# karpathy/minbpe

Hardware: AMD Instinct MI355X
Metric: BPE merges/sec (higher is better)
Workload: dtype int32; 1 GPU; regex1g: RegexTokenizer.train, 1 GB synth seed 2, vocab 32000; mode=default, parallelism=single

## Files before the change

minbpe_amd/csrc/api/api_ctx.hip:

```cpp

struct DpComm {
    bpe_allreduce_fn fn = nullptr;
    void *user = nullptr;
    int rank = 0, nranks = 1;
};

struct bpe_ctx {
    int device = 0;
    int num_cus = 256;
    hipStream_t stream = nullptr;
    bool own_stream = false;
    std::string err;

    uint8_t *d_bytes = nullptr;
    uint64_t nbytes = 0, cap_bytes = 0;
    uint64_t *d_offsets = nullptr;
    uint64_t n_chunks = 0, cap_offsets = 0;
    bool have_bytes = false;
    uint8_t *d_wexp = nullptr;
    const struct DpComm *dp_comm = nullptr;
    long long *d_dp_ckey = nullptr;
    uint32_t *d_dp_cfold = nullptr;
    uint64_t cap_dp_cfold = 0;
    bool dp_force_comm = false;
    int dp_kcap = DP_KCAP_DEFAULT;
    uint64_t *d_round_lb = nullptr;
    uint64_t cap_round_lb = 0;
    bool fuse_load = true;
    uint64_t cap_wexp = 0;
    bool weighted = false;

    uint32_t *d_ids[2] = {nullptr, nullptr};
    uint64_t cap_ids = 0;
    int par = 0;
    uint64_t n = 0;
    bool have_ids = false;

    uint32_t *d_mat = nullptr, *d_first = nullptr, *d_rowmax = nullptr;
    uint32_t vcap = 0;
    uint32_t vcur = 0;
    bool stats_valid = false;

    DevState *d_st = nullptr;
    uint64_t *d_tsum = nullptr, *d_tile_off = nullptr;
    uint8_t *d_tile_sin = nullptr;
    unsigned long long *d_sup = nullptr;
    uint64_t cap_tiles = 0;
    IterRec *h_rec = nullptr;
    int rec_cap = 0;
    unsigned long long *d_scratch = nullptr;
    uint32_t *d_delta = nullptr;
    uint32_t *d_dirty_list = nullptr;
    uint32_t *d_dirty_n = nullptr;
    int depth = 8;
    int repack_acc = 200;
    double repack_waste = 0.0;
    int use_slots = 2;
    int fused_rows = 0;
    uint32_t sel_epoch = 0;
    unsigned long long apply_target = 0;
    int rep_shift = 5;
    bool slotted = false;
    uint64_t slot_T = 0;
    int mq = 0;
    uint32_t *d_meta[2] = {nullptr, nullptr};
    uint4 *d_hdr[2] = {nullptr, nullptr};
    uint32_t *d_slot_lens = nullptr;
    unsigned long long *d_slot_off = nullptr, *d_slot_bsum = nullptr;
    uint32_t *d_ids2 = nullptr;
    bool slot2 = false;
    SlotHdr *d_hdr2[2] = {nullptr, nullptr};
    StageRec *d_stage = nullptr;
    uint32_t *d_smask = nullptr;
    uint32_t *d_cand = nullptr;
    uint32_t *d_idx = nullptr;
    uint32_t *d_idx_tmp = nullptr;
    uint32_t *d_idx_dirty = nullptr;
    uint32_t *d_removed = nullptr;
    uint64_t idx_cap_words = 0;
    uint64_t idx_cap_rows = 0;
    bool idx_rebuild = false;
    bool last_aa_indexed = false;
    bool idx_live = false;
    int use_sparse = 1;
    int rep_max = 8;
    int rep_min = 4;
    int lds_delta = 1;
    int exp_no_delta = 0;
    int tie_window = 0;
    int tie_index = 1;
    int sparse_ratio = 1;
    uint64_t last_count = ~0ull;
    uint64_t n_sparse = 0, n_dense = 0, n_index_builds = 0;
    uint64_t n_lean = 0, n_deferred = 0;
    int lean = 1;
    int64_t lean_count = 1 << 20;
    int lean_backoff = 1;
    int lean_grid = 256;
    int lean_scan = 31;
    int lean_select = 1;
    int aa_sparse = 1;
    int lean_chain = 1;
    int chain_dense = 1;
    unsigned long long *d_chain_req = nullptr;
    int ts = TILE2_MAX;
    int small_slots = 1;
    int count_is_removed = 1;
    int chain_prefetch = 1;
    int chain_kcap = CH_KSWEEP;
    int fuse_step = 0;
    unsigned long long *d_step_pub = nullptr;
    uint32_t *d_step_bar = nullptr;
    uint32_t step_bar_target = 0;
    bool forced = false;
    int32_t *d_forced = nullptr;
    uint64_t cap_forced = 0;
    int enc_replay = 1;
    int pinned_upload = 1;
    uint8_t *h_stage = nullptr;
    hipEvent_t ev_stage[4] = {nullptr, nullptr, nullptr, nullptr};
    bool stage_busy[4] = {false, false, false, false};
    uint64_t n_fused = 0;
    unsigned long long *d_step_stamps = nullptr;
    int pool_hint = 0;
    PoolEnt *d_pool = nullptr;
    uint32_t *d_pool_gather = nullptr;
    int chain_scan = 127;
    int chain = 1;
    StepRec *h_srec = nullptr;
    uint64_t n_steps = 0, n_full = 0, n_chained = 0;
    int lean_sum = 1;
    uint4 *d_lean_sum = nullptr;
    bool sum_valid = false;
    uint32_t *d_dbits = nullptr;
    unsigned long long *d_lean_res = nullptr;
    uint32_t lean_tag = 0;
    bool rows_pending = false;
    uint64_t cap_slots = 0;
    int dp_rank = 0, dp_nranks = 1, dp_merges = 0, dp_enq = 0, dp_done = 0;
    bool dp_active = false;
    void *comm = nullptr;
    int comm_rank = 0, comm_nranks = 1;
    uint32_t *d_dp_folded = nullptr, *d_dp_table = nullptr;
    long long *d_dp_key = nullptr;
    uint64_t dp_cur_len = 0;
    bool dp_sparse = false;
    uint32_t dp_dl = 0;
    std::vector<uint8_t> dp_flip;
    int merge_impl = 0;
    unsigned long long *d_desc = nullptr;
    unsigned long long *d_gdesc = nullptr;
    uint64_t cap_desc = 0;
    uint32_t epoch = 0;
    uint32_t lb_tune = 1;

    uint32_t *d_enc_tmp = nullptr, *d_enc_len = nullptr;
    int32_t *d_enc_out = nullptr;
    unsigned long long *d_enc_off = nullptr, *d_enc_bsum = nullptr, *d_enc_long = nullptr;
    unsigned long long *d_enc_huge = nullptr;
    int enc_long = 1;
    unsigned long long *d_ht_keys = nullptr;
    uint32_t *d_ht_vals = nullptr;
    int32_t *d_merge_ids = nullptr;
    uint64_t cap_enc_n = 0, cap_enc_chunks = 0, cap_ht = 0, cap_merge_ids = 0;
    EncEntry *d_enc_tab = nullptr;
    uint32_t *d_enc_rep = nullptr;
    uint8_t *d_enc_mid = nullptr;
    uint32_t *d_enc_midn = nullptr;
    uint64_t cap_enc_tab = 0;
    int enc_cache = 1;
    int enc_chain = 1;
    int enc_hash_bits = 0;

    uint8_t *d_dec_blob = nullptr, *d_dec_out = nullptr;
    unsigned long long *d_dec_voff = nullptr, *d_dec_off = nullptr, *d_dec_bsum = nullptr;
    int32_t *d_dec_ids = nullptr;
    uint32_t *d_dec_len = nullptr;
    uint64_t cap_dec_blob = 0, cap_dec_voff = 0, cap_dec_n = 0, cap_dec_out = 0;
    uint32_t dec_V = 0;
    bool dec_have_vocab = false, dec_have_result = false;
    uint64_t dec_n = 0, dec_total = 0;

    int mode = 1;
    int profile = 0;
    int prof_iter = -1;
    int prof_stride = 64;
    bool prof_active = false;
    int scan_sup_min = 1024;
    int k1 = 2;
    bool stream_is_bytes = false;

    std::vector<ProfEv> prof_open;
    std::vector<hipEvent_t> ev_pool;
    double prof_ms[BPE_PROF_NKINDS] = {0};
    uint64_t prof_launches[BPE_PROF_NKINDS] = {0};
    uint64_t prof_bytes[BPE_PROF_NKINDS] = {0};
};

#define GK(c, kern) ((c)->ts == TILE2_MIN ? bpe::bpe_g1::kern : bpe::bpe_g4::kern)
inline uint32_t idx_h(const bpe_ctx *c) { return c->ts == TILE2_MIN ? bpe::bpe_g1::IDX_H : bpe::bpe_g4::IDX_H; }

namespace {

int fail(bpe_ctx *c, int code, const char *fmt, ...) {
    char buf[512];
    va_list ap;
    va_start(ap, fmt);
    vsnprintf(buf, sizeof buf, fmt, ap);
    va_end(ap);
    if (c) c->err = buf; else g_create_err = buf;
    return code;
}

#define HIPCHK(c, call)                                                                  \
    do {                                                                                 \
        hipError_t e_ = (call);                                                          \
        if (e_ != hipSuccess)                                                            \
            return fail((c), BPE_E_HIP, "%s failed: %s (%s:%d)", #call, hipGetErrorString(e_), \
                        __FILE__, __LINE__);                                             \
    } while (0)

#define LAUNCHCHK(c, name)                                                                \
    do {                                                                                  \
        hipError_t e_ = hipGetLastError();                                                \
        if (e_ != hipSuccess)                                                             \
            return fail((c), BPE_E_HIP, "launch %s failed: %s", name, hipGetErrorString(e_)); \
    } while (0)

#define TRY(expr)              \
    do {                       \
        int rc_ = (expr);      \
        if (rc_ != BPE_OK) return rc_; \
    } while (0)

struct DevTmp {
    void *p = nullptr;
    DevTmp() = default;
    DevTmp(const DevTmp &) = delete;
    DevTmp &operator=(const DevTmp &) = delete;
    ~DevTmp() {
        if (p) (void)hipFree(p);
    }
    hipError_t alloc(size_t bytes) { return hipMalloc(&p, bytes ? bytes : 1); }
    template <typename T>
    T *as() const { return (T *)p; }
};

struct EventList {
    std::vector<hipEvent_t> v;
    ~EventList() {
        for (hipEvent_t e : v)
            if (e) (void)hipEventDestroy(e);
    }
};

template <typename T>
int dev_realloc(bpe_ctx *c, T *&p, size_t count) {
    if (p) HIPCHK(c, hipFree(p));
    p = nullptr;
    if (count) HIPCHK(c, hipMalloc((void **)&p, count * sizeof(T)));
    return BPE_OK;
}

inline uint64_t ntiles_of(uint64_t n) { return (n + TILE - 1) / TILE; }

int ensure_ids(bpe_ctx *c, uint64_t n) {
    const uint64_t need = (ntiles_of(n) + 2) * TILE;
    if (need > c->cap_ids) {
        TRY(dev_realloc(c, c->d_ids[0], need));
        TRY(dev_realloc(c, c->d_ids[1], need));
        TRY(dev_realloc(c, c->d_ids2, need));
        c->cap_ids = need;
    }
    const uint64_t nt = ntiles_of(n) + 1;
    const uint64_t nt2 = (TILE / TILE2_MIN) * nt + 4;
    if (nt > c->cap_tiles) {
        TRY(dev_realloc(c, c->d_tsum, nt));
        TRY(dev_realloc(c, c->d_tile_off, nt));
        TRY(dev_realloc(c, c->d_tile_sin, nt));
        TRY(dev_realloc(c, c->d_sup, 2 * 3 * (nt / SUP_TILES + 2)));
        TRY(dev_realloc(c, c->d_meta[0], nt));
        TRY(dev_realloc(c, c->d_meta[1], nt));
        TRY(dev_realloc(c, c->d_hdr[0], nt));
        TRY(dev_realloc(c, c->d_hdr[1], nt));
        TRY(dev_realloc(c, c->d_hdr2[0], nt2));
        TRY(dev_realloc(c, c->d_hdr2[1], nt2));
        TRY(dev_realloc(c, c->d_stage, nt2));
        TRY(dev_realloc(c, c->d_smask, nt2 / 32 + 2));
        TRY(dev_realloc(c, c->d_cand, nt2));
        HIPCHK(c, hipMemsetAsync(c->d_smask, 0, (nt2 / 32 + 2) * sizeof(uint32_t), c->stream));
        TRY(dev_realloc(c, c->d_slot_lens, nt2));
        TRY(dev_realloc(c, c->d_slot_off, nt2 + 1));
        TRY(dev_realloc(c, c->d_slot_bsum, nt2 / SCAN_TILE + 2));
        TRY(dev_realloc(c, c->d_desc, nt2));
        TRY(dev_realloc(c, c->d_gdesc, nt / 64 + 2));
        HIPCHK(c, hipMemsetAsync(c->d_desc, 0, nt2 * sizeof(unsigned long long), c->stream));
        HIPCHK(c, hipMemsetAsync(c->d_gdesc, 0, (nt / 64 + 2) * sizeof(unsigned long long), c->stream));
        c->cap_tiles = nt;
    }
    return BPE_OK;
}

int ensure_table(bpe_ctx *c, uint32_t v) {
    if (v > 65535) return fail(c, BPE_E_LIMIT, "vocab %u exceeds this build's 65535 limit", v);
    if (v <= c->vcap) return BPE_OK;
    uint32_t nv = std::max<uint32_t>(v, 256);
    nv = (nv + 63) & ~63u;
    TRY(dev_realloc(c, c->d_mat, (size_t)nv * nv));
    TRY(dev_realloc(c, c->d_rowmax, (size_t)nv * 2));
    TRY(dev_realloc(c, c->d_delta, (size_t)nv * 4 * DELTA_REPL + 256 * DELTA_SKEW));
    TRY(dev_realloc(c, c->d_dirty_list, (size_t)nv));
    if (!c->d_dirty_n) HIPCHK(c, hipMalloc((void **)&c->d_dirty_n, sizeof(uint32_t)));
    if (!c->d_dbits) {
        HIPCHK(c, hipMalloc((void **)&c->d_dbits, DBITS_WORDS * sizeof(uint32_t)));
        HIPCHK(c, hipMemsetAsync(c->d_dbits, 0, DBITS_WORDS * sizeof(uint32_t), c->stream));
    }
    TRY(dev_realloc(c, c->d_lean_res, 2 * ((size_t)nv + 8)));
    if (!c->d_lean_sum) HIPCHK(c, hipMalloc((void **)&c->d_lean_sum, 4 * (size_t)LEAN_SUM_CAP * sizeof(uint4)));
    HIPCHK(c, hipMemsetAsync(c->d_lean_res, 0, 2 * ((size_t)nv + 8) * sizeof(unsigned long long), c->stream));
    if (!c->d_removed) {
        HIPCHK(c, hipMalloc((void **)&c->d_removed, 256 * REMOVED_STRIDE * sizeof(uint32_t)));
        HIPCHK(c, hipMemsetAsync(c->d_removed, 0, 256 * REMOVED_STRIDE * sizeof(uint32_t), c->stream));
    }
    HIPCHK(c, hipMemsetAsync(c->d_delta, 0, ((size_t)nv * 4 * DELTA_REPL + 256 * DELTA_SKEW) * sizeof(uint32_t), c->stream));
    HIPCHK(c, hipMemsetAsync(c->d_dirty_n, 0, sizeof(uint32_t), c->stream));
    HIPCHK(c, hipMemsetAsync(c->d_rowmax, 0, (size_t)nv * 2 * sizeof(uint32_t), c->stream));
    if (c->d_first) {
        HIPCHK(c, hipFree(c->d_first));
        c->d_first = nullptr;
    }
    c->vcap = nv;
    c->stats_valid = false;
    return BPE_OK;
}

int ensure_rec(bpe_ctx *c, int n) {
    if (n <= c->rec_cap) return BPE_OK;
    if (c->h_rec) HIPCHK(c, hipHostFree(c->h_rec));
    c->h_rec = nullptr;
    HIPCHK(c, hipHostMalloc((void **)&c->h_rec, sizeof(IterRec) * (size_t)n, hipHostMallocMapped));
    c->rec_cap = n;
    return BPE_OK;
}

int ensure_srec(bpe_ctx *c) {
    if (!c->h_srec) HIPCHK(c, hipHostMalloc((void **)&c->h_srec, sizeof(StepRec) * STEP_RING, hipHostMallocMapped));
    memset(c->h_srec, 0, sizeof(StepRec) * STEP_RING);
    return BPE_OK;
}

constexpr int PROF_FULL_ITERS = 1024;
int prof_begin(bpe_ctx *c, int kind, uint64_t bytes) {
    c->prof_active = c->profile >= 2 || (c->profile == 1 && kind == BPE_PROF_MERGE);
    if (!c->prof_active) return BPE_OK;
    uint32_t weight = 1;
    if (c->prof_iter >= PROF_FULL_ITERS && c->prof_stride > 1) {
        if (c->prof_iter % c->prof_stride) {
            c->prof_active = false;
            return BPE_OK;
        }
        weight = (uint32_t)c->prof_stride;
    }
    ProfEv ev;
    ev.kind = kind;
    ev.bytes = bytes;
    ev.weight = weight;
    for (hipEvent_t *e : {&ev.e0, &ev.e1}) {
        if (!c->ev_pool.empty()) {
            *e = c->ev_pool.back();
            c->ev_pool.pop_back();
        } else {
            HIPCHK(c, hipEventCreate(e));
        }
    }
    HIPCHK(c, hipEventRecord(ev.e0, c->stream));
    c->prof_open.push_back(ev);
    return BPE_OK;
}
int prof_end(bpe_ctx *c) {
    if (!c->prof_active) return BPE_OK;
    c->prof_active = false;
    HIPCHK(c, hipEventRecord(c->prof_open.back().e1, c->stream));
    return BPE_OK;
}
int prof_drain(bpe_ctx *c) {
    if (c->prof_open.empty()) return BPE_OK;
    HIPCHK(c, hipStreamSynchronize(c->stream));
    for (ProfEv &ev : c->prof_open) {
        float ms = 0.f;
        HIPCHK(c, hipEventElapsedTime(&ms, ev.e0, ev.e1));
        c->prof_ms[ev.kind] += (double)ms * ev.weight;
        c->prof_launches[ev.kind] += ev.weight;
        c->prof_bytes[ev.kind] += ev.bytes * ev.weight;
        c->ev_pool.push_back(ev.e0);
        c->ev_pool.push_back(ev.e1);
    }
    c->prof_open.clear();
    return BPE_OK;
}

int dp_allreduce(bpe_ctx *c, void *buf, uint64_t count, int32_t dtype, int32_t op) {
    const DpComm *dp = c->dp_comm;
    if (!dp || !dp->fn) return fail(c, BPE_E_STATE, "no communicator");
    if (dp->nranks == 1 && !c->dp_force_comm) return BPE_OK;
    const int rc = dp->fn(dp->user, buf, count, dtype, op, (void *)c->stream);
    if (rc != 0) return fail(c, BPE_E_HIP, "all-reduce failed (%d)", rc);
    return BPE_OK;
}

inline unsigned grid_for(uint64_t work_items, unsigned per_block, unsigned cap) {
    uint64_t g = (work_items + per_block - 1) / per_block;
    if (g < 1) g = 1;
    if (g > cap) g = cap;
    return (unsigned)g;
}

inline bool load_count_fusable(const bpe_ctx *c) { return c->fuse_load && c->k1 == 2 && !c->weighted && c->nbytes >= 2; }

int start_from_bytes(bpe_ctx *c, bool count = false) {
    const uint64_t n = c->nbytes;
    TRY(ensure_ids(c, n));
    if (count) {
        const uint64_t segs = (n + LC_SEG - 1) / LC_SEG;
        if (segs + 2 > c->cap_round_lb) {
            TRY(dev_realloc(c, c->d_round_lb, (size_t)segs + 2));
            c->cap_round_lb = segs + 2;
        }
        TRY(prof_begin(c, BPE_PROF_PAIR_COUNT, 4 * n));
        const uint64_t *off = c->n_chunks ? c->d_offsets : nullptr;
        if (off) {
            hipLaunchKernelGGL(k_seg_lb, dim3((unsigned)((segs + 256) / 256)), dim3(256), 0, c->stream, off,
                               (uint64_t)c->n_chunks, segs, c->d_round_lb);
            LAUNCHCHK(c, "k_seg_lb");
        }
        const uint64_t wgs = (segs + LC_WAVES - 1) / LC_WAVES;
        hipLaunchKernelGGL(k_load_count, dim3((unsigned)std::min<uint64_t>(wgs, (uint64_t)c->num_cus)), dim3(PC_THREADS),
                           LC_LDS_BYTES, c->stream, c->d_bytes, off, c->d_round_lb, (uint64_t)c->n_chunks, n, c->d_ids[0],
                           c->d_mat, c->vcap);
        LAUNCHCHK(c, "k_load_count");
        hipLaunchKernelGGL(k_init_state, dim3(1), dim3(1), 0, c->stream, c->d_st, (unsigned long long)n);
        LAUNCHCHK(c, "k_init_state");
        TRY(prof_end(c));
    } else {
        TRY(prof_begin(c, BPE_PROF_WIDEN, 5 * n));
        if (n) {
            hipLaunchKernelGGL(k_widen, dim3(grid_for(n, 256 * 16, c->num_cus * 8)), dim3(256), 0,
                               c->stream, c->d_bytes, c->d_ids[0], n);
            LAUNCHCHK(c, "k_widen");
            if (c->n_chunks) {
                hipLaunchKernelGGL(k_mark_starts, dim3(grid_for(c->n_chunks, 256, c->num_cus * 8)),
                                   dim3(256), 0, c->stream, c->d_ids[0], c->d_offsets, c->n_chunks, n);
                LAUNCHCHK(c, "k_mark_starts");
                if (c->weighted) {
                    hipLaunchKernelGGL(k_mark_weights, dim3(grid_for(c->n_chunks, 256, c->num_cus * 8)), dim3(256),
                                       0, c->stream, c->d_ids[0], c->d_offsets, c->d_wexp, c->n_chunks, n);
                    LAUNCHCHK(c, "k_mark_weights");
                }
            }
        }
        hipLaunchKernelGGL(k_init_state, dim3(1), dim3(1), 0, c->stream, c->d_st, (unsigned long long)n);
        LAUNCHCHK(c, "k_init_state");
        TRY(prof_end(c));
    }
    c->apply_target = 0;
    c->par = 0;
    c->n = n;
    c->vcur = 256;
    c->have_ids = true;
    c->stats_valid = false;
    c->stream_is_bytes = true;
    return BPE_OK;
}

int clear_table(bpe_ctx *c) {
    TRY(prof_begin(c, BPE_PROF_TABLE, 0));
    HIPCHK(c, hipMemsetAsync(c->d_mat, 0, (size_t)c->vcur * c->vcap * sizeof(uint32_t), c->stream));
    TRY(prof_end(c));
    return BPE_OK;
}

int launch_pair_count(bpe_ctx *c, bool with_first) {
    const uint64_t n = c->n;
    TRY(prof_begin(c, BPE_PROF_PAIR_COUNT, 4 * n));
    if (n >= 2) {
        if (with_first) {
            hipLaunchKernelGGL(k_pair_count_simple<true>, dim3(grid_for(n, 1024, c->num_cus * 8)),
                               dim3(256), 0, c->stream, c->d_ids[c->par], c->d_st, c->par, c->d_mat,
                               c->vcap, c->d_first);
        } else if (c->k1 == 0) {
            hipLaunchKernelGGL(k_pair_count_simple<false>, dim3(grid_for(n, 1024, c->num_cus * 8)),
                               dim3(256), 0, c->stream, c->d_ids[c->par], c->d_st, c->par, c->d_mat,
                               c->vcap, (uint32_t *)nullptr);
        } else if (c->k1 == 2 && c->vcur <= 256 && c->stream_is_bytes && !c->weighted) {
            hipLaunchKernelGGL(k_pair_count_bytes, dim3(grid_for(n, 4 * PC_THREADS, c->num_cus)),
                               dim3(PC_THREADS), PC_LDS_BYTES, c->stream, c->d_ids[c->par], c->d_st,
                               c->par, c->d_mat, c->vcap);
        } else if (c->k1 >= 3 && !c->weighted && c->vcap <= 65536) {
            hipLaunchKernelGGL(k_pair_count_h32, dim3(grid_for(n, 4 * PC_THREADS, c->num_cus)),
                               dim3(PC_THREADS), PC_LDS_BYTES, c->stream, c->d_ids[c->par], c->d_st,
                               c->par, c->d_mat, c->vcap);
        } else {
            hipLaunchKernelGGL(k_pair_count_lds, dim3(grid_for(n, 4 * PC_THREADS, c->num_cus)),
                               dim3(PC_THREADS), PC_LDS_BYTES, c->stream, c->d_ids[c->par], c->d_st,
                               c->par, c->d_mat, c->vcap);
        }
        LAUNCHCHK(c, "k_pair_count");
    }
    TRY(prof_end(c));
    return BPE_OK;
}

inline uint32_t vcap_rep(const bpe_ctx *c) { return c->vcap | ((uint32_t)c->rep_shift << 24); }

SlotRef stream_ref(const bpe_ctx *c) {
    SlotRef r;
    if (c->slotted) {
        r.b0 = c->d_ids[0];
        r.b1 = c->d_ids[1];
        r.meta = c->d_meta[c->mq];
        r.T = c->slot_T;
    } else {
        r.b0 = c->d_ids[c->par];
        r.b1 = nullptr;
        r.meta = nullptr;
        r.T = 0;
    }
    return r;
}

SlotRefH stream_ref_h(const bpe_ctx *c) {
    SlotRefH r;
    r.b0 = c->d_ids[0];
    r.b1 = c->d_ids[1];
    r.hdr = c->d_hdr2[c->mq];
    r.T = c->slot_T;
    return r;
}

inline bool aa_through_index(const bpe_ctx *c) { return c->aa_sparse && c->idx_live; }

int launch_select(bpe_ctx *c, bool rowmax_all, bool sparse_next = false) {
    TRY(prof_begin(c, BPE_PROF_ARGMAX, 0));
    if (c->forced) {
        hipLaunchKernelGGL(GK(c, k_forced_pair), dim3(1), dim3(1), 0, c->stream, c->d_st, c->d_forced, (uint32_t)c->prof_iter,
                           c->d_mat, c->vcap);
        LAUNCHCHK(c, "k_forced_pair");
        if (sparse_next && c->slotted && c->slot2) {
            CandArgs C;
            C.idx = c->d_idx;
            C.dirty = c->d_idx_dirty;
            C.cand = c->d_cand;
            C.stride = (uint32_t)c->idx_cap_words;
            C.T = (uint32_t)c->slot_T;
            C.enable = 1;
            C.tie_index = C.tie_window = 0;
            C.aa = aa_through_index(c) ? 1u : 0u;
            hipLaunchKernelGGL(GK(c, k_dp_cand), dim3(1), dim3(1024), 0, c->stream, c->d_st, C);
            LAUNCHCHK(c, "k_dp_cand");
        }
        TRY(prof_end(c));
        return BPE_OK;
    }
    if (rowmax_all) {
        hipLaunchKernelGGL(k_rowmax_all, dim3(c->vcur), dim3(256), 0, c->stream, c->d_mat, c->vcap,
                           c->vcur, c->d_rowmax);
        LAUNCHCHK(c, "k_rowmax_all");
    }
    const uint64_t nslots = c->slotted ? c->slot_T : ntiles_of(c->n);
    const unsigned blocks = (unsigned)std::max<uint64_t>(1, std::min<uint64_t>(nslots, TIE_BLOCKS));
    CandArgs C;
    C.idx = c->d_idx;
    C.dirty = c->d_idx_dirty;
    C.cand = c->d_cand;
    C.stride = (uint32_t)c->idx_cap_words;
    C.T = (uint32_t)c->slot_T;
    C.enable = sparse_next ? 1u : 0u;
    C.tie_index = (c->slotted && c->slot2 && c->idx_live && c->tie_index) ? 1u : 0u;
    C.tie_window = c->tie_window ? 1u : 0u;
    C.aa = (sparse_next && aa_through_index(c)) ? 1u : 0u;
    if (c->slotted && c->slot2)
        hipLaunchKernelGGL(GK(c, k_select<SlotRefH>), dim3(blocks), dim3(1024), 0, c->stream, c->d_rowmax, c->d_mat,
                           c->vcap, c->vcur, c->d_st, stream_ref_h(c), c->par, c->dp_active ? 1 : 0,
                           ++c->sel_epoch, C);
    else
        hipLaunchKernelGGL(k_select<SlotRef>, dim3(blocks), dim3(1024), 0, c->stream, c->d_rowmax, c->d_mat,
                           c->vcap, c->vcur, c->d_st, stream_ref(c), c->par, c->dp_active ? 1 : 0,
                           ++c->sel_epoch, C);
    LAUNCHCHK(c, "k_select");
    TRY(prof_end(c));
    return BPE_OK;
}

int launch_rowsel_lean(bpe_ctx *c) {
    TRY(prof_begin(c, BPE_PROF_ARGMAX, 0));
    CandArgs C;
    C.idx = c->d_idx;
    C.dirty = c->d_idx_dirty;
    C.cand = nullptr;
    C.stride = (uint32_t)c->idx_cap_words;
    C.T = (uint32_t)c->slot_T;
    C.enable = 0;
    C.tie_index = 1;
    C.tie_window = 0;
    C.aa = 0;
    hipLaunchKernelGGL(GK(c, k_rowsel_lean), dim3(1 + (unsigned)c->lean_scan), dim3(1024), 0, c->stream, c->d_rowmax, c->d_mat,
                       c->vcap, c->vcur, c->d_st, stream_ref_h(c), C, c->d_dbits, c->d_lean_res, ++c->lean_tag);
    LAUNCHCHK(c, "k_rowsel_lean");
    TRY(prof_end(c));
    c->rows_pending = false;
    return BPE_OK;
}

int launch_sel_lean(bpe_ctx *c) {
    TRY(prof_begin(c, BPE_PROF_ARGMAX, 0));
    CandArgs C;
    C.idx = c->d_idx;
    C.dirty = c->d_idx_dirty;
    C.cand = nullptr;
    C.stride = (uint32_t)c->idx_cap_words;
    C.T = (uint32_t)c->slot_T;
    C.enable = 0;
    C.tie_index = 1;
    C.tie_window = 0;
    C.aa = 0;
    const uint32_t nwv = ((c->vcur + 255u) / 256u) * 4u;
    hipLaunchKernelGGL(GK(c, k_sel_lean), dim3(1 + (unsigned)c->lean_scan), dim3(1024), 0, c->stream, c->d_rowmax, c->d_mat,
                       c->vcap, c->vcur, c->d_st, stream_ref_h(c), C, c->d_dbits, c->d_lean_res, ++c->lean_tag,
                       c->d_lean_sum, nwv, (uint32_t)c->lean_chain);
    LAUNCHCHK(c, "k_sel_lean");
    TRY(prof_end(c));
    c->rows_pending = false;
    return BPE_OK;
}

int flush_lean_rows(bpe_ctx *c, uint32_t ncols) {
    if (!c->rows_pending) return BPE_OK;
    TRY(prof_begin(c, BPE_PROF_TABLE, 0));
    hipLaunchKernelGGL(GK(c, k_rowmax_lean), dim3((unsigned)c->lean_scan), dim3(1024), 0, c->stream, c->d_mat, c->vcap,
                       c->d_rowmax, c->d_st, ncols, c->d_dbits);
    LAUNCHCHK(c, "k_rowmax_lean");
    TRY(prof_end(c));
    c->rows_pending = false;
    return BPE_OK;
}

template <bool FOLDED>
int launch_table_update(bpe_ctx *c, uint32_t *delta, uint32_t Z, int par, IterRec *rec, int iter,
                        int slot_finish) {
    const uint32_t na = (Z + 1 + 31) / 32;
    if (c->fused_rows) {
        c->apply_target += na;
        hipLaunchKernelGGL(k_apply_delta<FOLDED>, dim3(na + ROW_BLOCKS), dim3(256), 0, c->stream, c->d_mat,
                           c->vcap, delta, FOLDED ? c->vcap : vcap_rep(c), c->d_rowmax, c->d_st, Z,
                           c->d_dirty_list, c->d_dirty_n, par, rec, iter, slot_finish, na,
                           c->apply_target);
    } else {
        hipLaunchKernelGGL(k_apply_delta<FOLDED>, dim3(na), dim3(256), 0, c->stream, c->d_mat, c->vcap,
                           delta, FOLDED ? c->vcap : vcap_rep(c), c->d_rowmax, c->d_st, Z,
                           c->d_dirty_list, c->d_dirty_n, par, rec, iter, slot_finish, na, 0ull);
        LAUNCHCHK(c, "k_apply_delta");
        hipLaunchKernelGGL(k_rowmax_list, dim3(ROW_BLOCKS), dim3(256), 0, c->stream, c->d_mat, c->vcap,
                           Z + 1, c->d_rowmax, c->d_st, c->d_dirty_list, c->d_dirty_n);
    }
    LAUNCHCHK(c, "k_apply_delta");
    return BPE_OK;
}

int launch_merge(bpe_ctx *c, uint32_t newid, int iter, IterRec *rec, bool with_delta) {
    const uint64_t n = c->n;
    const uint64_t nt = ntiles_of(n);
    TRY(prof_begin(c, BPE_PROF_MERGE, 0));
    if (c->merge_impl == 1) {
        if ((++c->epoch & EPOCH_MASK) == 0) {
            HIPCHK(c, hipMemsetAsync(c->d_desc, 0, c->cap_tiles * sizeof(unsigned long long), c->stream));
            HIPCHK(c, hipMemsetAsync(c->d_gdesc, 0, (c->cap_tiles / 64 + 2) * sizeof(unsigned long long), c->stream));
            c->epoch++;
        }
        const unsigned grid = (unsigned)std::max<uint64_t>(nt, 1);
        if (with_delta)
            hipLaunchKernelGGL(k_merge_lookback<true>, dim3(grid), dim3(MT), 0, c->stream,
                               c->d_ids[c->par], c->d_ids[c->par ^ 1], c->d_st, c->par, c->d_desc,
                               c->d_gdesc, c->epoch, newid, c->d_delta, vcap_rep(c), rec, iter, c->d_dirty_n, c->lb_tune);
        else
            hipLaunchKernelGGL(k_merge_lookback<false>, dim3(grid), dim3(MT), 0, c->stream,
                               c->d_ids[c->par], c->d_ids[c->par ^ 1], c->d_st, c->par, c->d_desc,
                               c->d_gdesc, c->epoch, newid, (uint32_t *)nullptr, c->vcap, rec, iter, c->d_dirty_n,
                               c->lb_tune);
        LAUNCHCHK(c, "k_merge_lookback");
    } else {
    if (nt) {
        hipLaunchKernelGGL(k_merge_count, dim3((unsigned)nt), dim3(MT), 0, c->stream,
                           c->d_ids[c->par], c->d_st, c->par, c->d_tsum);
        LAUNCHCHK(c, "k_merge_count");
    }
    if (nt > (uint64_t)c->scan_sup_min) {
        static_assert(sizeof(TS) == 24, "a TS is three 8-byte words");
        const uint64_t nsup = (nt + SUP_TILES - 1) / SUP_TILES;
        TS *ssum = reinterpret_cast<TS *>(c->d_sup), *spre = ssum + (nt / SUP_TILES + 2);
        hipLaunchKernelGGL(k_tile_sup, dim3((unsigned)nsup), dim3(SUP_TILES), 0, c->stream, c->d_tsum, nt, c->d_st, c->par, ssum);
        hipLaunchKernelGGL(k_tile_scan_sup, dim3(1), dim3(1024), 0, c->stream, ssum, nsup, spre, c->d_st, c->par, rec, iter,
                           c->d_ids[c->par], c->d_dirty_n);
        hipLaunchKernelGGL(k_tile_expand, dim3((unsigned)nsup), dim3(SUP_TILES), 0, c->stream, c->d_tsum, nt, c->d_st, c->par,
                           spre, c->d_tile_off, c->d_tile_sin);
    } else {
        hipLaunchKernelGGL(k_tile_scan, dim3(1), dim3(1024), 0, c->stream, c->d_tsum, nt, c->d_tile_off,
                           c->d_tile_sin, c->d_st, c->par, rec, iter, c->d_ids[c->par], c->d_dirty_n);
    }
    LAUNCHCHK(c, "k_tile_scan");
    if (nt) {
        if (with_delta)
            hipLaunchKernelGGL(k_merge_scatter<true>, dim3((unsigned)nt), dim3(MT), 0, c->stream,
                               c->d_ids[c->par], c->d_ids[c->par ^ 1], c->d_st, c->par,
                               c->d_tile_off, c->d_tile_sin, newid, c->d_delta, vcap_rep(c));
        else
            hipLaunchKernelGGL(k_merge_scatter<false>, dim3((unsigned)nt), dim3(MT), 0, c->stream,
                               c->d_ids[c->par], c->d_ids[c->par ^ 1], c->d_st, c->par,
                               c->d_tile_off, c->d_tile_sin, newid, (uint32_t *)nullptr, c->vcap);
        LAUNCHCHK(c, "k_merge_scatter");
    }
    }
    TRY(prof_end(c));
    if (with_delta && c->dp_active) {
        hipLaunchKernelGGL(k_dp_fold, dim3((c->vcap + 255) / 256), dim3(256), 0, c->stream, c->d_delta,
                           vcap_rep(c), newid, c->d_dp_folded);
        LAUNCHCHK(c, "k_dp_fold");
    } else if (with_delta) {
        TRY(prof_begin(c, BPE_PROF_TABLE, 0));
        TRY(launch_table_update<false>(c, c->d_delta, newid, 0, nullptr, 0, 0));
        TRY(prof_end(c));
    }
    c->par ^= 1;
    c->stats_valid = false;
    c->stream_is_bytes = false;
    return BPE_OK;
}


int slots_enter(bpe_ctx *c) {
    c->slot_T = ntiles_of(c->n);
    c->mq = 0;
    hipLaunchKernelGGL(k_slot_init, dim3(grid_for(std::max<uint64_t>(c->slot_T, 1), 256, c->num_cus * 4)),
                       dim3(256), 0, c->stream, c->d_meta[0], c->d_hdr[0], c->slot_T, c->d_st, c->par,
                       (uint32_t)c->par, c->d_ids[c->par]);
    LAUNCHCHK(c, "k_slot_init");
    c->slotted = true;
    return BPE_OK;
}

int slots_leave(bpe_ctx *c) {
    const uint64_t T = c->slot_T;
    if (T) {
        const uint64_t nb = (T + SCAN_TILE - 1) / SCAN_TILE;
        hipLaunchKernelGGL(k_slot_lens, dim3(grid_for(T, 256, c->num_cus * 4)), dim3(256), 0, c->stream,
                           c->d_meta[c->mq], T, c->d_slot_lens);
        hipLaunchKernelGGL(k_scan_blocksum, dim3((unsigned)nb), dim3(256), 0, c->stream, c->d_slot_lens, T,
                           c->d_slot_bsum);
        hipLaunchKernelGGL(k_scan_top, dim3(1), dim3(1024), 0, c->stream, c->d_slot_bsum, nb,
                           c->d_scratch + 3);
        hipLaunchKernelGGL(k_scan_apply, dim3((unsigned)nb), dim3(256), 0, c->stream, c->d_slot_lens, T,
                           c->d_slot_bsum, c->d_slot_off);
        hipLaunchKernelGGL(k_slot_compact, dim3((unsigned)T), dim3(256), 0, c->stream, c->d_ids[0],
                           c->d_ids[1], c->d_meta[c->mq], c->d_slot_off, c->d_ids2);
        LAUNCHCHK(c, "k_slot_compact");
    }
    std::swap(c->d_ids[0], c->d_ids2);
    if (c->par != 0) {
        hipLaunchKernelGGL(k_move_n, dim3(1), dim3(1), 0, c->stream, c->d_st, c->par, 0);
        LAUNCHCHK(c, "k_move_n");
    }
    c->par = 0;
    c->slotted = false;
    return BPE_OK;
}

int launch_merge_slot(bpe_ctx *c, uint32_t newid, int iter, IterRec *rec) {
    TRY(prof_begin(c, BPE_PROF_MERGE, 0));
    if ((++c->epoch & EPOCH_MASK) == 0) {
        HIPCHK(c, hipMemsetAsync(c->d_desc, 0, c->cap_tiles * sizeof(unsigned long long), c->stream));
        HIPCHK(c, hipMemsetAsync(c->d_gdesc, 0, (c->cap_tiles / 64 + 2) * sizeof(unsigned long long), c->stream));
        c->epoch++;
    }
    const unsigned slot_grid = (unsigned)std::max<uint64_t>(c->slot_T, 1);
    hipLaunchKernelGGL(k_merge_slot<true>, dim3(slot_grid), dim3(MT), 0,
                       c->stream, c->d_ids[0], c->d_ids[1], c->d_ids[0], c->d_ids[1], c->d_meta[c->mq],
                       c->d_meta[c->mq ^ 1], c->slot_T, c->d_st, c->par, newid, c->d_delta, vcap_rep(c),
                       c->d_dirty_n, c->d_desc, c->epoch, c->d_hdr[c->mq], c->d_hdr[c->mq ^ 1]);
    LAUNCHCHK(c, "k_merge_slot");
    TRY(prof_end(c));
    if (c->dp_active) {
        hipLaunchKernelGGL(k_dp_fold, dim3((c->vcap + 255) / 256), dim3(256), 0, c->stream, c->d_delta,
                           vcap_rep(c), newid, c->d_dp_folded);
        LAUNCHCHK(c, "k_dp_fold");
    } else {
        TRY(prof_begin(c, BPE_PROF_TABLE, 0));
        TRY(launch_table_update<false>(c, c->d_delta, newid, c->par, rec, iter, 1));
        TRY(prof_end(c));
    }
    c->par ^= 1;
    c->mq ^= 1;
    c->stats_valid = false;
    c->stream_is_bytes = false;
    return BPE_OK;
}

constexpr unsigned SPARSE_GRID = 1024;

int index_build(bpe_ctx *c) {
    const uint64_t nwords = (c->slot_T + 31) / 32;
    if (nwords + 4 > c->idx_cap_words || idx_h(c) > c->idx_cap_rows) {
        if (c->d_idx) HIPCHK(c, hipFree(c->d_idx));
        if (c->d_idx_dirty) HIPCHK(c, hipFree(c->d_idx_dirty));
        c->d_idx = c->d_idx_dirty = nullptr;
        const uint64_t cap = (nwords + 4 + 63) / 64 * 64;
        if (c->d_idx_tmp) HIPCHK(c, hipFree(c->d_idx_tmp));
        c->d_idx_tmp = nullptr;
        c->idx_cap_words = c->idx_cap_rows = 0;
        HIPCHK(c, hipMalloc((void **)&c->d_idx, cap * idx_h(c) * sizeof(uint32_t)));
        HIPCHK(c, hipMalloc((void **)&c->d_idx_tmp, cap * idx_h(c) * sizeof(uint32_t)));
        HIPCHK(c, hipMalloc((void **)&c->d_idx_dirty, cap * sizeof(uint32_t)));
        c->idx_cap_words = cap;
        c->idx_cap_rows = idx_h(c);
    }
    if (nwords) {
        hipLaunchKernelGGL(GK(c, k_index_build), dim3((unsigned)nwords), dim3(1024), (size_t)idx_h(c) * 4, c->stream,
                           c->d_ids[0], c->d_ids[1], c->d_hdr2[c->mq], (uint32_t)c->slot_T, c->d_idx_tmp,
                           c->d_idx_dirty, c->d_st);
        LAUNCHCHK(c, "k_index_build");
        hipLaunchKernelGGL(GK(c, k_index_transpose), dim3((unsigned)((nwords + 31) / 32), idx_h(c) / 32), dim3(256), 0,
                           c->stream, c->d_idx_tmp, (uint32_t)nwords, c->d_idx, (uint32_t)c->idx_cap_words);
        LAUNCHCHK(c, "k_index_transpose");
    }
    c->idx_live = true;
    c->idx_rebuild = false;
    c->n_index_builds++;
    return BPE_OK;
}

int slots2_enter(bpe_ctx *c) {
    c->slot_T = (c->n + (uint64_t)c->ts - 1) / (uint64_t)c->ts;
    c->mq = 0;
    hipLaunchKernelGGL(GK(c, k_slot2_init), dim3(grid_for(std::max<uint64_t>(c->slot_T, 1), 256, c->num_cus * 4)),
                       dim3(256), 0, c->stream, c->d_hdr2[0], c->slot_T, c->d_st, c->par, (uint32_t)c->par,
                       c->d_ids[c->par]);
    LAUNCHCHK(c, "k_slot2_init");
    c->slotted = true;
    c->slot2 = true;
    HIPCHK(c, hipMemsetAsync(c->d_smask, 0, (c->slot_T / 32 + 1) * sizeof(uint32_t), c->stream));
    if (c->idx_live) TRY(index_build(c));
    return BPE_OK;
}

int slots2_leave(bpe_ctx *c) {
    const uint64_t T = c->slot_T;
    if (T) {
        const uint64_t nb = (T + SCAN_TILE - 1) / SCAN_TILE;
        hipLaunchKernelGGL(GK(c, k_slot2_lens), dim3(grid_for(T, 256, c->num_cus * 4)), dim3(256), 0, c->stream,
                           c->d_hdr2[c->mq], T, c->d_slot_lens);
        hipLaunchKernelGGL(k_scan_blocksum, dim3((unsigned)nb), dim3(256), 0, c->stream, c->d_slot_lens, T,
                           c->d_slot_bsum);
        hipLaunchKernelGGL(k_scan_top, dim3(1), dim3(1024), 0, c->stream, c->d_slot_bsum, nb,
                           c->d_scratch + 3);
        hipLaunchKernelGGL(k_scan_apply, dim3((unsigned)nb), dim3(256), 0, c->stream, c->d_slot_lens, T,
                           c->d_slot_bsum, c->d_slot_off);
        hipLaunchKernelGGL(GK(c, k_slot2_compact), dim3((unsigned)((T + 3) / 4)), dim3(256), 0, c->stream, c->d_ids[0],
                           c->d_ids[1], c->d_hdr2[c->mq], T, c->d_slot_off, c->d_ids2);
        LAUNCHCHK(c, "k_slot2_compact");
    }
    std::swap(c->d_ids[0], c->d_ids2);
    if (c->par != 0) {
        hipLaunchKernelGGL(k_move_n, dim3(1), dim3(1), 0, c->stream, c->d_st, c->par, 0);
        LAUNCHCHK(c, "k_move_n");
    }
    c->par = 0;
    c->slotted = false;
    c->slot2 = false;
    return BPE_OK;
}

inline uint32_t delta_layout(const bpe_ctx *c, uint32_t Z) {
    const uint32_t dstride = std::min<uint32_t>(c->vcap, ((Z + 1 + 63) / 64) * 64);
    const uint64_t buf_words = (uint64_t)c->vcap * 4 * DELTA_REPL;
    int shift = 0;
    while (shift < 7 && ((uint64_t)dstride * 4 << (shift + 1)) <= buf_words) shift++;
    const uint64_t cnt = c->last_count;
    const int want = cnt >= (1u << 20) ? 8 : (cnt >= (1u << 16) ? 5 : (cnt >= (1u << 12) ? 3 : 0));
    return dstride | ((uint32_t)std::min(std::min(shift, std::max(want, c->rep_min)), c->rep_max) << 24);
}

int plan_pass2(bpe_ctx *c, bool *sparse_out) {
    const uint32_t T = (uint32_t)c->slot_T;
    const bool small = T <= 16 * SPARSE_GRID;
    const bool can_index = c->use_sparse && T > 0 && (c->use_sparse == 2 || !small || c->lean);
    const bool rare = c->last_count != ~0ull && (small ? c->last_count <= (uint64_t)c->lean_count
                                                       : c->last_count * (uint64_t)c->sparse_ratio < T);
    const bool sparse = can_index && (c->use_sparse == 2 || rare);
    if (sparse && c->small_slots && c->ts != TILE2_MIN && (!small || c->small_slots == 2)) {
        TRY(slots2_leave(c));
        c->ts = TILE2_MIN;
        TRY(slots2_enter(c));
    }
    if (sparse && (!c->idx_live || c->idx_rebuild)) TRY(index_build(c));
    *sparse_out = sparse;
    return BPE_OK;
}

int launch_passes2(bpe_ctx *c, uint32_t newid, bool sparse, uint32_t dl) {
    TRY(prof_begin(c, BPE_PROF_MERGE, 0));
    if ((++c->epoch & EPOCH_MASK) == 0) {
        HIPCHK(c, hipMemsetAsync(c->d_desc, 0, ((TILE / TILE2_MIN) * c->cap_tiles + 4) * sizeof(unsigned long long), c->stream));
        c->epoch++;
    }
    const uint32_t T = (uint32_t)c->slot_T;
    AbArgs A;
    A.b0 = c->d_ids[0];
    A.b1 = c->d_ids[1];
    A.hdr_in = c->d_hdr2[c->mq];
    A.hdr_out = c->d_hdr2[c->mq ^ 1];
    A.stage = c->d_stage;
    A.smask = c->d_smask;
    A.T = T;
    A.st = c->d_st;
    A.newid = newid;
    A.delta = c->exp_no_delta ? nullptr : c->d_delta;
    A.vcap = dl;
    A.idx = c->idx_live ? c->d_idx : nullptr;
    A.istride = (uint32_t)c->idx_cap_words;
    A.cand = c->d_cand;
    A.removed = c->d_removed;
    A.dirty_n = c->d_dirty_n;
    const bool ldsd = c->lds_delta && newid + 1 <= (uint32_t)LDSD_CAP;
    if (sparse) {
        if (ldsd)
            hipLaunchKernelGGL(GK(c, k_merge_ab_sparse<true>), dim3(SPARSE_GRID), dim3(MT), 0, c->stream, A);
        else
            hipLaunchKernelGGL(GK(c, k_merge_ab_sparse<false>), dim3(SPARSE_GRID), dim3(MT), 0, c->stream, A);
        c->n_sparse++;
    } else {
        const unsigned g = std::max((T + MT / 64 - 1) / (MT / 64), 1u);
        const unsigned ge = std::min(g, 5u * (unsigned)c->num_cus);
        if (ldsd && A.idx)
            hipLaunchKernelGGL(GK(c, k_merge_ab_dense_early<true>), dim3(ge), dim3(MT), 0, c->stream, A);
        else if (ldsd)
            hipLaunchKernelGGL(GK(c, k_merge_ab_dense_early<false>), dim3(ge), dim3(MT), 0, c->stream, A);
        else if (A.idx)
            hipLaunchKernelGGL(GK(c, k_merge_ab_dense<true>), dim3(g), dim3(MT), 0, c->stream, A);
        else
            hipLaunchKernelGGL(GK(c, k_merge_ab_dense<false>), dim3(g), dim3(MT), 0, c->stream, A);
        c->n_dense++;
    }
    LAUNCHCHK(c, "k_merge_ab");
    AaArgs B;
    B.b0 = c->d_ids[0];
    B.b1 = c->d_ids[1];
    B.w0 = c->d_ids[0];
    B.w1 = c->d_ids[1];
    B.hdr_in = A.hdr_in;
    B.hdr_out = A.hdr_out;
    B.stage = sparse ? c->d_stage : nullptr;
    B.smask = c->d_smask;
    B.T = T;
    B.st = c->d_st;
    B.newid = newid;
    B.delta = c->d_delta;
    B.vcap = dl;
    B.sdesc = c->d_desc;
    B.epoch = c->epoch;
    const bool aas = sparse && aa_through_index(c);
    B.dirty = (c->idx_live && !aas) ? c->d_idx_dirty : nullptr;
    B.removed = c->d_removed;
    B.cand = aas ? c->d_cand : nullptr;
    B.idx = aas ? c->d_idx : nullptr;
    B.istride = (uint32_t)c->idx_cap_words;
    c->last_aa_indexed = aas;
    hipLaunchKernelGGL(GK(c, k_merge_aa), dim3(std::max(1u, std::min(T, 8u * (unsigned)c->num_cus))), dim3(64), 0,
                       c->stream, B);
    LAUNCHCHK(c, "k_merge_aa");
    TRY(prof_end(c));
    return BPE_OK;
}

int launch_table2(bpe_ctx *c, uint32_t newid, int iter, IterRec *rec, bool sparse, uint32_t dl, bool folded) {
    const uint32_t T = (uint32_t)c->slot_T;
    TRY(prof_begin(c, BPE_PROF_TABLE, 0));
    const uint32_t na = (newid + 1 + 31) / 32;
    if (folded)
        hipLaunchKernelGGL(k_apply2<true>, dim3(na + 8), dim3(256), 0, c->stream, c->d_mat, c->vcap, c->d_dp_folded,
                           c->vcap, c->d_rowmax, c->d_st, newid, c->d_dirty_list, c->d_dirty_n, c->par, rec, iter,
                           na, c->d_hdr2[c->mq], c->d_stage, c->d_removed, c->d_smask, (T + 31) / 32);
    else
        hipLaunchKernelGGL(k_apply2<false>, dim3(na + 8), dim3(256), 0, c->stream, c->d_mat, c->vcap, c->d_delta, dl,
                           c->d_rowmax, c->d_st, newid, c->d_dirty_list, c->d_dirty_n, c->par, rec, iter, na,
                           c->d_hdr2[c->mq], c->d_stage, c->d_removed, c->d_smask, (T + 31) / 32);
    LAUNCHCHK(c, "k_apply2");
    hipLaunchKernelGGL(k_rowmax_list, dim3(ROW_BLOCKS), dim3(1024), 0, c->stream, c->d_mat, c->vcap, newid + 1,
                       c->d_rowmax, c->d_st, c->d_dirty_list, c->d_dirty_n);
    LAUNCHCHK(c, "k_rowmax_list");
    TRY(prof_end(c));
    c->par ^= 1;
    if (!sparse) c->mq ^= 1;
    c->stats_valid = false;
    c->stream_is_bytes = false;
    return BPE_OK;
}

int launch_merge2(bpe_ctx *c, uint32_t newid, int iter, IterRec *rec, bool sparse) {
    const uint32_t dl = delta_layout(c, newid);
    TRY(launch_passes2(c, newid, sparse, dl));
    return launch_table2(c, newid, iter, rec, sparse, dl, false);
}

int launch_lean(bpe_ctx *c, uint32_t newid, int iter, IterRec *rec, bool use_index) {
    const uint32_t T = (uint32_t)c->slot_T;
    const uint32_t dl = delta_layout(c, newid);
    AbArgs A;
    A.b0 = c->d_ids[0];
    A.b1 = c->d_ids[1];
    A.hdr_in = c->d_hdr2[c->mq];
    A.hdr_out = nullptr;
    A.stage = c->d_stage;
    A.smask = c->d_smask;
    A.T = T;
    A.st = c->d_st;
    A.newid = newid;
    A.delta = c->d_delta;
    A.vcap = dl;
    A.idx = c->idx_live ? c->d_idx : nullptr;
    A.istride = (uint32_t)c->idx_cap_words;
    A.cand = nullptr;
    A.removed = c->d_removed;
    A.dirty_n = c->d_dirty_n;
    const uint32_t nwords = (T + 31) / 32;
    const unsigned g = std::max(1u, std::min(use_index ? nwords : (T + 15) / 16, (unsigned)c->lean_grid));
    TRY(prof_begin(c, BPE_PROF_MERGE, 0));
    if (c->idx_live)
        hipLaunchKernelGGL(GK(c, k_merge_ab_lean<true>), dim3(g), dim3(LEAN_MT), 0, c->stream, A, c->d_idx_dirty,
                           use_index ? 1u : 0u, c->d_dbits);
    else
        hipLaunchKernelGGL(GK(c, k_merge_ab_lean<false>), dim3(g), dim3(LEAN_MT), 0, c->stream, A, (const uint32_t *)nullptr, 0u,
                           c->d_dbits);
    LAUNCHCHK(c, "k_merge_ab_lean");
    TRY(prof_end(c));
    TRY(prof_begin(c, BPE_PROF_TABLE, 0));
    const uint32_t na = (newid + 1 + 255) / 256;
    const uint32_t ncommit = std::max(8u, std::min(128u, (nwords + 255) / 256));
    hipLaunchKernelGGL(GK(c, k_apply_lean), dim3(na + ncommit), dim3(256), 0, c->stream, c->d_mat, c->vcap, c->d_delta, dl,
                       c->d_rowmax, c->d_st, newid, c->d_dbits, c->par, rec, iter, na, c->d_hdr2[c->mq], c->d_stage,
                       c->d_removed, c->d_smask, nwords, c->d_lean_sum);
    LAUNCHCHK(c, "k_apply_lean");
    TRY(prof_end(c));
    c->par ^= 1;
    c->stats_valid = false;
    c->stream_is_bytes = false;
    c->rows_pending = true;
    c->n_lean++;
    if (use_index) c->n_sparse++; else c->n_dense++;
    return BPE_OK;
}

int launch_chain_step(bpe_ctx *c, uint32_t step, uint32_t zhi, bool use_index, bool records, bool dense = false) {
    const uint32_t T = (uint32_t)c->slot_T;
    const uint32_t dl = delta_layout(c, zhi);
    const bool fused = c->fuse_step && !c->forced && !dense && !c->dp_comm && use_index && c->idx_live;
    if (!fused) TRY(prof_begin(c, BPE_PROF_ARGMAX, 0));
    CandArgs C;
    C.idx = c->d_idx;
    C.dirty = c->d_idx_dirty;
    C.cand = nullptr;
    C.stride = (uint32_t)c->idx_cap_words;
    C.T = T;
    C.enable = 0;
    C.tie_index = 1;
    C.tie_window = 0;
    C.aa = 0;
    if (!c->idx_live) C.T = 0;
    if (dense && c->dp_comm) C.T = 0;
    (void)records;
    if (!c->d_chain_req) {
        HIPCHK(c, hipMalloc((void **)&c->d_chain_req, PL_REQ_WORDS * sizeof(unsigned long long)));
        HIPCHK(c, hipMemsetAsync(c->d_chain_req, 0, PL_REQ_WORDS * sizeof(unsigned long long), c->stream));
    }
    if (!c->d_pool) {
        HIPCHK(c, hipMalloc((void **)&c->d_pool, (3 * PL_CAP + 128) * sizeof(PoolEnt)));
        HIPCHK(c, hipMalloc((void **)&c->d_pool_gather, (2 + 2 * PL_GATHER) * sizeof(uint32_t)));
        HIPCHK(c, hipMemsetAsync(c->d_pool, 0, (3 * PL_CAP + 128) * sizeof(PoolEnt), c->stream));
        HIPCHK(c, hipMemsetAsync(c->d_pool_gather, 0, (2 + 2 * PL_GATHER) * sizeof(uint32_t), c->stream));
    }
    const DpComm *dp = c->dp_comm;
    uint32_t kcap = (uint32_t)(dense ? CH_KDENSE : std::min(CH_KSWEEP, c->chain_kcap));
    if (dp) kcap = std::min(kcap, (uint32_t)c->dp_kcap);
    const uint32_t hint_below = (uint32_t)(c->pool_hint > 0 ? c->pool_hint : (int)kcap);
    const unsigned nscan = (unsigned)std::max(1, std::min(c->chain_scan, c->num_cus - 1));
    if (fused) {
        if (!c->d_step_pub) {
            HIPCHK(c, hipMalloc((void **)&c->d_step_pub, 64 * sizeof(unsigned long long)));
            HIPCHK(c, hipMemsetAsync(c->d_step_pub, 0, 64 * sizeof(unsigned long long), c->stream));
        }
        if (!c->d_step_bar) {
            HIPCHK(c, hipMalloc((void **)&c->d_step_bar, 256));
            HIPCHK(c, hipMemsetAsync(c->d_step_bar, 0, 256, c->stream));
            c->step_bar_target = 0;
        }
        const uint32_t nwords = (T + 31) / 32;
        StepArgs S;
        S.rowmax = c->d_rowmax;
        S.mat = c->d_mat;
        S.stride = c->vcap;
        S.st = c->d_st;
        S.ref = stream_ref_h(c);
        S.C = C;
        S.dbits = c->d_dbits;
        S.res = c->d_lean_res;
        S.tag = ++c->lean_tag;
        S.req = c->d_chain_req;
        S.kcap = kcap;
        S.pool = c->d_pool;
        S.gather = c->d_pool_gather;
        S.hint_below = hint_below;
        AbArgs &A = S.A;
        A.b0 = c->d_ids[0];
        A.b1 = c->d_ids[1];
        A.hdr_in = c->d_hdr2[c->mq];
        A.hdr_out = nullptr;
        A.stage = c->d_stage;
        A.smask = c->d_smask;
        A.T = T;
        A.st = c->d_st;
        A.newid = 0;
        A.delta = c->d_delta;
        A.vcap = dl;
        A.idx = c->d_idx;
        A.istride = (uint32_t)c->idx_cap_words;
        A.cand = nullptr;
        uint32_t *const removed = (c->weighted || !c->count_is_removed) ? c->d_removed : nullptr;
        A.removed = removed;
        A.dirty_n = c->d_dirty_n;
        S.idx_dirty = c->d_idx_dirty;
        S.use_index = 1u | (c->chain_prefetch ? 2u : 0u);
        const unsigned gapply = (zhi + 1 + 1023) / 1024;
        const unsigned cap = std::min((unsigned)c->num_cus, std::max(std::max((unsigned)c->lean_grid, gapply), 2u));
        const unsigned gmerge = std::max(1u, std::min(std::min(nwords, (unsigned)c->lean_grid), cap));
        const unsigned ns = std::min(nscan, cap - 1);
        const unsigned G = std::min(cap, std::max(std::max(gmerge, gapply), 1 + ns));
        if (G < gapply) return fail(c, BPE_E_INTERNAL, "fused chain step: %u workgroups cannot hold %u tokens", G, zhi + 1);
        S.nscan = ns;
        S.gm = gmerge;
        S.delta = c->d_delta;
        S.dl = dl;
        S.par = c->par;
        S.rec = c->h_rec;
        S.srec = c->h_srec;
        S.step = step;
        S.hdr_cur = c->d_hdr2[c->mq];
        S.stage = c->d_stage;
        S.removed = removed;
        S.smask = c->d_smask;
        S.nwords = nwords;
        S.sums = c->d_lean_sum;
        S.pub = c->d_step_pub;
        S.bar = c->d_step_bar;
        c->step_bar_target += G;
        S.bar_target = c->step_bar_target;
        S.stamps = c->d_step_stamps;
        TRY(prof_begin(c, BPE_PROF_MERGE, 0));
        hipLaunchKernelGGL(GK(c, k_step), dim3(G), dim3(LEAN_MT), 0, c->stream, S);
        LAUNCHCHK(c, "k_step");
        TRY(prof_end(c));
        c->par ^= 1;
        c->stats_valid = false;
        c->stream_is_bytes = false;
        c->rows_pending = true;
        c->n_steps++;
        c->n_fused++;
        c->n_sparse++;
        return BPE_OK;
    }
    if (c->forced)
        hipLaunchKernelGGL(GK(c, k_forced_sel), dim3(1), dim3(64), 0, c->stream, c->d_st, c->d_forced, c->d_mat, c->vcap, kcap);
    else
        hipLaunchKernelGGL(GK(c, k_pool_sel), dim3(1 + nscan), dim3(1024), 0, c->stream, c->d_rowmax, c->d_mat,
                           c->vcap, c->d_st, stream_ref_h(c), C, c->d_dbits, c->d_lean_res, ++c->lean_tag, c->d_chain_req,
                           kcap, c->d_pool, c->d_pool_gather, hint_below, dp ? c->d_dp_ckey : (long long *)nullptr,
                           (unsigned long long)(dp ? dp->rank : 0), c->d_pool + PL_CAP);
    LAUNCHCHK(c, "k_pool_sel");
    if (dp) {
        TRY(dp_allreduce(c, c->d_dp_ckey, DP_KEY_WORDS, BPE_DT_INT64, BPE_OP_MIN));
        hipLaunchKernelGGL(GK(c, k_pool_sel_dp), dim3(1), dim3(PL_CAP), 0, c->stream, c->d_st, c->d_dp_ckey, kcap, c->d_pool,
                           c->d_pool + PL_CAP, hint_below);
        LAUNCHCHK(c, "k_pool_sel_dp");
    }
    TRY(prof_end(c));
    AbArgs A;
    A.b0 = c->d_ids[0];
    A.b1 = c->d_ids[1];
    A.hdr_in = c->d_hdr2[c->mq];
    A.hdr_out = dense ? c->d_hdr2[c->mq ^ 1] : nullptr;
    A.stage = c->d_stage;
    A.smask = c->d_smask;
    A.T = T;
    A.st = c->d_st;
    A.newid = 0;
    A.delta = c->d_delta;
    A.vcap = dl;
    A.idx = c->idx_live ? c->d_idx : nullptr;
    A.istride = (uint32_t)c->idx_cap_words;
    A.cand = nullptr;
    uint32_t *const removed = (c->weighted || dp || !c->count_is_removed) ? c->d_removed : nullptr;
    A.removed = removed;
    A.dirty_n = c->d_dirty_n;
    const uint32_t nwords = (T + 31) / 32;
    TRY(prof_begin(c, BPE_PROF_MERGE, 0));
    if (dense) {
        const unsigned g = std::max(1u, std::min((T + 15) / 16, (unsigned)c->num_cus));
        hipLaunchKernelGGL(GK(c, k_merge_chain_dense), dim3(g), dim3(LEAN_MT), 0, c->stream, A, c->d_dbits);
        const unsigned g1 = std::max(1u, std::min((T + MT / 64 - 1) / (MT / 64), 5u * (unsigned)c->num_cus));
        hipLaunchKernelGGL(GK(c, k_merge_chain_dense1), dim3(g1), dim3(MT), 0, c->stream, A);
    } else {
        const unsigned g = std::max(1u, std::min(use_index ? nwords : (T + 15) / 16, (unsigned)c->lean_grid));
        hipLaunchKernelGGL(GK(c, k_merge_chain), dim3(g), dim3(LEAN_MT), 0, c->stream, A, c->d_idx_dirty,
                           (use_index ? 1u : 0u) | (c->chain_prefetch ? 2u : 0u), c->d_dbits);
    }
    LAUNCHCHK(c, "k_merge_chain");
    TRY(prof_end(c));
    TRY(prof_begin(c, BPE_PROF_TABLE, 0));
    const uint32_t na = (zhi + 1 + 255) / 256;
    const uint32_t ncommit = std::max(8u, std::min(128u, (nwords + 255) / 256));
    const uint32_t fS = std::min<uint32_t>(c->vcap, ((zhi + 1 + 63) / 64) * 64);
    uint32_t *ftail = dp ? c->d_dp_cfold + (size_t)2 * kcap * fS : nullptr;
    if (dp) {
        hipLaunchKernelGGL(GK(c, k_dp_fold_chain), dim3(na), dim3(256), 0, c->stream, c->d_delta, dl, c->d_st, c->d_dp_cfold, fS, ftail);
        LAUNCHCHK(c, "k_dp_fold_chain");
        TRY(dp_allreduce(c, c->d_dp_cfold, (uint64_t)2 * kcap * fS + 64, BPE_DT_INT32, BPE_OP_SUM));
    }
    hipLaunchKernelGGL(GK(c, k_apply_chain), dim3(na + ncommit), dim3(256), 0, c->stream, c->d_mat, c->vcap, c->d_delta, dl, c->d_rowmax,
                       c->d_st, c->d_dbits, c->par, c->h_rec, c->h_srec, step, na, c->d_hdr2[c->mq], c->d_stage,
                       removed, c->d_smask, nwords, c->d_lean_sum, dp ? c->d_dp_cfold : (const uint32_t *)nullptr, fS,
                       (const uint32_t *)ftail);
    LAUNCHCHK(c, "k_apply_chain");
    TRY(prof_end(c));
    c->par ^= 1;
    if (dense) c->mq ^= 1;
    c->stats_valid = false;
    c->stream_is_bytes = false;
    c->rows_pending = true;
    c->n_steps++;
    if (use_index) c->n_sparse++; else c->n_dense++;
    return BPE_OK;
}

constexpr size_t STAGE_PIECE = 32u << 20;
constexpr int STAGE_R = 4, STAGE_T_MAX = 16;
int upload_h2d(bpe_ctx *c, void *dst, const void *src, size_t bytes) {
    if (!bytes) return BPE_OK;
    if (!c->pinned_upload || bytes < 2 * STAGE_PIECE) {
        HIPCHK(c, hipMemcpyAsync(dst, src, bytes, hipMemcpyHostToDevice, c->stream));
        return BPE_OK;
    }
    if (!c->h_stage) {
        if (hipHostMalloc((void **)&c->h_stage, STAGE_PIECE * STAGE_R, hipHostMallocDefault) != hipSuccess) {
            c->h_stage = nullptr;
            (void)hipGetLastError();
            HIPCHK(c, hipMemcpyAsync(dst, src, bytes, hipMemcpyHostToDevice, c->stream));
            return BPE_OK;
        }
        for (int r = 0; r < STAGE_R; r++) HIPCHK(c, hipEventCreateWithFlags(&c->ev_stage[r], hipEventDisableTiming));
    }
    const unsigned hw = std::max(1u, std::thread::hardware_concurrency());
    const int T = (int)std::max(1u, std::min((unsigned)STAGE_T_MAX, hw / 2));
    const size_t pieces = (bytes + STAGE_PIECE - 1) / STAGE_PIECE;
    std::atomic<long long> go{-1};
    std::atomic<unsigned long long> done{0};
    const uint8_t *s8 = static_cast<const uint8_t *>(src);
    uint8_t *stage = c->h_stage;
    auto worker = [&](int w) {
        for (size_t i = 0; i < pieces; i++) {
            while (go.load(std::memory_order_acquire) < (long long)i) std::this_thread::yield();
            const size_t len = std::min(STAGE_PIECE, bytes - i * STAGE_PIECE);
            const size_t per = (len + (size_t)T - 1) / (size_t)T, lo = std::min(len, per * (size_t)w), hi = std::min(len, lo + per);
            if (hi > lo) memcpy(stage + (i % STAGE_R) * STAGE_PIECE + lo, s8 + i * STAGE_PIECE + lo, hi - lo);
            done.fetch_add(1, std::memory_order_release);
        }
    };
    std::vector<std::thread> pool;
    pool.reserve((size_t)T);
    for (int w = 1; w < T; w++) pool.emplace_back(worker, w);
    int rc = BPE_OK;
    hipError_t err = hipSuccess;
    for (size_t i = 0; i < pieces; i++) {
        if (c->stage_busy[i % STAGE_R] && err == hipSuccess) {
            err = hipEventSynchronize(c->ev_stage[i % STAGE_R]);
            c->stage_busy[i % STAGE_R] = false;
        }
        go.store((long long)i, std::memory_order_release);
        {
            const size_t len = std::min(STAGE_PIECE, bytes - i * STAGE_PIECE);
            const size_t per = (len + (size_t)T - 1) / (size_t)T, hi = std::min(len, per);
            if (hi) memcpy(stage + (i % STAGE_R) * STAGE_PIECE, s8 + i * STAGE_PIECE, hi);
            done.fetch_add(1, std::memory_order_release);
        }
        while (done.load(std::memory_order_acquire) < (unsigned long long)T * (i + 1)) std::this_thread::yield();
        if (err == hipSuccess) {
            const size_t len = std::min(STAGE_PIECE, bytes - i * STAGE_PIECE);
            err = hipMemcpyAsync(static_cast<uint8_t *>(dst) + i * STAGE_PIECE, stage + (i % STAGE_R) * STAGE_PIECE, len,
                                 hipMemcpyHostToDevice, c->stream);
            if (err == hipSuccess) err = hipEventRecord(c->ev_stage[i % STAGE_R], c->stream);
            if (err == hipSuccess) c->stage_busy[i % STAGE_R] = true;
        }
    }
    for (std::thread &t : pool) t.join();
    if (err != hipSuccess) rc = fail(c, BPE_E_HIP, "pinned upload: %s", hipGetErrorString(err));
    return rc;
}

int download_d2h(bpe_ctx *c, void *dst, const void *src_dev, size_t bytes) {
    if (!bytes) return BPE_OK;
    if (!c->pinned_upload || bytes < 2 * STAGE_PIECE || !c->h_stage) {
        HIPCHK(c, hipMemcpyAsync(dst, src_dev, bytes, hipMemcpyDeviceToHost, c->stream));
        HIPCHK(c, hipStreamSynchronize(c->stream));
        return BPE_OK;
    }
    const unsigned hw = std::max(1u, std::thread::hardware_concurrency());
    const int T = (int)std::max(1u, std::min((unsigned)STAGE_T_MAX, hw / 2));
    const size_t pieces = (bytes + STAGE_PIECE - 1) / STAGE_PIECE;
    std::atomic<long long> go{-1};
    std::atomic<unsigned long long> done{0};
    uint8_t *d8 = static_cast<uint8_t *>(dst);
    const uint8_t *stage = c->h_stage;
    auto copy_out = [&](size_t i, int w) {
        const size_t len = std::min(STAGE_PIECE, bytes - i * STAGE_PIECE);
        const size_t per = (len + (size_t)T - 1) / (size_t)T, lo = std::min(len, per * (size_t)w), hi = std::min(len, lo + per);
        if (hi > lo) memcpy(d8 + i * STAGE_PIECE + lo, stage + (i % STAGE_R) * STAGE_PIECE + lo, hi - lo);
        done.fetch_add(1, std::memory_order_release);
    };
    auto worker = [&](int w) {
        for (size_t i = 0; i < pieces; i++) {
            while (go.load(std::memory_order_acquire) < (long long)i) std::this_thread::yield();
            copy_out(i, w);
        }
    };
    std::vector<std::thread> pool;
    pool.reserve((size_t)T);
    for (int w = 1; w < T; w++) pool.emplace_back(worker, w);
    hipError_t err = hipSuccess;
    size_t issued = 0;
    for (size_t i = 0; i < pieces; i++) {
        for (; issued < pieces && issued < i + (size_t)STAGE_R && err == hipSuccess; issued++) {
            const size_t len = std::min(STAGE_PIECE, bytes - issued * STAGE_PIECE);
            if (c->stage_busy[issued % STAGE_R]) {
                err = hipEventSynchronize(c->ev_stage[issued % STAGE_R]);
                c->stage_busy[issued % STAGE_R] = false;
                if (err != hipSuccess) break;
            }
            err = hipMemcpyAsync(c->h_stage + (issued % STAGE_R) * STAGE_PIECE, static_cast<const uint8_t *>(src_dev) + issued * STAGE_PIECE,
                                 len, hipMemcpyDeviceToHost, c->stream);
            if (err == hipSuccess) err = hipEventRecord(c->ev_stage[issued % STAGE_R], c->stream);
        }
        if (err == hipSuccess) err = hipEventSynchronize(c->ev_stage[i % STAGE_R]);
        go.store((long long)i, std::memory_order_release);
        copy_out(i, 0);
        while (done.load(std::memory_order_acquire) < (unsigned long long)T * (i + 1)) std::this_thread::yield();
    }
    for (std::thread &t : pool) t.join();
    if (err != hipSuccess) return fail(c, BPE_E_HIP, "pinned download: %s", hipGetErrorString(err));
    return BPE_OK;
}

int read_state(bpe_ctx *c, DevState *out) {
    HIPCHK(c, hipMemcpyAsync(out, c->d_st, sizeof(DevState), hipMemcpyDeviceToHost, c->stream));
    HIPCHK(c, hipStreamSynchronize(c->stream));
    return BPE_OK;
}

}
```

minbpe_amd/csrc/bpe_device.h:

```cpp
#pragma once
#include <stdint.h>

namespace bpe {

constexpr uint32_t FLAG = 0x80000000u;
constexpr uint32_t IDMASK = 0x03FFFFFFu;
constexpr int WSHIFT = 26;
constexpr uint32_t WMASK = 0x7C000000u;
constexpr uint32_t NWMASK = ~WMASK;
constexpr uint32_t INVALID_WORD = 0xFFFFFFFFu;
constexpr uint32_t EMPTY_KEY = 0xFFFFFFFFu;
constexpr unsigned long long NOPOS = ~0ull;

constexpr int MT = 256;
#define BPE_GEOMETRY(NS, MJV, IDXH_LOG2)                                                                         \
    namespace NS {                                                                                               \
    constexpr int MJ = MJV;                            \
    constexpr int WAVE_SPAN = MJ * 256;                                                                          \
    constexpr int TILE = (MT / 64) * WAVE_SPAN;  \
                      \
    constexpr int TILE2 = WAVE_SPAN;                                                                             \
                                  \
    constexpr uint32_t IDX_H = 1u << IDXH_LOG2;                                                                  \
    constexpr int IDX_SHIFT = 32 - IDXH_LOG2;                                                                    \
    }
BPE_GEOMETRY(bpe_g4, 4, 15)
#ifndef BPE_G1_IDXH_LOG2
#define BPE_G1_IDXH_LOG2 13
#endif
BPE_GEOMETRY(bpe_g1, 1, BPE_G1_IDXH_LOG2)
constexpr int TILE2_MAX = 1024, TILE2_MIN = 256;

constexpr int PC_BITS = 14;
constexpr int PC_THREADS = 1024;
constexpr int PC_LDS_BYTES = 131072;
constexpr int PCB_ROUND = 61440;

constexpr int TIE_CAP = 96;
constexpr int ARGMAX_ROWS = 2048;
constexpr uint32_t TIE_WINDOW0 = 0;
constexpr int TIE_BLOCKS = 256;
constexpr int ROW_BLOCKS = 64;
constexpr int DELTA_REPL = 256;
constexpr int DELTA_SKEW = 64;
constexpr int REMOVED_STRIDE = 64;
constexpr int LDSD_CAP = 1920;
__host__ __device__ inline size_t delta_rep_off(uint32_t r, uint32_t stride) {
    return (size_t)r * (4 * (size_t)stride + DELTA_SKEW);
}

constexpr int CH_KMAX = 16;
constexpr int CH_KSWEEP = 15;
constexpr int CH_RSTRIDE = 16;
constexpr uint32_t CH_REP_COUNT = 16384;
constexpr int CH_REP = 4;
constexpr int CH_RMV = 16;
constexpr int DP_KCAP_MAX = CH_KSWEEP;
constexpr int DP_KCAP_DEFAULT = 8;
static_assert(CH_KMAX * CH_RSTRIDE <= DELTA_REPL, "a batch's delta vectors must fit the replica blocks");
static_assert(CH_KMAX * CH_RMV <= 256, "removal counters of a batch");
static_assert(CH_KSWEEP < 16 && CH_KSWEEP <= CH_KMAX, "pair number + 1 must fit a nibble");
constexpr uint32_t CH_FULL = 0, CH_LIST = 1;
constexpr int DP_KEY_WORDS = TIE_CAP + 2;

constexpr int ENC_THREADS = 256;
constexpr int ENC_LMAX = 32;
constexpr int SCAN_TILE = 4096;

constexpr uint32_t ST_OK = 0, ST_EMPTY = 1, ST_INTERNAL = 2, ST_LOOKBACK = 3;
constexpr uint32_t ST_DEFER = 4;
constexpr uint32_t EPOCH_MASK = 0xFFFFFu;
constexpr uint32_t LOOKBACK_SPINS = 1u << 20;

struct SlotRef {
    const uint32_t *b0, *b1;
    const uint32_t *meta;
    unsigned long long T;
};

struct SlotHdr {
    uint32_t w0, w1, w2;
    uint32_t meta;
    uint32_t l0, l1;
    uint32_t pad0, pad1;
};
struct SlotRefH {
    const uint32_t *b0, *b1;
    const SlotHdr *hdr;
    unsigned long long T;
};
struct StageRec {
    uint32_t t, pad[3];
    uint32_t h[8];
};
constexpr uint32_t ROWARG_MULTI = 0xFFFFFFFFu;

struct DevState {
    unsigned long long n[2];
    unsigned long long firstpos;
    int32_t a, b;
    uint32_t count;
    uint32_t ntied;
    uint32_t found;
    uint32_t status;
    int32_t tied[2 * TIE_CAP];
    int32_t fin_a, fin_b;
    unsigned long long removed;
    unsigned long long apply_done;
    uint32_t sel_tie;
    uint32_t sel_done;
    uint32_t adj;
    uint32_t ncand;
    uint32_t gap;
    uint32_t tlive;
    uint32_t defer;
    uint32_t scan_a, scan_b, scan_z;
    uint32_t chain_n, chain_pos, chain_cut;
    uint32_t chain_taken;
    uint32_t sel_ran;
    int32_t chain[2 * TIE_CAP];
    uint32_t iter;
    uint32_t num_merges;
    uint32_t sel_mode;
    uint32_t tl_n, tl_M, tl_skip;
    uint32_t bk, bz0;
    int32_t ba[CH_KMAX], bb[CH_KMAX];
    uint32_t badj[CH_KMAX];
    uint32_t bcnt[CH_KMAX];
    uint32_t brep;
    uint32_t bhm, bhm_key;
    uint32_t dp_wait;
    uint32_t pool_n, pool_theta;
    uint32_t pool_hint;
    uint32_t pool_hint_next;
    unsigned long long pool_epoch;
    alignas(128) uint32_t sel_flag;
    uint32_t pad_flag_[31];
};

struct CandArgs {
    const uint32_t *idx, *dirty;
    uint32_t *cand;
    uint32_t stride;
    uint32_t T;
    uint32_t enable;
    uint32_t tie_index;
    uint32_t tie_window;
    uint32_t aa;
};
struct AbArgs {
    uint32_t *b0, *b1;
    const SlotHdr *hdr_in;
    SlotHdr *hdr_out;
    StageRec *stage;
    uint32_t *smask;
    uint32_t T;
    DevState *st;
    uint32_t newid;
    uint32_t *delta;
    uint32_t vcap;
    uint32_t *idx;
    uint32_t istride;
    const uint32_t *cand;
    uint32_t *removed;
    uint32_t *dirty_n;
};
struct AaArgs {
    const uint32_t *b0, *b1;
    uint32_t *w0, *w1;
    const SlotHdr *hdr_in;
    SlotHdr *hdr_out;
    StageRec *stage;
    uint32_t *smask;
    uint32_t T;
    DevState *st;
    uint32_t newid;
    uint32_t *delta;
    uint32_t vcap;
    unsigned long long *sdesc;
    uint32_t epoch;
    uint32_t *dirty;
    uint32_t *removed;
    const uint32_t *cand;
    uint32_t *idx;
    uint32_t istride;
};
struct PoolEnt {
    uint32_t xy, c;
    unsigned long long key;
};

constexpr uint32_t STEP_RING = 4096;
struct StepRec {
    uint32_t first_iter, k;
    uint32_t status, pad;
    unsigned long long new_len;
    unsigned long long seq;
};

struct IterRec {
    int32_t a, b;
    uint32_t count;
    uint32_t status;
    unsigned long long new_len;
    unsigned long long seq;
};

struct StepArgs {
    uint32_t *rowmax, *mat;
    uint32_t stride;
    DevState *st;
    SlotRefH ref;
    CandArgs C;
    uint32_t *dbits;
    unsigned long long *res;
    uint32_t tag;
    unsigned long long *req;
    uint32_t kcap;
    PoolEnt *pool;
    uint32_t *gather;
    uint32_t hint_below;
    uint32_t nscan;
    AbArgs A;
    const uint32_t *idx_dirty;
    uint32_t use_index;
    uint32_t gm;
    uint32_t *delta;
    uint32_t dl;
    int par;
    IterRec *rec;
    StepRec *srec;
    uint32_t step;
    SlotHdr *hdr_cur;
    const StageRec *stage;
    uint32_t *removed;
    uint32_t *smask;
    uint32_t nwords;
    uint4 *sums;
    unsigned long long *pub;
    uint32_t *bar;
    uint32_t bar_target;
    unsigned long long *stamps;
};
constexpr uint32_t STEP_STAMP_RING = 8192;

}
```

minbpe_amd/csrc/kernels/k_chain.hip:

```cpp
#include <hip/hip_runtime.h>
#include <stdint.h>

#include "../bpe_device.h"

namespace bpe {
namespace BPE_G {

constexpr uint32_t CH_EX_CAP = 2048;

__device__ __forceinline__ int chain_match(const uint32_t *pa, const uint32_t *pb, uint32_t K, uint32_t w0, uint32_t w1) {
    const uint32_t x = w0 & IDMASK, y = w1 & NWMASK;
    int hit = -1;
    for (uint32_t p = 0; p < K; p++)
        if (x == pa[p] && y == pb[p]) hit = (int)p;
    return (w0 == INVALID_WORD) ? -1 : hit;
}

constexpr uint32_t CH_DCAP = 1024;
constexpr uint32_t CH_SD = 2 * CH_DCAP + 2;
__device__ __forceinline__ void chain_slot_load(const AbArgs &A, const uint32_t t, uint4 (&rv)[MJ], uint4 &hv) {
    const int lane = lane_id();
    const uint32_t *src = A.b0 + (size_t)t * TILE2;
#pragma unroll
    for (int j = 0; j < MJ; j++) rv[j] = *reinterpret_cast<const uint4 *>(src + j * 256 + lane * 4);
    hv = (lane & 1) ? make_uint4(INVALID_WORD, INVALID_WORD, 0u, 0u) : make_uint4(INVALID_WORD, INVALID_WORD, INVALID_WORD, 0u);
    const long long hi = 2ll * (long long)t - 2 + lane;
    if (lane < 6 && hi >= 0 && hi < 2ll * (long long)A.T) hv = reinterpret_cast<const uint4 *>(A.hdr_in)[hi];
}
template <bool DENSE, bool THROUGH = false>
__device__ __forceinline__ void merge_chain_wave(uint32_t *__restrict__ out, uint32_t *__restrict__ sd, const uint32_t t, const AbArgs &A,
                                                 const uint32_t *pa, const uint32_t *pb, const uint32_t *pb1,
                                                 const uint32_t K, const uint32_t z0, const uint32_t brep,
                                                 uint4 (&rv)[MJ], const uint4 hv,
                                                 const uint32_t *ph = nullptr, const uint32_t hm = 0,
                                                 const uint32_t tl_in = 0xFFFFFFFFu) {
    const int lane = lane_id();
    const uint32_t Tl = tl_in != 0xFFFFFFFFu ? tl_in : min(A.T, A.st->tlive);
    const uint32_t *src;
    const uint32_t meta = bcast(hv.w, 2);
    const uint32_t len = meta & 0x7FFFFFFFu, buf = meta >> 31;
    auto keep_header = [&]() {
        if (DENSE && (lane == 2 || lane == 3)) reinterpret_cast<uint4 *>(A.hdr_out)[2 * (size_t)t + (lane - 2)] = hv;
    };
    if (len == 0) {
        keep_header();
        return;
    }
    if (buf) {
        src = A.b1 + (size_t)t * TILE2;
#pragma unroll
        for (int j = 0; j < MJ; j++) rv[j] = *reinterpret_cast<const uint4 *>(src + j * 256 + lane * 4);
    }
    const uint32_t first = bcast(hv.x, 2);
    uint32_t halo0 = bcast(hv.x, 4), halo1 = bcast(hv.y, 4), halo2 = bcast(hv.z, 4);
    uint32_t prev2 = bcast(hv.x, 1), prev1 = bcast(hv.y, 1);
    uint32_t tprev = t - 1;
    uint32_t tnext = t + 1;
    {
        const uint32_t nlen = bcast(hv.w, 4) & 0x7FFFFFFFu, plen = bcast(hv.w, 0) & 0x7FFFFFFFu;
        if ((t + 1 < Tl && nlen < 3) || (t > 0 && plen < 2)) {
            uint32_t ctx[7] = {0, 0, 0, 0, 0, 0, 0};
            if (lane == 0) slot_context_walk(A.hdr_in, t, Tl, ctx);
            halo0 = bcast(ctx[0], 0);
            halo1 = bcast(ctx[1], 0);
            halo2 = bcast(ctx[2], 0);
            prev2 = bcast(ctx[3], 0);
            prev1 = bcast(ctx[4], 0);
            tprev = bcast(ctx[5], 0);
            tnext = bcast(ctx[6], 0);
        }
    }
    auto at = [&](int q, uint32_t own) -> uint32_t {
        const int d = q - (int)len;
        return d < 0 ? own : (d == 0 ? halo0 : (d == 1 ? halo1 : (d == 2 ? halo2 : INVALID_WORD)));
    };
    uint32_t x[MJ][4];
#pragma unroll
    for (int j = 0; j < MJ; j++) {
        const int q0 = j * 256 + lane * 4;
        if ((j + 1) * 256 <= (int)len) {
            x[j][0] = rv[j].x;
            x[j][1] = rv[j].y;
            x[j][2] = rv[j].z;
            x[j][3] = rv[j].w;
        } else {
            x[j][0] = at(q0 + 0, rv[j].x);
            x[j][1] = at(q0 + 1, rv[j].y);
            x[j][2] = at(q0 + 2, rv[j].z);
            x[j][3] = at(q0 + 3, rv[j].w);
        }
    }
    uint32_t tail[3];
#pragma unroll
    for (int i = 0; i < 3; i++) tail[i] = at(TILE2 + i, 0u);
    uint32_t rb[MJ], jc[MJ], valid[MJ];
#pragma unroll
    for (int j = 0; j < MJ; j++) {
        rb[j] = 0;
        jc[j] = 0;
    }
    uint32_t s = 0;
    uint32_t ia[MJ];
#pragma unroll
    for (int j = 0; j < MJ; j++) ia[j] = 0;
    uint32_t ip = 0;
    if (hm) {
        auto code = [&](uint32_t w) -> uint32_t {
            const uint32_t id = w & IDMASK;
            const uint32_t e = ph[(__umul24(id, hm) >> 8) & 255u];
            return (e >> 8) == id ? (e & 15u) : 0u;
        };
#pragma unroll
        for (int j = 0; j < MJ; j++) {
#pragma unroll
            for (int k = 0; k < 4; k++) ia[j] |= code(x[j][k]) << (4 * k);
        }
        ip = code(prev1);
    } else {
        for (uint32_t p = 0; p < K; p++) {
            const uint32_t a = pa[p];
#pragma unroll
            for (int j = 0; j < MJ; j++) {
#pragma unroll
                for (int k = 0; k < 4; k++) ia[j] |= ((x[j][k] & IDMASK) == a) ? (p + 1u) << (4 * k) : 0u;
            }
            ip = ((prev1 & IDMASK) == a) ? p + 1u : ip;
        }
    }
#pragma unroll
    for (int j = 0; j < MJ; j++) {
        const uint32_t up = (j < MJ - 1) ? lane_first(x[(j + 1) % MJ][0]) : tail[0];
        const uint32_t nxw = lane_next(x[j][0], up);
#pragma unroll
        for (int k = 0; k < 4; k++) {
            const uint32_t nxt = (k < 3) ? x[j][k + 1] : nxw;
            const uint32_t i = (ia[j] >> (4 * k)) & 15u;
            const uint32_t m = (uint32_t)((nxt & NWMASK) == pb1[i]);
            rb[j] |= m << k;
            jc[j] |= (m ? i : 0u) << (4 * k);
        }
    }
    s = (uint32_t)((prev1 != INVALID_WORD) & ((first & NWMASK) == pb1[ip]));
#pragma unroll
    for (int j = 0; j < MJ; j++) {
        const int nb = (int)len - (j * 256 + lane * 4);
        valid[j] = nb >= 4 ? 0xFu : (nb <= 0 ? 0u : ((1u << nb) - 1u));
    }
    uint32_t anyr = 0;
#pragma unroll
    for (int j = 0; j < MJ; j++) anyr |= rb[j] & valid[j];
    const bool sites = __any(anyr != 0) != 0;
    if (!sites && !s) {
        keep_header();
        return;
    }
    uint32_t mb[MJ], kb[MJ], ex[MJ], cnt[MJ];
#pragma unroll
    for (int j = 0; j < MJ; j++) {
        mb[j] = rb[j] & valid[j];
        const uint32_t upr = (j > 0) ? ((lane_last(rb[(j + MJ - 1) % MJ]) >> 3) & 1u) : s;
        const uint32_t mp = (uint32_t)dpp_mov<0x138>((int)upr, (int)((rb[j] >> 3) & 1u));
        kb[j] = ~((mb[j] << 1) | mp) & valid[j] & 0xFu;
        cnt[j] = (uint32_t)__popc(kb[j]);
    }
    uint32_t total = 0;
    if constexpr (MJ == 4) {
        const uint32_t i01 = wave_iscan_add(cnt[0] | (cnt[1] << 16));
        const uint32_t i23 = wave_iscan_add(cnt[2] | (cnt[3] << 16));
        const uint32_t t01 = lane_last(i01), t23 = lane_last(i23);
        const uint32_t tot0 = t01 & 0xFFFFu, tot1 = t01 >> 16, tot2 = t23 & 0xFFFFu, tot3 = t23 >> 16;
        ex[0] = (i01 & 0xFFFFu) - cnt[0];
        ex[1] = tot0 + (i01 >> 16) - cnt[1];
        ex[2] = tot0 + tot1 + (i23 & 0xFFFFu) - cnt[2];
        ex[3] = tot0 + tot1 + tot2 + (i23 >> 16) - cnt[3];
        total = tot0 + tot1 + tot2 + tot3;
    } else {
#pragma unroll
        for (int j = 0; j < MJ; j++) {
            const uint32_t inc = wave_iscan_add(cnt[j]);
            ex[j] = total + inc - cnt[j];
            total += lane_last(inc);
        }
    }
    uint32_t fstore = 0;
    if (!s) {
        uint32_t fc = 0x7FFFFFFFu;
#pragma unroll
        for (int j = 0; j < MJ; j++) {
            if (mb[j]) {
                const uint32_t k0 = (uint32_t)__ffs((int)mb[j]) - 1u;
                fc = min(fc, ex[j] + (uint32_t)__popc(kb[j] & ((1u << k0) - 1u)));
            }
        }
        fstore = (uint32_t)wave_min_i32((int)fc) & ~3u;
    }
#pragma unroll
    for (int j = 0; j < MJ; j++) {
        uint32_t o = ex[j];
#pragma unroll
        for (int k = 0; k < 4; k++) {
            if ((kb[j] >> k) & 1u) {
                const uint32_t w = x[j][k];
                const uint32_t z = z0 + ((jc[j] >> (4 * k)) & 15u) - 1u;
                out[o++] = ((mb[j] >> k) & 1u) ? (z | (w & (FLAG | WMASK))) : w;
            }
        }
    }
    __builtin_amdgcn_fence(__ATOMIC_RELEASE, "wavefront");
    __builtin_amdgcn_wave_barrier();
    __builtin_amdgcn_fence(__ATOMIC_ACQUIRE, "wavefront");
    {
        uint32_t *dst = (buf ? A.b1 : A.b0) + (size_t)t * TILE2;
        for (uint32_t i = fstore + (uint32_t)lane * 4; i < total; i += 256)
            *reinterpret_cast<uint4 *>(dst + i) = *reinterpret_cast<const uint4 *>(&out[i]);
    }
    if (lane == 0) {
        uint32_t h[8];
        h[0] = total > 0 ? out[0] : INVALID_WORD;
        h[1] = total > 1 ? out[1] : INVALID_WORD;
        h[2] = total > 2 ? out[2] : INVALID_WORD;
        h[3] = total | (buf << 31);
        h[4] = total > 1 ? out[total - 2] : INVALID_WORD;
        h[5] = total > 0 ? out[total - 1] : INVALID_WORD;
        h[6] = h[7] = 0;
        if (DENSE) {
            reinterpret_cast<uint4 *>(A.hdr_out)[2 * (size_t)t] = make_uint4(h[0], h[1], h[2], h[3]);
            reinterpret_cast<uint4 *>(A.hdr_out)[2 * (size_t)t + 1] = make_uint4(h[4], h[5], 0u, 0u);
        } else {
            stage_put<THROUGH>(A.stage + t, t, h);
            atomicOr(&A.smask[t >> 5], 1u << (t & 31));
        }
        if (total < 3 && t + 1 < Tl) A.st->gap = 1;
    }
    if (!sites) return;
    const uint32_t vc = A.vcap & 0xFFFFFFu;
    uint32_t cm2 = 0, ct0 = 0, ct1 = 0;
    if (bcast(mb[0], 0) & 1u) cm2 = (uint32_t)(chain_match(pa, pb, K, prev2, prev1) + 1);
    const uint32_t cm1 = s ? ip : 0u;
    if (bcast(mb[MJ - 1], 63) & 0xCu) {
        ct0 = (uint32_t)(chain_match(pa, pb, K, tail[0], tail[1]) + 1);
        ct1 = (uint32_t)(chain_match(pa, pb, K, tail[1], tail[2]) + 1);
    }
#pragma unroll
    for (int j = 0; j < MJ; j++) {
        if (!__any(mb[j] != 0)) continue;
        uint32_t upm1, dn0;
        if (j > 0) upm1 = lane_last(x[(j + MJ - 1) % MJ][3]);
        else upm1 = prev1;
        if (j < MJ - 1) dn0 = lane_first(x[(j + 1) % MJ][0]);
        else dn0 = tail[0];
        uint32_t W[7];
        W[0] = (uint32_t)dpp_mov<0x138>((int)upm1, (int)x[j][3]);
        W[1] = x[j][0];
        W[2] = x[j][1];
        W[3] = x[j][2];
        W[4] = x[j][3];
        W[5] = lane_next(x[j][0], dn0);
        W[6] = lane_next(x[j][1], (j < MJ - 1) ? lane_first(x[(j + 1) % MJ][1]) : tail[1]);
        const uint32_t lo_fill = (j > 0) ? ((lane_last(jc[(j + MJ - 1) % MJ]) >> 8) & 0xFFu) : (cm2 | (cm1 << 4));
        const uint32_t hi_fill = (j < MJ - 1) ? (lane_first(jc[(j + 1) % MJ]) & 0xFFu) : (ct0 | (ct1 << 4));
        const uint32_t lo = (uint32_t)dpp_mov<0x138>((int)lo_fill, (int)((jc[j] >> 8) & 0xFFu));
        const uint32_t hi = lane_next(jc[j] & 0xFFu, hi_fill);
        const uint32_t win = lo | (jc[j] << 8) | (hi << 24);
        if (mb[j] == 0) continue;
        uint32_t todo = mb[j];
#pragma unroll
        for (int si = 0; si < 2; si++) {
            if (todo == 0) continue;
            const uint32_t k = (uint32_t)__ffs((int)todo) - 1u;
            todo &= todo - 1u;
            const int q = j * 256 + lane * 4 + (int)k;
            const uint32_t wk = win >> (4u * k);
            const uint32_t p = ((wk >> 8) & 15u) - 1u;
            const int li = (int)(wk & 15u) - 1, ri = (int)((wk >> 16) & 15u) - 1;
            const uint32_t Z = z0 + p;
            uint32_t *dl, *dr;
            if (DENSE) {
                dl = sd + p * CH_SD;
                dr = dl + CH_DCAP;
                atomicAdd(&dl[2 * CH_DCAP + 1], 1u);
            } else {
                if (A.removed) atomicAdd(&A.removed[(p * (uint32_t)CH_RMV + (t & (uint32_t)(CH_RMV - 1))) * REMOVED_STRIDE], 1u);
                dl = A.delta + delta_rep_off(p * (uint32_t)CH_RSTRIDE + (t & (brep - 1u)), vc);
                dr = dl + vc;
            }
            const bool k1 = (k & 1u) != 0, k2 = (k & 2u) != 0;
            const uint32_t wa = k2 ? (k1 ? W[4] : W[3]) : (k1 ? W[2] : W[1]);
            const uint32_t wt = word_weight(wa);
            const uint32_t Lw = k2 ? (k1 ? W[3] : W[2]) : (k1 ? W[1] : W[0]);
            if (!(wa & FLAG) && Lw != INVALID_WORD) {
                if (li != (int)p) {
                    const uint32_t Lseq = (li >= 0 && (uint32_t)li < p) ? z0 + (uint32_t)li : (Lw & IDMASK);
                    atomicAdd(&dl[Lseq], wt);
                    if (!DENSE || A.idx) {
                        const uint32_t Lfin = li >= 0 ? z0 + (uint32_t)li : (Lw & IDMASK);
                        index_add(A.idx, A.istride, t, Lfin, Z);
                        if (q == 0) index_add(A.idx, A.istride, tprev, Lfin, Z);
                    }
                }
            }
            const uint32_t R = k2 ? (k1 ? W[6] : W[5]) : (k1 ? W[4] : W[3]);
            if (!(R & FLAG)) {
                if (ri == (int)p) {
                    if (DENSE) atomicAdd(&dl[2 * CH_DCAP], wt);
                    else atomicAdd(&A.st->badj[p], wt);
                } else {
                    atomicAdd(&dr[(ri >= 0 && (uint32_t)ri < p) ? z0 + (uint32_t)ri : (R & IDMASK)], wt);
                }
                if (!DENSE || A.idx) {
                    const uint32_t y = ri >= 0 ? z0 + (uint32_t)ri : (R & IDMASK);
                    index_add(A.idx, A.istride, t, Z, y);
                    if (q + 2 >= (int)len) index_add(A.idx, A.istride, tnext, Z, y);
                }
            }
        }
    }
}

__device__ __forceinline__ uint32_t chain_hash_find(const uint32_t *pa, uint32_t K) {
    if (K < 5) return 0u;
    const uint32_t m = 129u + 2u * (uint32_t)lane_id();
    bool ok = true;
    for (uint32_t i = 1; i < K; i++) {
        const uint32_t hi = (__umul24(pa[i], m) >> 8) & 255u;
        for (uint32_t j = 0; j < i; j++) ok &= hi != ((__umul24(pa[j], m) >> 8) & 255u);
    }
    const unsigned long long bal = __ballot(ok);
    return bal ? 129u + 2u * (uint32_t)(__ffsll((long long)bal) - 1) : 0u;
}
__device__ __forceinline__ uint32_t chain_hash_build(uint32_t *s_ph, uint32_t *s_hm, const uint32_t *s_pa, uint32_t K,
                                                     bool pre_ok = false, uint32_t pre_hm = 0) {
    if (threadIdx.x < 256) s_ph[threadIdx.x] = 0xFFFFFFFFu;
    uint32_t hm = pre_hm;
    if (!pre_ok) {
        if (threadIdx.x == 0) *s_hm = 0;
        __syncthreads();
        if (wave_id() == 0) {
            const uint32_t f = chain_hash_find(s_pa, K);
            if (lane_id() == 0) *s_hm = f;
        }
        __syncthreads();
        hm = *s_hm;
    } else {
        __syncthreads();
    }
    if (hm && threadIdx.x < K) s_ph[(__umul24(s_pa[threadIdx.x], hm) >> 8) & 255u] = (s_pa[threadIdx.x] << 8) | (threadIdx.x + 1u);
    __syncthreads();
    return hm;
}

struct MergeLds {
    alignas(16) uint32_t s_out[LEAN_MT / 64][TILE2];
    uint32_t s_list[LEAN_SUB * 32];
    uint32_t s_tot[2];
    uint32_t s_pa[CH_KMAX], s_pb[CH_KMAX], s_pb1[CH_KMAX + 1];
    uint32_t s_ph[256], s_hm;
};
template <bool THROUGH = false>
__device__ __forceinline__ void merge_chain_body(const AbArgs &A, const uint32_t *__restrict__ idx_dirty, uint32_t use_index,
                                                 MergeLds &L, const uint32_t K, const uint32_t z0, const uint32_t brep,
                                                 const uint32_t blk, const uint32_t nblk, unsigned long long *dbg = nullptr,
                                                 const bool have_st = false, const uint32_t tlive_in = 0, const uint32_t gap_in = 0,
                                                 const bool pre_ok = false, const uint32_t pre_hm = 0) {
    auto dstamp = [&](int i) {
        if (dbg && threadIdx.x == 0) dbg[i] = wall_clock64();
    };
    DevState *st = A.st;
    auto &s_out = L.s_out;
    auto &s_list = L.s_list;
    auto &s_tot = L.s_tot;
    auto &s_pa = L.s_pa;
    auto &s_pb = L.s_pb;
    auto &s_pb1 = L.s_pb1;
    const uint32_t hm = chain_hash_build(L.s_ph, &L.s_hm, s_pa, K, pre_ok, pre_hm);
    const uint32_t *s_ph = L.s_ph;
    const uint32_t Tl = min(A.T, have_st ? tlive_in : st->tlive);
    const uint32_t gap = have_st ? gap_in : st->gap;
    constexpr uint32_t NWV = LEAN_MT / 64;
    AbArgs A1 = A;
    A1.newid = z0;
    const uint32_t a0 = s_pa[0], b0 = s_pb[0];
    auto do_slot = [&](uint32_t t) {
        if (K == 1) {
            merge_ab_wave<true, true, false, THROUGH>(s_out[wave_id()], nullptr, t, A1, a0, b0, Tl);
        } else {
            uint4 rv[MJ], hv;
            chain_slot_load(A, t, rv, hv);
            merge_chain_wave<false, THROUGH>(s_out[wave_id()], nullptr, t, A, s_pa, s_pb, s_pb1, K, z0, brep, rv, hv, s_ph, hm, Tl);
        }
    };
    if (!(use_index & 1u) || gap != 0) {
        const uint32_t nw = nblk * NWV;
        for (uint32_t t = blk * NWV + wave_id(); t < Tl; t += nw) do_slot(t);
        return;
    }
    dstamp(8);
    const uint32_t nwords = (Tl + 31) / 32;
    const uint32_t per = (nwords + nblk - 1) / nblk;
    const uint32_t wlo = blk * per, whi = min(nwords, wlo + per);
    for (uint32_t sub = wlo; sub < whi; sub += LEAN_SUB) {
        uint32_t mk = 0;
        const uint32_t w = sub + threadIdx.x;
        if (threadIdx.x < LEAN_SUB && w < whi) {
            mk = idx_dirty[w];
            for (uint32_t p = 0; p < K; p++) {
                uint32_t h1, h2, h3;
                pair_hash(s_pa[p], s_pb[p], h1, h2, h3);
                mk |= A.idx[(size_t)h1 * A.istride + w] & A.idx[(size_t)h2 * A.istride + w] &
                      A.idx[(size_t)h3 * A.istride + w];
            }
            const uint32_t left = Tl - w * 32;
            if (left < 32) mk &= (1u << left) - 1u;
        }
        const uint32_t c = (uint32_t)__popc(mk);
        const uint32_t inc = wave_iscan_add(c);
        if (threadIdx.x < 128 && lane_id() == 63) s_tot[wave_id()] = inc;
        __syncthreads();
        const uint32_t n = s_tot[0] + s_tot[1];
        if (threadIdx.x < LEAN_SUB) {
            uint32_t o = inc - c + (wave_id() == 1 ? s_tot[0] : 0u);
            while (mk) {
                s_list[o++] = w * 32 + (uint32_t)__ffs((int)mk) - 1u;
                mk &= mk - 1u;
            }
        }
        __syncthreads();
        if (sub == wlo) dstamp(9);
        if (K == 1 || MJ > 1 || !(use_index & 2u)) {
            for (uint32_t i = wave_id(); i < n; i += NWV) do_slot(s_list[i]);
        } else {
            uint32_t i = wave_id();
            uint4 rv[MJ], hv, nrv[MJ], nhv;
            if (i < n) chain_slot_load(A, s_list[i], rv, hv);
            for (; i < n; i += NWV) {
                const bool more = i + NWV < n;
                if (more) chain_slot_load(A, s_list[i + NWV], nrv, nhv);
                merge_chain_wave<false, THROUGH>(s_out[wave_id()], nullptr, s_list[i], A, s_pa, s_pb, s_pb1, K, z0, brep, rv, hv, s_ph, hm, Tl);
                if (more) {
#pragma unroll
                    for (int j = 0; j < MJ; j++) rv[j] = nrv[j];
                    hv = nhv;
                }
            }
        }
        __syncthreads();
    }
}
enum { SW_BK = 48, SW_BZ0, SW_BREP, SW_STATUS, SW_DEFER, SW_SEL_RAN, SW_TLIVE, SW_GAP, SW_BHM, SW_BHM_KEY, SW_ADJ, SW_N };
static_assert(SW_N <= 64, "one wave fetches the state words");
__device__ __forceinline__ void step_words_fetch(const DevState *st, uint32_t *s_w) {
    const uint32_t i = threadIdx.x;
    if (i < (uint32_t)SW_N) {
        const uint32_t *base = reinterpret_cast<const uint32_t *>(st);
        uint32_t off;
        if (i < 16) off = (uint32_t)offsetof(DevState, ba) / 4 + i;
        else if (i < 32) off = (uint32_t)offsetof(DevState, bb) / 4 + (i - 16);
        else if (i < 48) off = (uint32_t)offsetof(DevState, badj) / 4 + (i - 32);
        else {
            constexpr uint32_t o[SW_N - 48] = {
                (uint32_t)offsetof(DevState, bk) / 4,      (uint32_t)offsetof(DevState, bz0) / 4,     (uint32_t)offsetof(DevState, brep) / 4,
                (uint32_t)offsetof(DevState, status) / 4,  (uint32_t)offsetof(DevState, defer) / 4,   (uint32_t)offsetof(DevState, sel_ran) / 4,
                (uint32_t)offsetof(DevState, tlive) / 4,   (uint32_t)offsetof(DevState, gap) / 4,     (uint32_t)offsetof(DevState, bhm) / 4,
                (uint32_t)offsetof(DevState, bhm_key) / 4, (uint32_t)offsetof(DevState, adj) / 4};
            off = o[0];
#pragma unroll
            for (int k = 1; k < SW_N - 48; k++) off = (i == 48u + (uint32_t)k) ? o[k] : off;
        }
        s_w[i] = base[off];
    }
    __syncthreads();
}
__global__ void __launch_bounds__(LEAN_MT)
k_merge_chain(AbArgs A, const uint32_t *__restrict__ idx_dirty, uint32_t use_index, uint32_t *__restrict__ dbits) {
    __shared__ MergeLds L;
    __shared__ uint32_t s_w[64];
    DevState *st = A.st;
    step_words_fetch(st, s_w);
    const uint32_t ran = s_w[SW_SEL_RAN];
    if (blockIdx.x == 0 && ran) {
        for (uint32_t i = threadIdx.x; i < DBITS_WORDS; i += LEAN_MT) dbits[i] = 0;
        __syncthreads();
        if (threadIdx.x == 0) st->sel_ran = 0;
    }
    const uint32_t K = s_w[SW_BK];
    if (s_w[SW_STATUS] || s_w[SW_DEFER] || K == 0) return;
    const uint32_t z0 = s_w[SW_BZ0], brep = s_w[SW_BREP];
    if (threadIdx.x < CH_KMAX) {
        L.s_pa[threadIdx.x] = threadIdx.x < K ? s_w[threadIdx.x] : 0xFFFFFFFFu;
        L.s_pb[threadIdx.x] = threadIdx.x < K ? s_w[16 + threadIdx.x] : 0xFFFFFFFFu;
        L.s_pb1[threadIdx.x + 1] = threadIdx.x < K ? s_w[16 + threadIdx.x] : 0xFFFFFFFFu;
        if (threadIdx.x == 0) L.s_pb1[0] = 0xFFFFFFFFu;
    }
    __syncthreads();
    merge_chain_body(A, idx_dirty, use_index, L, K, z0, brep, blockIdx.x, gridDim.x, nullptr, true, s_w[SW_TLIVE], s_w[SW_GAP],
                     s_w[SW_BHM_KEY] == ((z0 << 8) | K), s_w[SW_BHM]);
}

constexpr int CH_KDENSE = 6;
static_assert((LEAN_MT / 64) * TILE2 * 4 + CH_KDENSE * (int)CH_SD * 4 + 256 <= 160 * 1024, "dense chain pass: LDS");
__global__ void __launch_bounds__(LEAN_MT)
k_merge_chain_dense(AbArgs A, uint32_t *__restrict__ dbits) {
    __shared__ __attribute__((aligned(16))) uint32_t s_out[LEAN_MT / 64][TILE2];
    __shared__ uint32_t s_sd[CH_KDENSE * CH_SD];
    __shared__ uint32_t s_pa[CH_KMAX], s_pb[CH_KMAX], s_pb1[CH_KMAX + 1];
    DevState *st = A.st;
    const uint32_t ran = st->sel_ran;
    if (blockIdx.x == 0 && ran) {
        for (uint32_t i = threadIdx.x; i < DBITS_WORDS; i += LEAN_MT) dbits[i] = 0;
        __syncthreads();
        if (threadIdx.x == 0) st->sel_ran = 0;
    }
    const uint32_t K = st->bk;
    if (!(st->status || st->defer) && K == 1) return;
    if (st->status || st->defer || K == 0 || K > (uint32_t)CH_KDENSE) {
        const uint4 *hi = reinterpret_cast<const uint4 *>(A.hdr_in);
        uint4 *ho = reinterpret_cast<uint4 *>(A.hdr_out);
        for (size_t i = (size_t)blockIdx.x * LEAN_MT + threadIdx.x; i < 2 * (size_t)A.T; i += (size_t)gridDim.x * LEAN_MT) ho[i] = hi[i];
        if (K > (uint32_t)CH_KDENSE && blockIdx.x == 0 && threadIdx.x == 0) st->status = ST_INTERNAL;
        return;
    }
    const uint32_t z0 = st->bz0, brep = st->brep;
    if (threadIdx.x < CH_KMAX) {
        s_pa[threadIdx.x] = threadIdx.x < K ? (uint32_t)st->ba[threadIdx.x] : 0xFFFFFFFFu;
        s_pb[threadIdx.x] = threadIdx.x < K ? (uint32_t)st->bb[threadIdx.x] : 0xFFFFFFFFu;
        s_pb1[threadIdx.x + 1] = threadIdx.x < K ? (uint32_t)st->bb[threadIdx.x] : 0xFFFFFFFFu;
        if (threadIdx.x == 0) s_pb1[0] = 0xFFFFFFFFu;
    }
    for (uint32_t i = threadIdx.x; i < K * CH_SD; i += LEAN_MT) s_sd[i] = 0;
    __syncthreads();
    constexpr uint32_t NWV = LEAN_MT / 64;
    const uint32_t nw = gridDim.x * NWV;
    const uint32_t Tl = min(A.T, st->tlive);
    for (uint32_t t = blockIdx.x * NWV + wave_id(); t < A.T; t += nw)
    {
        uint4 rv[MJ], hv;
        chain_slot_load(A, t, rv, hv);
        merge_chain_wave<true>(s_out[wave_id()], s_sd, t, A, s_pa, s_pb, s_pb1, K, z0, (uint32_t)CH_RSTRIDE, rv, hv, nullptr, 0, Tl);
    }
    __syncthreads();
    const uint32_t vc = A.vcap & 0xFFFFFFu;
    const uint32_t lim = min(vc, (uint32_t)CH_DCAP);
    for (uint32_t p = 0; p < K; p++) {
        const uint32_t *sd = s_sd + p * CH_SD;
        uint32_t *g = A.delta + delta_rep_off(p * (uint32_t)CH_RSTRIDE + (blockIdx.x & (brep - 1u)), vc);
        for (uint32_t i = threadIdx.x; i < lim; i += LEAN_MT) {
            const uint32_t l = sd[i], r = sd[CH_DCAP + i];
            if (l) atomicAdd(&g[i], l);
            if (r) atomicAdd(&g[vc + i], r);
        }
        if (threadIdx.x == 0) {
            const uint32_t adj = sd[2 * CH_DCAP], rem = sd[2 * CH_DCAP + 1];
            if (adj) atomicAdd(&st->badj[p], adj);
            if (rem && A.removed) atomicAdd(&A.removed[(p * (uint32_t)CH_RMV + (blockIdx.x & (uint32_t)(CH_RMV - 1))) * REMOVED_STRIDE], rem);
        }
    }
}
__global__ void __launch_bounds__(MT, 5)
k_merge_chain_dense1(AbArgs A) {
    __shared__ __attribute__((aligned(16))) uint32_t s_out[MT / 64][TILE2];
    __shared__ uint32_t s_delta[2 * LDSD_CAP + 2];
    const DevState *st = A.st;
    if (st->status || st->defer || st->bk != 1) return;
    const uint32_t a = (uint32_t)st->ba[0], b = (uint32_t)st->bb[0];
    A.newid = st->bz0;
    ldsd_clear(s_delta);
    const uint32_t nw = gridDim.x * (MT / 64);
    const uint32_t Tl = min(A.T, st->tlive);
    for (uint32_t t = blockIdx.x * (MT / 64) + wave_id(); t < A.T; t += nw)
        merge_ab_wave<false, false, true>(s_out[wave_id()], s_delta, t, A, a, b, Tl);
    ldsd_flush(s_delta, A);
}

template <bool OWNED>
__device__ __forceinline__ void apply_chain_tokens(const uint32_t t, uint32_t *__restrict__ mat, uint32_t stride,
                                                   uint32_t *__restrict__ delta, uint32_t vcap, const uint32_t *__restrict__ rowmax,
                                                   uint32_t *__restrict__ dbits, uint4 *__restrict__ sums,
                                                   const uint32_t *__restrict__ folded, uint32_t fS, const uint32_t *__restrict__ ftail,
                                                   const uint32_t K, const uint32_t z0, const uint32_t ran,
                                                   const uint32_t *pairs, const uint32_t *adjs, const uint32_t brep_in) {
    auto dld = [&](const uint32_t *p) -> uint32_t { return OWNED ? ld_agent(p) : *p; };
    auto pair_a = [&](uint32_t p) -> uint32_t { return pairs[p] >> 16; };
    auto pair_b = [&](uint32_t p) -> uint32_t { return pairs[p] & 0xFFFFu; };
    {
        const uint32_t Zlast = z0 + K - 1u;
        if ((t & ~255u) > Zlast) return;
        const bool live = t <= Zlast;
        const uint32_t nrep = 1u << (vcap >> 24);
        const uint32_t vc = vcap & 0xFFFFFFu;
        uint2 rm = make_uint2(0u, 0u);
        uint32_t prevflag = 0, oldword = 0;
        if (OWNED) {
            oldword = ran ? 0u : dbits[t >> 5];
            prevflag = (oldword >> (t & 31)) & 1u;
            if (live) {
                const unsigned long long v = ld_agent64(reinterpret_cast<const unsigned long long *>(rowmax) + t);
                rm = make_uint2((uint32_t)v, (uint32_t)(v >> 32));
            }
        } else if (live) {
            prevflag = (dbits[t >> 5] >> (t & 31)) & 1u;
            rm = reinterpret_cast<const uint2 *>(rowmax)[t];
        }
        bool flagged = false;
        if (K == 1) {
            const uint32_t a = pair_a(0), b = pair_b(0), Z = z0;
            const uint32_t adj = folded ? ftail[0] : adjs[0];
            constexpr int RB = OWNED ? 8 : 16;
            uint32_t x[RB][2];
            auto load_batch = [&](uint32_t r0) {
#pragma unroll
                for (int k = 0; k < RB; k++) {
                    const uint32_t r = r0 + k;
                    x[k][0] = (live && r < nrep) ? dld(&delta[delta_rep_off(r, vc) + t]) : 0u;
                    x[k][1] = (live && r < nrep) ? dld(&delta[delta_rep_off(r, vc) + vc + t]) : 0u;
                }
            };
            if (!folded) load_batch(0);
            const uint32_t old_ta = live ? mat[(size_t)t * stride + a] : 0u;
            uint32_t sl = 0, sr = 0;
            if (folded) {
                sl = live ? folded[t] : 0u;
                sr = live ? folded[(size_t)fS + t] : 0u;
            }
            for (uint32_t r0 = 0; !folded;) {
#pragma unroll
                for (int k = 0; k < RB; k++) {
                    if (x[k][0]) delta[delta_rep_off(r0 + k, vc) + t] = 0;
                    if (x[k][1]) delta[delta_rep_off(r0 + k, vc) + vc + t] = 0;
                    sl += x[k][0];
                    sr += x[k][1];
                }
                r0 += RB;
                if (r0 >= nrep) break;
                load_batch(r0);
            }
            const uint32_t dr = sr + (t == a ? adj : 0u), ir = sr + (t == Z ? adj : 0u);
            if (sl) {
                atomicSub(&mat[(size_t)t * stride + a], sl);
                atomicAdd(&mat[(size_t)t * stride + Z], sl);
                flagged |= old_ta == rm.x;
            }
            if (dr) atomicSub(&mat[(size_t)b * stride + t], dr);
            if (ir) atomicAdd(&mat[(size_t)Z * stride + t], ir);
            if (live && t == b) mat[(size_t)a * stride + b] = 0;
            flagged |= live && ((t == a) | (t == b) | (t == Z));
        } else {
            const uint32_t brep = folded ? 0u : brep_in;
            constexpr int G = OWNED ? 4 : 8;
            for (uint32_t g = 0; g < K; g += G) {
                uint32_t x[G][CH_REP][2];
                if (brep == (uint32_t)CH_REP) {
#pragma unroll
                    for (int q = 0; q < G; q++) {
#pragma unroll
                        for (int r = 0; r < CH_REP; r++) {
                            const size_t o = delta_rep_off((g + (uint32_t)q) * (uint32_t)CH_RSTRIDE + (uint32_t)r, vc);
                            x[q][r][0] = (live && g + (uint32_t)q < K) ? dld(&delta[o + t]) : 0u;
                            x[q][r][1] = (live && g + (uint32_t)q < K) ? dld(&delta[o + vc + t]) : 0u;
                        }
                    }
                }
#pragma unroll
                for (int q = 0; q < G; q++) {
                    const uint32_t p = g + (uint32_t)q;
                    if (p >= K) break;
                    const uint32_t a = pair_a(p), b = pair_b(p), Z = z0 + p;
                    const uint32_t adj = folded ? ftail[p] : adjs[p];
                    uint32_t sl = 0, sr = 0;
                    if (folded) {
                        sl = live ? folded[(size_t)(2 * p) * fS + t] : 0u;
                        sr = live ? folded[(size_t)(2 * p + 1) * fS + t] : 0u;
                    } else if (brep == (uint32_t)CH_REP) {
#pragma unroll
                        for (int r = 0; r < CH_REP; r++) {
                            const size_t o = delta_rep_off(p * (uint32_t)CH_RSTRIDE + (uint32_t)r, vc);
                            if (x[q][r][0]) delta[o + t] = 0;
                            if (x[q][r][1]) delta[o + vc + t] = 0;
                            sl += x[q][r][0];
                            sr += x[q][r][1];
                        }
                    } else {
                        constexpr int YB = OWNED ? CH_RSTRIDE / 2 : CH_RSTRIDE;
#pragma unroll
                        for (int r0 = 0; r0 < CH_RSTRIDE; r0 += YB) {
                            uint32_t y[YB][2];
#pragma unroll
                            for (int r = 0; r < YB; r++) {
                                const size_t o = delta_rep_off(p * (uint32_t)CH_RSTRIDE + (uint32_t)(r0 + r), vc);
                                y[r][0] = live ? dld(&delta[o + t]) : 0u;
                                y[r][1] = live ? dld(&delta[o + vc + t]) : 0u;
                            }
#pragma unroll
                            for (int r = 0; r < YB; r++) {
                                const size_t o = delta_rep_off(p * (uint32_t)CH_RSTRIDE + (uint32_t)(r0 + r), vc);
                                if (y[r][0]) delta[o + t] = 0;
                                if (y[r][1]) delta[o + vc + t] = 0;
                                sl += y[r][0];
                                sr += y[r][1];
                            }
                        }
                    }
                    const uint32_t dr = sr + (t == a ? adj : 0u), ir = sr + (t == Z ? adj : 0u);
                    if (sl) {
                        const uint32_t old = atomicSub(&mat[(size_t)t * stride + a], sl);
                        atomicAdd(&mat[(size_t)t * stride + Z], sl);
                        flagged |= old == rm.x;
                    }
                    if (dr) atomicSub(&mat[(size_t)b * stride + t], dr);
                    if (ir) atomicAdd(&mat[(size_t)Z * stride + t], ir);
                    if (live && t == b) mat[(size_t)a * stride + b] = 0;
                    flagged |= live && ((t == a) | (t == b) | (t == Z));
                }
            }
        }
        if (OWNED) {
            const unsigned long long fb = __ballot(flagged);
            const uint32_t mine = (lane_id() < 32) ? (uint32_t)fb : (uint32_t)(fb >> 32);
            const uint32_t neww = oldword | mine;
            if ((lane_id() & 31) == 0 && (ran || neww != oldword)) dbits[t >> 5] = neww;
        } else if (flagged && !prevflag) {
            atomicOr(&dbits[t >> 5], 1u << (t & 31));
        }
        const uint32_t vs = (!live || flagged || prevflag) ? 0u : rm.x;
        const uint32_t gw = t >> 6, base = gw * 64u;
        const int lane = lane_id();
        const uint32_t m = wave_umax_dpp(vs);
        const unsigned long long bal = __ballot(m != 0 && vs == m);
        const int fl = bal ? __ffsll((long long)bal) - 1 : 0;
        const uint32_t arg = (uint32_t)__shfl((int)rm.y, fl);
        if (lane == 0) sums[gw] = make_uint4(m, base + (uint32_t)fl, arg, (uint32_t)__popcll(bal));
    }
}
__device__ __forceinline__ void apply_chain_records(DevState *st, int par, IterRec *rec, StepRec *srec, uint32_t step,
                                                    uint32_t *__restrict__ removed, const uint32_t K, const bool noop,
                                                    const uint32_t status, const uint32_t defer, const uint32_t remote) {
    {
        uint32_t v = 0;
        if (removed) {
#pragma unroll
            for (int i = 0; i < 4; i++) {
                const uint32_t x = ld_agent(&removed[(threadIdx.x * 4 + i) * REMOVED_STRIDE]);
                if (x) removed[(threadIdx.x * 4 + i) * REMOVED_STRIDE] = 0;
                v += x;
            }
        }
        static_assert(CH_RMV == 16, "lanes 4p .. 4p + 3 hold the removals of pair p");
        v += (uint32_t)__shfl_xor((int)v, 1);
        v += (uint32_t)__shfl_xor((int)v, 2);
        uint32_t rem[CH_KMAX];
#pragma unroll
        for (int p = 0; p < CH_KMAX; p++) rem[p] = (uint32_t)__shfl((int)v, 4 * p);
        if (K == 1) {
            uint32_t tot = 0;
#pragma unroll
            for (int p = 0; p < CH_KMAX; p++) tot += rem[p];
            rem[0] = tot;
        }
        if (!removed) {
#pragma unroll
            for (int p = 0; p < CH_KMAX; p++) rem[p] = st->bcnt[p];
        }
        if (threadIdx.x == 0) {
            const unsigned long long n = st->n[par];
            unsigned long long nn = n;
            const uint32_t iter = st->iter;
            const uint32_t mode_used = st->sel_mode;
            uint32_t k_done = 0;
            if (!noop) {
                for (uint32_t p = 0; p < K; p++) {
                    nn -= rem[p];
                    iter_rec_put(rec + iter + p, st->ba[p], st->bb[p], st->bcnt[p], ST_OK, nn);
                }
                k_done = K;
                st->iter = iter + K;
                st->sel_mode = (st->tl_n > st->tl_skip) ? CH_LIST : CH_FULL;
            } else if (status == 0 && !defer) {
                st->sel_mode = CH_FULL;
            }
            if (status == 0) st->n[par ^ 1] = nn;
            if (remote && st->status == 0) st->status = ST_INTERNAL;
            st->removed = 0;
            st->pool_hint = st->pool_hint_next;
            StepRec *sr = srec + (step % STEP_RING);
            step_rec_put(sr, iter, k_done, (status == 0 && defer) ? (uint32_t)ST_DEFER : status, mode_used | (defer << 8), nn);
            __builtin_amdgcn_s_waitcnt(0);
            for (uint32_t p = 0; p < k_done; p++) iter_rec_seal(rec + iter + p, (unsigned long long)(iter + p) + 1);
            step_rec_seal(sr, (unsigned long long)step + 1);
        }
    }
}
template <bool THROUGH = false>
__device__ __forceinline__ void apply_chain_commit(uint32_t first, uint32_t stp, uint32_t nwords, uint32_t *__restrict__ smask,
                                                   const StageRec *__restrict__ stage, SlotHdr *__restrict__ hdr_cur) {
    for (uint32_t w = first; w < nwords; w += stp) {
        uint32_t m = THROUGH ? ld_agent(&smask[w]) : smask[w];
        if (!m) continue;
        smask[w] = 0;
        while (m) {
            uint32_t tt[4], h[4][8];
#pragma unroll
            for (int i = 0; i < 4; i++) {
                tt[i] = m ? w * 32 + (uint32_t)__ffs((int)m) - 1u : 0xFFFFFFFFu;
                m &= m - 1u;
                if (tt[i] != 0xFFFFFFFFu) stage_get<THROUGH>(stage + tt[i], h[i]);
            }
#pragma unroll
            for (int i = 0; i < 4; i++) {
                if (tt[i] == 0xFFFFFFFFu) continue;
                uint4 *dst = reinterpret_cast<uint4 *>(hdr_cur + tt[i]);
                dst[0] = make_uint4(h[i][0], h[i][1], h[i][2], h[i][3]);
                dst[1] = make_uint4(h[i][4], h[i][5], h[i][6], h[i][7]);
            }
        }
    }
}
__global__ void __launch_bounds__(256)
k_apply_chain(uint32_t *__restrict__ mat, uint32_t stride, uint32_t *__restrict__ delta, uint32_t vcap,
              const uint32_t *__restrict__ rowmax, DevState *st, uint32_t *__restrict__ dbits, int par, IterRec *rec,
              StepRec *srec, uint32_t step, uint32_t na, SlotHdr *__restrict__ hdr_cur, const StageRec *__restrict__ stage,
              uint32_t *__restrict__ removed, uint32_t *__restrict__ smask, uint32_t nwords, uint4 *__restrict__ sums,
              const uint32_t *__restrict__ folded, uint32_t fS, const uint32_t *__restrict__ ftail) {
    __shared__ uint32_t s_w[64], s_pairs[CH_KMAX];
    step_words_fetch(st, s_w);
    const uint32_t remote = (folded && ftail[16] != 0) ? 1u : 0u;
    const uint32_t status = s_w[SW_STATUS] ? s_w[SW_STATUS] : (remote ? ST_INTERNAL : 0u), defer = s_w[SW_DEFER];
    const uint32_t K = s_w[SW_BK], z0 = s_w[SW_BZ0];
    const bool noop = status || defer || K == 0;
    if (blockIdx.x < na) {
        if (noop) return;
        if (threadIdx.x < CH_KMAX) s_pairs[threadIdx.x] = (s_w[threadIdx.x] << 16) | (s_w[16 + threadIdx.x] & 0xFFFFu);
        if (threadIdx.x == 0 && K == 1) s_w[32] = s_w[SW_ADJ];
        __syncthreads();
        apply_chain_tokens<false>(blockIdx.x * 256u + threadIdx.x, mat, stride, delta, vcap, rowmax, dbits, sums, folded, fS,
                                  ftail, K, z0, 0u, s_pairs, s_w + 32, s_w[SW_BREP]);
        return;
    }
    if (blockIdx.x == na && threadIdx.x < 64) apply_chain_records(st, par, rec, srec, step, removed, K, noop, status, defer, remote);
    if (noop) return;
    apply_chain_commit((blockIdx.x - na) * blockDim.x + threadIdx.x, (gridDim.x - na) * blockDim.x, nwords, smask, stage, hdr_cur);
}

__global__ void __launch_bounds__(256)
k_dp_fold_chain(uint32_t *__restrict__ delta, uint32_t dl, const DevState *__restrict__ st, uint32_t *__restrict__ folded,
                uint32_t S, uint32_t *__restrict__ tail) {
    const uint32_t status = st->status, K = st->bk, z0 = st->bz0;
    const bool noop = status || st->defer || K == 0;
    const uint32_t t = blockIdx.x * 256u + threadIdx.x;
    if (t < 32) tail[t] = t == 16 ? (status ? 1u : 0u) : ((!noop && t < K && t < 16) ? (K == 1 ? st->adj : st->badj[t]) : 0u);
#ifdef BPE_DP_DEBUG
    if (t >= 32 && t < 64) {
        uint32_t v = 0;
        if (t == 32) v = st->iter;
        else if (t == 33) v = st->sel_mode;
        else if (t == 34) v = K;
        else if (t == 35) v = st->tl_n;
        else if (t == 36) v = st->tl_M;
        else if (t == 37) v = st->tl_skip;
        else if (t == 38) v = st->defer;
        else if (t == 39) v = st->gap;
        else if (t < 48) v = (uint32_t)st->ba[t - 40] << 16 | (uint32_t)st->bb[t - 40];
        else v = (uint32_t)st->chain[2 * (t - 48)] << 16 | (uint32_t)st->chain[2 * (t - 48) + 1];
        tail[t] = v;
    }
#endif
    if (noop || t > z0 + K - 1u || t >= S) return;
    const uint32_t nrep = 1u << (dl >> 24), vc = dl & 0xFFFFFFu;
    if (K == 1) {
        uint32_t sl = 0, sr = 0;
        for (uint32_t r = 0; r < nrep; r++) {
            const size_t o = delta_rep_off(r, vc);
            const uint32_t x = delta[o + t], y = delta[o + vc + t];
            if (x) delta[o + t] = 0;
            if (y) delta[o + vc + t] = 0;
            sl += x;
            sr += y;
        }
        folded[t] = sl;
        folded[(size_t)S + t] = sr;
        return;
    }
    const uint32_t brep = st->brep;
    for (uint32_t p = 0; p < K; p++) {
        uint32_t x[CH_RSTRIDE][2];
#pragma unroll
        for (int r = 0; r < CH_RSTRIDE; r++) {
            const size_t o = delta_rep_off(p * (uint32_t)CH_RSTRIDE + (uint32_t)r, vc);
            x[r][0] = (uint32_t)r < brep ? delta[o + t] : 0u;
            x[r][1] = (uint32_t)r < brep ? delta[o + vc + t] : 0u;
        }
        uint32_t sl = 0, sr = 0;
#pragma unroll
        for (int r = 0; r < CH_RSTRIDE; r++) {
            const size_t o = delta_rep_off(p * (uint32_t)CH_RSTRIDE + (uint32_t)r, vc);
            if (x[r][0]) delta[o + t] = 0;
            if (x[r][1]) delta[o + vc + t] = 0;
            sl += x[r][0];
            sr += x[r][1];
        }
        folded[(size_t)(2 * p) * S + t] = sl;
        folded[(size_t)(2 * p + 1) * S + t] = sr;
    }
}
__global__ void k_dp_after_sum(DevState *st, const uint32_t *__restrict__ tail) {
    if (tail[8] != 0 && st->status == 0) st->status = ST_INTERNAL;
}

__global__ void __launch_bounds__(64)
k_forced_sel(DevState *st, const int32_t *__restrict__ pairs, const uint32_t *__restrict__ mat, uint32_t stride, uint32_t kcap) {
    const uint32_t lane = threadIdx.x;
    const uint32_t status = st->status, defer = st->defer, iter = st->iter, nm = st->num_merges;
    if (status || defer) return;
    if (iter >= nm) {
        if (lane == 0) st->bk = 0;
        return;
    }
    const uint32_t r = iter + lane;
    const bool in = lane < kcap && r < nm;
    const uint32_t a = in ? (uint32_t)pairs[2 * r] : 0xFFFFFFFEu, b = in ? (uint32_t)pairs[2 * r + 1] : 0xFFFFFFFDu;
    uint32_t bad = in ? ((a == b) | (a >= 256u + iter) | (b >= 256u + iter)) : 1u;
#pragma unroll
    for (int j = 0; j < CH_KSWEEP - 1; j++) {
        const uint32_t aj = (uint32_t)__shfl((int)a, j), bj = (uint32_t)__shfl((int)b, j);
        if ((uint32_t)j < lane) bad |= (aj == a) | (aj == b) | (bj == a) | (bj == b);
    }
    const unsigned long long bb = __ballot(bad != 0);
    const uint32_t K = bb ? min(kcap, (uint32_t)__ffsll((long long)bb) - 1u) : kcap;
    const uint32_t c = lane < K ? mat[(size_t)a * stride + b] : 0u;
    const uint32_t cmax = wave_umax_dpp(c);
    __shared__ uint32_t s_pa[CH_KMAX];
    if (lane < CH_KMAX) s_pa[lane] = a;
    __syncthreads();
    const uint32_t hm = chain_hash_find(s_pa, K);
    if (lane == 0) {
        st_agent(&st->adj, 0u);
        st->count = c;
        st->ntied = 1;
        st->firstpos = NOPOS;
        st->sel_tie = 0;
        st->a = (int32_t)a;
        st->b = (int32_t)b;
        st->fin_a = (int32_t)a;
        st->fin_b = (int32_t)b;
        st->bk = K;
        st->bz0 = 256u + iter;
        st->tl_n = st->tl_skip = 0;
        st->dp_wait = 0;
        st->sel_mode = CH_LIST;
        st->found = K ? 1u : 0u;
        if (K == 0) st->defer = 1;
        st->brep = cmax > CH_REP_COUNT ? (uint32_t)CH_RSTRIDE : (uint32_t)CH_REP;
        st->bhm = hm;
        st->bhm_key = ((256u + iter) << 8) | K;
        st->pool_n = 0;
    }
    if (lane < K) {
        st->ba[lane] = (int32_t)a;
        st->bb[lane] = (int32_t)b;
        st_agent(&st->badj[lane], 0u);
        st->bcnt[lane] = c;
    }
}
__global__ void k_forced_pair(DevState *st, const int32_t *__restrict__ pairs, uint32_t iter, const uint32_t *__restrict__ mat,
                              uint32_t stride) {
    if (threadIdx.x != 0 || blockIdx.x != 0) return;
    st->adj = 0;
    st->chain_n = 0;
    if (st->status) return;
    const int32_t a = pairs[2 * iter], b = pairs[2 * iter + 1];
    st->a = a;
    st->b = b;
    st->fin_a = a;
    st->fin_b = b;
    st->count = mat[(size_t)(uint32_t)a * stride + (uint32_t)b];
    st->ntied = 1;
    st->firstpos = NOPOS;
    st->sel_tie = 0;
    st->found = 1;
    st->ncand = 0;
}

__global__ void k_set_iter(DevState *st, uint32_t iter, uint32_t num_merges) {
    st->iter = iter;
    st->num_merges = num_merges;
    st->sel_mode = CH_FULL;
    st->tl_n = st->tl_skip = 0;
    st->bk = 0;
    st->scan_a = st->scan_b = st->scan_z = NOROW;
    st->chain_n = 0;
    st->dp_wait = 0;
    st->pool_n = 0;
    st->pool_hint = st->pool_hint_next = 1;
    st->pool_epoch = 0;
}
__global__ void k_clear_defer_chain(DevState *st) {
    st->defer = 0;
    st->chain_n = 0;
    st->sel_mode = CH_FULL;
    st->tl_n = st->tl_skip = 0;
    st->bk = 0;
    st->dp_wait = 0;
    st->pool_n = 0;
    st->pool_hint = st->pool_hint_next = 1;
}

}
}
```

minbpe_amd/csrc/kernels/k_pool.hip:

```cpp
#include <hip/hip_runtime.h>
#include <stdint.h>

#include "../bpe_device.h"

namespace bpe {
namespace BPE_G {

constexpr uint32_t PL_CAP = 256;
constexpr uint32_t PL_ROWS = 128;
constexpr uint32_t PL_GATHER = 1024;
static_assert(PL_GATHER >= 4 * PL_CAP, "maintain: four variants per entry");
constexpr uint32_t PL_REQ_WORDS = 2 + PL_ROWS + 256;

struct PoolScratch {
    uint32_t dl[PL_CAP];
    uint32_t rank[PL_GATHER];
    uint32_t w[8];
    uint32_t wtot[PL_CAP / 64];
    uint32_t fv, nl, k;
};
__device__ __forceinline__ void pool_sort(const uint32_t *ixy, const uint32_t *ic, const unsigned long long *ikey,
                                          uint32_t *oxy, uint32_t *oc, unsigned long long *okey, uint32_t n, PoolScratch &X) {
    const uint32_t tid = threadIdx.x;
    uint32_t sh = 0;
    while (sh < 4 && (n << (sh + 1)) <= blockDim.x) sh++;
    const uint32_t tpe = 1u << sh, e = tid >> sh, q = tid & (tpe - 1u);
    if (tid < n) X.rank[tid] = 0;
    __syncthreads();
    if (e < n) {
        const uint32_t c = ic[e], x = ixy[e];
        uint32_t r = 0;
#pragma unroll 4
        for (uint32_t j = q; j < n; j += tpe) {
            const uint32_t cj = ic[j];
            r += (cj > c) | ((cj == c) & (ixy[j] < x));
        }
        if (r) atomicAdd(&X.rank[e], r);
    }
    __syncthreads();
    if (tid < n) {
        const uint32_t r = X.rank[tid];
        oxy[r] = ixy[tid];
        oc[r] = ic[tid];
        okey[r] = ikey[tid];
    }
    __syncthreads();
}
constexpr int PL_KSH = 40, PL_KSH_DP = 43, PL_POS_DP = 33;
__device__ __forceinline__ void pool_level_bounds(const uint32_t *c, uint32_t n, uint32_t *ls, uint32_t *le, PoolScratch &X) {
    const uint32_t tid = threadIdx.x, w = (uint32_t)wave_id(), lane = (uint32_t)lane_id();
    const bool in = tid < n;
    const bool start = in && (tid == 0 || c[tid - 1] != c[tid]);
    const unsigned long long bal = __ballot(start);
    if (tid < PL_CAP && lane == 0) {
        X.w[w] = bal ? w * 64u + 63u - (uint32_t)__clzll((long long)bal) : 0xFFFFFFFFu;
        X.w[4 + w] = bal ? w * 64u + (uint32_t)__ffsll((long long)bal) - 1u : 0xFFFFFFFFu;
    }
    __syncthreads();
    if (in) {
        const unsigned long long upto = lane == 63 ? ~0ull : ((2ull << lane) - 1ull);
        const unsigned long long below = bal & upto, above = bal & ~upto;
        uint32_t lo = 0, hi = n;
        if (below) {
            lo = w * 64u + 63u - (uint32_t)__clzll((long long)below);
        } else {
            for (int v = (int)w - 1; v >= 0; v--)
                if (X.w[v] != 0xFFFFFFFFu) {
                    lo = X.w[v];
                    break;
                }
        }
        if (above) {
            hi = w * 64u + (uint32_t)__ffsll((long long)above) - 1u;
        } else {
            for (uint32_t v = w + 1; v < PL_CAP / 64; v++)
                if (X.w[4 + v] != 0xFFFFFFFFu) {
                    hi = X.w[4 + v];
                    break;
                }
        }
        ls[tid] = lo;
        le[tid] = hi;
    }
    __syncthreads();
}
__device__ __forceinline__ void pool_levels_dirty(const unsigned long long *key, uint32_t n, const uint32_t *ls, const uint32_t *le,
                                                  uint32_t *dirty, int ksh, PoolScratch &X) {
    const uint32_t tid = threadIdx.x;
    if (tid < n) X.dl[tid] = 0;
    __syncthreads();
    if (tid < n) {
        const uint32_t lo = ls[tid], hi = le[tid];
        const unsigned long long e0 = key[lo] >> ksh;
        if (hi - lo > 1 && (e0 == 0 || (key[tid] >> ksh) != e0)) X.dl[lo] = 1;
    }
    __syncthreads();
    if (tid < n) dirty[tid] = X.dl[ls[tid]];
    __syncthreads();
}
__device__ __forceinline__ void pool_finish(DevState *st, PoolEnt *__restrict__ pool, const uint32_t *b_xy, const uint32_t *b_c,
                                            const unsigned long long *b_key, uint32_t *a_xy, uint32_t *a_c,
                                            unsigned long long *a_key, const uint32_t *s_ls, const uint32_t *s_le,
                                            uint32_t *s_dirty, uint32_t *s_clash, uint32_t *s_k, uint32_t *s_unt, uint32_t n,
                                            uint32_t kmax, uint32_t iter, uint32_t theta, unsigned long long epoch, bool rebuilt,
                                            uint32_t hint_below, int ksh, PoolScratch &X) {
    const uint32_t tid = threadIdx.x;
    const uint32_t nwalk = min(n, kmax);
    const uint32_t sh = blockDim.x >= 4 * PL_CAP ? 2u : 0u;
    const uint32_t tpe = 1u << sh, e = tid >> sh, q = tid & (tpe - 1u);
    if (tid < n) {
        X.rank[tid] = 0;
        X.dl[tid] = 0;
    }
    if (tid == 0) *s_unt = 0;
    __syncthreads();
    if (e < n) {
        const uint32_t lo = s_ls[e], hi = s_le[e];
        const unsigned long long k = b_key[e];
        uint32_t r = 0;
#pragma unroll 4
        for (uint32_t j = lo + q; j < hi; j += tpe) {
            const unsigned long long kj = b_key[j];
            r += (kj < k) | ((kj == k) & (j < e));
        }
        if (r) atomicAdd(&X.rank[e], r);
        if (q == 0) {
            const unsigned long long e0 = b_key[lo] >> ksh;
            if (hi - lo > 1 && (e0 == 0 || (k >> ksh) != e0)) X.dl[lo] = 1;
        }
    }
    __syncthreads();
    if (tid < n) {
        const uint32_t lo = s_ls[tid];
        const uint32_t r = lo + X.rank[tid];
        a_xy[r] = b_xy[tid];
        a_c[r] = b_c[tid];
        a_key[r] = b_key[tid];
        s_dirty[r] = X.dl[lo];
    }
    __syncthreads();
    if (tid < 64) {
        uint32_t bad = 0;
        if (tid < nwalk) {
            const uint32_t x = a_xy[tid] >> 16, y = a_xy[tid] & 0xFFFFu;
            bad = (x == y) | s_dirty[tid];
#pragma unroll
            for (uint32_t j = 0; j < (uint32_t)CH_KSWEEP - 1u; j++) {
                if (j < tid) {
                    const uint32_t xj = a_xy[j] >> 16, yj = a_xy[j] & 0xFFFFu;
                    bad |= (xj == x) | (xj == y) | (yj == x);
                }
            }
        }
        const unsigned long long bb = __ballot(bad != 0);
        if (tid == 0) *s_k = bb ? min(nwalk, (uint32_t)__ffsll((long long)bb) - 1u) : nwalk;
    }
    __syncthreads();
    const uint32_t K = *s_k;
    if (tid == 0) {
        st_agent(&st->adj, 0u);
        st->count = a_c[0];
        st->ntied = s_le[0];
        st->firstpos = NOPOS;
        st->sel_tie = 0;
        st->a = (int32_t)(a_xy[0] >> 16);
        st->b = (int32_t)(a_xy[0] & 0xFFFFu);
        st->fin_a = (int32_t)(a_xy[0] >> 16);
        st->fin_b = (int32_t)(a_xy[0] & 0xFFFFu);
        st->bk = K;
        st->bz0 = 256u + iter;
        st->tl_n = st->tl_skip = 0;
        st->dp_wait = 0;
        st->sel_mode = rebuilt ? CH_FULL : CH_LIST;
        if (K == 0) {
            st->found = 0;
            st->defer = ((a_xy[0] >> 16) == (a_xy[0] & 0xFFFFu) && !s_dirty[0]) ? 1u : 2u;
            st->pool_n = 0;
            st->pool_hint_next = 1;
        } else {
            st->found = 1;
        }
    }
    if (K == 0) return;
    if (tid < K) X.rank[tid] = a_xy[tid] >> 16;
    __syncthreads();
    if (tid < 64) {
        uint32_t c = 0;
        if (tid < K) {
            c = a_c[tid];
            st->ba[tid] = (int32_t)(a_xy[tid] >> 16);
            st->bb[tid] = (int32_t)(a_xy[tid] & 0xFFFFu);
            st_agent(&st->badj[tid], 0u);
            st->bcnt[tid] = c;
        }
        const uint32_t cmax = wave_umax_dpp(c);
        const uint32_t hm = chain_hash_find(reinterpret_cast<const uint32_t *>(X.rank), K);
        if (tid == 0) {
            st->brep = cmax > CH_REP_COUNT ? (uint32_t)CH_RSTRIDE : (uint32_t)CH_REP;
            st->bhm = hm;
            st->bhm_key = ((256u + iter) << 8) | K;
        }
    }
    bool unt = false;
    if (tid >= K && tid < n) {
        PoolEnt e2;
        e2.xy = a_xy[tid];
        e2.c = a_c[tid];
        e2.key = a_key[tid];
        pool[tid - K] = e2;
        const uint32_t x = e2.xy >> 16, y = e2.xy & 0xFFFFu;
        bool touched = false;
#pragma unroll
        for (uint32_t p = 0; p < (uint32_t)CH_KSWEEP; p++)
            if (p < K) touched |= ((a_xy[p] & 0xFFFFu) == x) | ((a_xy[p] >> 16) == y);
        unt = !touched;
    }
    if (tid < PL_CAP) {
        const unsigned long long ub = __ballot(unt);
        if (lane_id() == 0 && ub) atomicAdd(s_unt, (uint32_t)__popcll(ub));
    }
    __syncthreads();
    if (tid == 0) {
        st->pool_n = n - K;
        st->pool_theta = theta;
        st->pool_epoch = epoch;
        st->pool_hint_next = *s_unt < hint_below ? 1u : 0u;
    }
}

struct PoolLds {
    unsigned long long s_red[32];
    uint32_t s_words[DBITS_WORDS], s_pref[DBITS_WORDS + 1];
    uint32_t s_exrow[CH_EX_CAP], s_exm[CH_EX_CAP], s_exarg[CH_EX_CAP];
    uint32_t a_xy[PL_GATHER], a_c[PL_GATHER], b_xy[PL_GATHER], b_c[PL_GATHER];
    unsigned long long a_key[PL_GATHER], b_key[PL_GATHER];
    uint32_t s_ls[PL_CAP], s_le[PL_CAP], s_dirty[PL_CAP], s_clash[PL_CAP];
    int32_t s_tied[2 * TIE_CAP];
    unsigned long long s_pos[TIE_CAP];
    uint32_t s_lidx[TIE_CAP];
    uint32_t s_rows[PL_ROWS], s_cnt[8], s_r16[16], s_wtot[PL_CAP / 64];
    uint32_t s_fail, s_n, s_theta, s_nrows, s_nl, s_reach, s_k, s_unt, s_x;
    PoolScratch X;
    uint32_t s_sw[64];
};
__device__ __forceinline__ void
pool_sel_body(uint32_t *__restrict__ rowmax, uint32_t *__restrict__ mat, uint32_t stride, DevState *st, const SlotRefH &ref,
              const CandArgs &C, uint32_t *__restrict__ dbits, unsigned long long *__restrict__ res, uint32_t tag,
              unsigned long long *__restrict__ req, uint32_t kcap, PoolEnt *__restrict__ pool, uint32_t *__restrict__ gather,
              uint32_t hint_below, long long *__restrict__ dpkey, unsigned long long dprank, PoolEnt *__restrict__ mid,
              PoolLds &L, const uint32_t blk, const uint32_t nblk, unsigned long long *dbg = nullptr) {
    auto dstamp = [&](int i) {
        if (dbg && threadIdx.x == 0 && blk == 0) dbg[i] = wall_clock64();
    };
    auto &s_red = L.s_red;
    auto &s_words = L.s_words;
    auto &s_pref = L.s_pref;
    auto &s_exrow = L.s_exrow;
    auto &s_exm = L.s_exm;
    auto &s_exarg = L.s_exarg;
    auto &a_xy = L.a_xy;
    auto &a_c = L.a_c;
    auto &b_xy = L.b_xy;
    auto &b_c = L.b_c;
    auto &a_key = L.a_key;
    auto &b_key = L.b_key;
    auto &s_ls = L.s_ls;
    auto &s_le = L.s_le;
    auto &s_dirty = L.s_dirty;
    auto &s_clash = L.s_clash;
    auto &s_tied = L.s_tied;
    auto &s_pos = L.s_pos;
    auto &s_lidx = L.s_lidx;
    auto &s_rows = L.s_rows;
    auto &s_cnt = L.s_cnt;
    auto &s_r16 = L.s_r16;
    auto &s_wtot = L.s_wtot;
    uint32_t &s_fail = L.s_fail, &s_n = L.s_n, &s_theta = L.s_theta, &s_nrows = L.s_nrows, &s_nl = L.s_nl, &s_k = L.s_k, &s_reach = L.s_reach,
             &s_unt = L.s_unt, &s_x = L.s_x;
    const uint32_t tid = threadIdx.x;
    enum { PW_STATUS = 32, PW_DEFER, PW_GAP, PW_ITER, PW_NM, PW_HINT, PW_THETA, PW_POOLN, PW_BK, PW_BZ0, PW_EPOCH_LO, PW_EPOCH_HI, PW_N };
    PoolEnt my_ent;
    my_ent.xy = my_ent.c = 0;
    my_ent.key = 0;
    if (blk == 0 && tid < PL_CAP) my_ent = pool[tid];
    if (tid < (uint32_t)PW_N) {
        const uint32_t *base = reinterpret_cast<const uint32_t *>(st);
        uint32_t off;
        if (tid < 16) off = (uint32_t)offsetof(DevState, ba) / 4 + tid;
        else if (tid < 32) off = (uint32_t)offsetof(DevState, bb) / 4 + (tid - 16);
        else {
            constexpr uint32_t o[PW_N - 32] = {
                (uint32_t)offsetof(DevState, status) / 4,     (uint32_t)offsetof(DevState, defer) / 4,      (uint32_t)offsetof(DevState, gap) / 4,
                (uint32_t)offsetof(DevState, iter) / 4,       (uint32_t)offsetof(DevState, num_merges) / 4, (uint32_t)offsetof(DevState, pool_hint) / 4,
                (uint32_t)offsetof(DevState, pool_theta) / 4, (uint32_t)offsetof(DevState, pool_n) / 4,     (uint32_t)offsetof(DevState, bk) / 4,
                (uint32_t)offsetof(DevState, bz0) / 4,        (uint32_t)offsetof(DevState, pool_epoch) / 4, (uint32_t)offsetof(DevState, pool_epoch) / 4 + 1};
            off = o[0];
#pragma unroll
            for (int k = 1; k < PW_N - 32; k++) off = (tid == 32u + (uint32_t)k) ? o[k] : off;
        }
        L.s_sw[tid] = base[off];
    }
    __syncthreads();
    const uint32_t *s_sw = L.s_sw;
    const uint32_t status = s_sw[PW_STATUS], defer = s_sw[PW_DEFER], gap = s_sw[PW_GAP];
    const uint32_t iter = s_sw[PW_ITER], nm = s_sw[PW_NM], hint = s_sw[PW_HINT];
    if (dpkey && blk == 0 && tid < (uint32_t)DP_KEY_WORDS)
        dpkey[tid] = tid == 0 ? -(long long)status : (tid == 1 ? 0ll : 0x7FFFFFFFFFFFFFFFll);
    if (status || defer) return;
    if (iter >= nm) {
        if (blk == 0 && tid == 0) st->bk = 0;
        return;
    }
    const uint32_t vcur = 256u + iter;
    const DirtyView D{s_words, s_pref};
    if (blk != 0) {
        if (!hint) return;
        const uint32_t nd = dirty_view_build(dbits, D);
        if (nd) lean_scan_rows(mat, stride, rowmax, vcur, NOROW, NOROW, NOROW, D, 3 + nd, blk - 1, nblk - 1, res, tag,
                               true, s_red, 3);
        if (tid == 0) {
            uint32_t n = 0, th = 0;
            if (!granule_get(req, tag, n)) n = 0;
            if (n && !granule_get(req + 1 + PL_ROWS, tag, th)) n = 0;
            s_n = n;
            s_theta = th;
        }
        __syncthreads();
        const uint32_t n = s_n, theta = s_theta;
        if (blk - 1 >= n) return;
        for (uint32_t j = blk - 1; j < n; j += nblk - 1) {
            if (tid == 0) {
                uint32_t x = 0;
                s_x = granule_get(req + 1 + j, tag, x) ? x : 0xFFFFFFFFu;
            }
            __syncthreads();
            const uint32_t x = s_x;
            if (x != 0xFFFFFFFFu) {
                const uint32_t *row = mat + (size_t)x * stride;
                const uint32_t n4 = (vcur + 3) & ~3u;
                constexpr int U = 8;
                for (uint32_t base = 0; base < n4; base += U * 4096) {
                    uint4 q[U];
#pragma unroll
                    for (int u = 0; u < U; u++) {
                        const uint32_t y = base + ((uint32_t)u * 1024u + tid) * 4u;
                        q[u] = (y < n4) ? *reinterpret_cast<const uint4 *>(row + y) : make_uint4(0u, 0u, 0u, 0u);
                    }
#pragma unroll
                    for (int u = 0; u < U; u++) {
                        const uint32_t y = base + ((uint32_t)u * 1024u + tid) * 4u;
                        const uint32_t v[4] = {q[u].x, q[u].y, q[u].z, q[u].w};
#pragma unroll
                        for (int k = 0; k < 4; k++) {
                            if (v[k] >= theta && y + k < vcur) {
                                const uint32_t s = atomicAdd(&gather[0], 1u);
                                if (s < PL_GATHER) {
                                    __hip_atomic_store(&gather[2 + 2 * s], (x << 16) | (y + k), __ATOMIC_RELAXED, __HIP_MEMORY_SCOPE_AGENT);
                                    __hip_atomic_store(&gather[3 + 2 * s], v[k], __ATOMIC_RELAXED, __HIP_MEMORY_SCOPE_AGENT);
                                }
                            }
                        }
                    }
                }
            }
            __syncthreads();
        }
        __builtin_amdgcn_s_waitcnt(0);
        __syncthreads();
        if (tid == 0) granule_put(req + 2 + PL_ROWS + blk, tag, 1u);
        return;
    }
    auto dismiss = [&]() {
        if (hint && tid == 0) granule_put(req, tag, 0u);
    };
    uint32_t rm[SEL_RPT];
    if (hint) select_load(rowmax, vcur, rm);
    uint32_t theta = s_sw[PW_THETA];
    unsigned long long epoch = (unsigned long long)s_sw[PW_EPOCH_LO] | ((unsigned long long)s_sw[PW_EPOCH_HI] << 32);
    const uint32_t n0 = min(s_sw[PW_POOLN], PL_CAP);
    if (tid == 0) {
        s_fail = 0;
        s_nrows = 0;
        s_nl = 0;
        s_unt = 0;
    }
    if (tid < 8) s_cnt[tid] = 0;
    dstamp(8);
    uint32_t vx[4] = {0, 0, 0, 0}, vy[4] = {0, 0, 0, 0}, cv[4] = {0, 0, 0, 0}, keepm = 0, ec = 0;
    unsigned long long ekey = 0;
    uint32_t mxm = 0, nmulti = 0;
    bool multi = false;
    auto multi_variants = [&](auto &&emit) {
        const uint32_t zp = s_sw[PW_BZ0];
        const uint32_t x = vx[0], y = vy[0];
        const bool hy = vy[2] != y;
        for (uint32_t m = mxm | 0x80000000u; m; m &= m - 1u) {
            const uint32_t p = (uint32_t)__ffs((int)m) - 1u;
            const uint32_t lx = p == 31u ? x : zp + p;
            for (uint32_t r = 0; r < (hy ? 2u : 1u); r++) {
                const uint32_t ry = r ? vy[2] : y;
                const uint32_t c = mat[(size_t)lx * stride + ry];
                if (c >= theta) emit(lx, ry, c);
            }
        }
    };
    if (tid < n0) {
        const uint32_t Kp = min(s_sw[PW_BK], (uint32_t)CH_KMAX), zp = s_sw[PW_BZ0];
        const PoolEnt e = my_ent;
        const uint32_t x = e.xy >> 16, y = e.xy & 0xFFFFu;
        ec = e.c;
        ekey = e.key;
        int32_t zx = -1, zy = -1;
        for (uint32_t p = 0; p < Kp; p++) {
            if (s_sw[16 + p] == x) {
                zx = (int32_t)(zp + p);
                mxm |= 1u << p;
            }
            if (s_sw[p] == y) zy = (int32_t)(zp + p);
        }
        multi = (mxm & (mxm - 1u)) != 0;
        vx[0] = vx[2] = x;
        vx[1] = vx[3] = zx >= 0 ? (uint32_t)zx : x;
        vy[0] = vy[1] = y;
        vy[2] = vy[3] = zy >= 0 ? (uint32_t)zy : y;
        if (zx < 0 && zy < 0) {
            cv[0] = e.c;
            keepm = 1u;
        } else if (multi) {
            multi_variants([&](uint32_t, uint32_t, uint32_t) { nmulti++; });
        } else {
            const bool on[4] = {true, zx >= 0, zy >= 0, zx >= 0 && zy >= 0};
#pragma unroll
            for (int v = 0; v < 4; v++) cv[v] = on[v] ? mat[(size_t)vx[v] * stride + vy[v]] : 0u;
#pragma unroll
            for (int v = 0; v < 4; v++) keepm |= (on[v] && cv[v] >= theta) ? 1u << v : 0u;
        }
    }
    __syncthreads();
    {
        const uint32_t no = multi ? nmulti : (uint32_t)__popc(keepm);
        const uint32_t inc = wave_iscan_add(no);
        if (tid < PL_CAP && lane_id() == 63) s_wtot[wave_id()] = inc;
        __syncthreads();
        if (tid < PL_CAP) {
            uint32_t o = inc - no;
            for (int w = 0; w < wave_id(); w++) o += s_wtot[w];
            if (multi) {
                multi_variants([&](uint32_t lx, uint32_t ry, uint32_t c) {
                    if (o < PL_GATHER) {
                        a_xy[o] = (lx << 16) | ry;
                        a_c[o] = c;
                        a_key[o] = c == ec ? ekey : 0ull;
                    }
                    o++;
                });
            }
#pragma unroll
            for (int v = 0; v < 4; v++) {
                if ((keepm >> v) & 1u) {
                    if (o < PL_GATHER) {
                        a_xy[o] = (vx[v] << 16) | vy[v];
                        a_c[o] = cv[v];
                        a_key[o] = cv[v] == ec ? ekey : 0ull;
                    }
                    o++;
                }
            }
        }
        __syncthreads();
    }
    dstamp(9);
    uint32_t n1 = 0;
    if (n0) for (uint32_t w = 0; w < PL_CAP / 64; w++) n1 += s_wtot[w];
    if (n1 > PL_GATHER) n1 = 0;
    bool rebuilt = false;
    if (hint && n1 < min(kcap, nm - iter)) n1 = 0;
    if (n1 == 0) {
        if (!hint) {
            if (tid == 0) {
                st->bk = 0;
                st->found = 0;
                st->pool_n = 0;
                st->pool_hint_next = 1;
                st->sel_mode = CH_LIST;
                st->tl_n = st->tl_skip = 0;
            }
            return;
        }
        rebuilt = true;
        const uint32_t nd = dirty_view_build(dbits, D);
        if (tid == 0) st->sel_ran = 1;
        if (nd > CH_EX_CAP) {
            if (tid == 0) {
                st->found = 0;
                st->bk = 0;
                st->defer = 2;
            }
            dismiss();
            return;
        }
        for (uint32_t i = tid; i < nd; i += 1024) {
            const uint32_t x = dirty_view_row(D, i);
            uint32_t m = 0, arg = 0;
            const bool ok = granule_get(res + 2 * (size_t)i, tag, m) && granule_get(res + 2 * (size_t)i + 1, tag, arg);
            if (!ok) s_fail = 1;
            s_exrow[i] = x;
            s_exm[i] = m;
            s_exarg[i] = arg;
        }
        __syncthreads();
        if (s_fail) {
            if (tid == 0) atomicExch(&st->status, ST_LOOKBACK);
            dismiss();
            return;
        }
        const uint2 *__restrict__ rowma = reinterpret_cast<const uint2 *>(rowmax);
        auto stale = [&](uint32_t x) -> bool { return (s_words[x >> 5] >> (x & 31)) & 1u; };
        uint32_t m = 0;
#pragma unroll
        for (int i = 0; i < SEL_RPT; i++) {
            const uint32_t x = tid + 1024u * (uint32_t)i;
            if (x >= vcur || stale(x)) rm[i] = 0u;
            m = max(m, rm[i]);
        }
        for (uint32_t x = tid + 1024u * SEL_RPT; x < vcur; x += 1024)
            if (!stale(x)) m = max(m, rowma[x].x);
        for (uint32_t i = tid; i < nd; i += 1024) m = max(m, s_exm[i]);
        m = wave_umax_dpp(m);
        if (lane_id() == 0) s_r16[wave_id()] = m;
        __syncthreads();
        uint32_t M = 0;
#pragma unroll
        for (int w = 0; w < 16; w++) M = max(M, s_r16[w]);
        if (M == 0) {
            if (tid == 0) {
                st->status = ST_EMPTY;
                st->count = 0;
                st->found = 0;
                st->bk = 0;
                st->sel_tie = 0;
            }
            dismiss();
            return;
        }
        uint32_t th[8], cn[8];
#pragma unroll
        for (int k = 0; k < 8; k++) {
            th[k] = k < 7 ? M - (M >> (2 + k)) : M;
            cn[k] = 0;
        }
        auto tally = [&](uint32_t v) {
#pragma unroll
            for (int k = 0; k < 8; k++) cn[k] += v >= th[k];
        };
#pragma unroll
        for (int i = 0; i < SEL_RPT; i++) tally(rm[i]);
        for (uint32_t x = tid + 1024u * SEL_RPT; x < vcur; x += 1024)
            if (!stale(x)) tally(rowma[x].x);
        for (uint32_t i = tid; i < nd; i += 1024) tally(s_exm[i]);
#pragma unroll
        for (int k = 0; k < 8; k++) {
            const uint32_t s = wave_sum_u32(cn[k]);
            if (lane_id() == 0 && s) atomicAdd(&s_cnt[k], s);
        }
        __syncthreads();
        int ks = -1;
#pragma unroll
        for (int k = 7; k >= 0; k--)
            if (s_cnt[k] <= PL_ROWS) ks = k;
        if (ks < 0) {
            if (tid == 0) {
                st->count = M;
                st->found = 0;
                st->bk = 0;
                st->defer = 2;
            }
            dismiss();
            return;
        }
        theta = th[0];
#pragma unroll
        for (int k = 1; k < 8; k++) theta = (k == ks) ? th[k] : theta;
        if (ks == 0) theta = th[0];
        auto row_in = [&](uint32_t x, uint32_t v) {
            if (v >= theta) {
                const uint32_t s = atomicAdd(&s_nrows, 1u);
                if (s < PL_ROWS) s_rows[s] = x;
            }
        };
#pragma unroll
        for (int i = 0; i < SEL_RPT; i++) row_in(tid + 1024u * (uint32_t)i, rm[i]);
        for (uint32_t x = tid + 1024u * SEL_RPT; x < vcur; x += 1024)
            if (!stale(x)) row_in(x, rowma[x].x);
        for (uint32_t i = tid; i < nd; i += 1024) row_in(s_exrow[i], s_exm[i]);
        if (tid == 0) __hip_atomic_store(&gather[0], 0u, __ATOMIC_RELAXED, __HIP_MEMORY_SCOPE_AGENT);
        __builtin_amdgcn_s_waitcnt(0);
        __syncthreads();
        const uint32_t nrows = min(s_nrows, PL_ROWS);
        if (tid < nrows) granule_put(req + 1 + tid, tag, s_rows[tid]);
        if (tid == 0) {
            granule_put(req + 1 + PL_ROWS, tag, theta);
            granule_put(req, tag, nrows);
        }
        const uint32_t nh = min(nblk - 1, nrows);
        if (tid < nh) {
            uint32_t d = 0;
            if (!granule_get(req + 2 + PL_ROWS + (tid + 1), tag, d)) s_fail = 1;
        }
        __syncthreads();
        if (s_fail) {
            if (tid == 0) atomicExch(&st->status, ST_LOOKBACK);
            return;
        }
        const uint32_t ng = __hip_atomic_load(&gather[0], __ATOMIC_RELAXED, __HIP_MEMORY_SCOPE_AGENT);
        if (ng > PL_GATHER || ng == 0) {
            if (tid == 0) {
                st->count = M;
                st->found = 0;
                st->bk = 0;
                if (ng) st->defer = 2; else atomicExch(&st->status, ST_INTERNAL);
            }
            return;
        }
        if (tid < ng) {
            a_xy[tid] = __hip_atomic_load(&gather[2 + 2 * tid], __ATOMIC_RELAXED, __HIP_MEMORY_SCOPE_AGENT);
            a_c[tid] = __hip_atomic_load(&gather[3 + 2 * tid], __ATOMIC_RELAXED, __HIP_MEMORY_SCOPE_AGENT);
            a_key[tid] = 0ull;
        }
        n1 = ng;
        __syncthreads();
    } else {
        dismiss();
        if (hint && tid == 0) st->sel_ran = 1;
    }
    dstamp(10);
    pool_sort(a_xy, a_c, a_key, b_xy, b_c, b_key, n1, L.X);
    dstamp(11);
    uint32_t n = n1;
    if (n1 > PL_CAP) {
        if (tid == 0) {
            uint32_t cut = PL_CAP;
            while (cut > 0 && b_c[cut - 1] == b_c[cut]) cut--;
            s_n = cut;
        }
        __syncthreads();
        n = s_n;
        if (n == 0) {
            if (tid == 0) {
                st->count = b_c[0];
                st->found = 0;
                st->bk = 0;
                st->defer = 2;
                st->pool_n = 0;
                st->pool_hint_next = 1;
            }
            return;
        }
        theta = b_c[n] + 1;
        __syncthreads();
    }
    const uint32_t kmax = min(kcap, nm - iter);
    const uint32_t nwalk = min(n, kmax);
    const int ksh = dpkey ? PL_KSH_DP : PL_KSH;
    PoolScratch &X = L.X;
    pool_level_bounds(b_c, n, s_ls, s_le, X);
    pool_levels_dirty(b_key, n, s_ls, s_le, s_dirty, ksh, X);
    if (tid < 64) s_clash[tid] = 0;
    if (tid == 0) {
        X.fv = 0xFFFFFFFFu;
        X.nl = 0;
    }
    __syncthreads();
    if (tid < n) {
        const uint32_t x = b_xy[tid] >> 16, y = b_xy[tid] & 0xFFFFu;
#pragma unroll
        for (uint32_t i = 0; i < (uint32_t)CH_KSWEEP; i++) {
            if (i < nwalk) {
                const uint32_t xi = b_xy[i] >> 16, yi = b_xy[i] & 0xFFFFu;
                if (tid != i && tid < s_le[i] && ((xi == x) | (xi == y) | (yi == x))) s_clash[i] = 1;
            }
        }
        if (tid < nwalk && x == y) s_clash[tid] = 1;
    }
    __syncthreads();
    if (tid < 64) {
        const unsigned long long cb = __ballot(tid < nwalk && s_clash[tid] != 0);
        const uint32_t lim = cb ? (uint32_t)__ffsll((long long)cb) - 1u : nwalk - 1u;
        if (tid == 0) s_reach = s_le[lim];
    }
    __syncthreads();
    {
        const uint32_t reach = s_reach;
        const bool locate = dpkey || (C.T != 0 && gap == 0);
        const uint32_t scan_end = min(n, reach + 48u);
        const bool cons = locate && tid < n && s_ls[tid] < scan_end && s_dirty[tid] != 0;
        const uint32_t one = cons ? 1u : 0u;
        const uint32_t inc = wave_iscan_add(one);
        if (tid < PL_CAP && lane_id() == 63) X.wtot[wave_id()] = inc;
        __syncthreads();
        uint32_t P = inc - one;
        if (tid < PL_CAP)
            for (int v = 0; v < wave_id(); v++) P += X.wtot[v];
        if (cons && s_ls[tid] == tid) {
            const uint32_t size = s_le[tid] - tid;
            if ((tid >= reach && P + size > 16u) || P + size > (uint32_t)TIE_CAP) atomicMin(&X.fv, tid);
        }
        __syncthreads();
        const bool take = cons && s_ls[tid] < X.fv;
        if (take) {
            s_tied[2 * P] = (int32_t)(b_xy[tid] >> 16);
            s_tied[2 * P + 1] = (int32_t)(b_xy[tid] & 0xFFFFu);
            s_lidx[P] = tid;
        }
        if (tid < PL_CAP) {
            const unsigned long long tb = __ballot(take);
            if (lane_id() == 0 && tb) atomicAdd(&X.nl, (uint32_t)__popcll(tb));
        }
        __syncthreads();
        if (tid == 0) s_nl = X.nl;
        __syncthreads();
    }
    const uint32_t nl = s_nl;
    dstamp(12);
    if (dpkey) {
        const bool objection = nl != 0 && gap != 0;
        if (nl && !objection) (void)tie_by_index(ref, C, s_tied, nl, s_pos);
        __syncthreads();
        if (tid == 1 && objection) dpkey[1] = -1ll;
        if (tid < nl && !objection && s_pos[tid] != NOPOS)
            dpkey[2 + tid] = (long long)((dprank << PL_POS_DP) | (s_pos[tid] & ((1ull << PL_POS_DP) - 1ull)));
        if (tid < n) {
            PoolEnt e;
            e.xy = b_xy[tid];
            e.c = b_c[tid];
            e.key = b_key[tid];
            mid[1 + tid] = e;
        }
        if (tid < nl) mid[1 + PL_CAP + tid].xy = s_lidx[tid];
        if (tid == 0) {
            PoolEnt h;
            h.xy = n | (nl << 16);
            h.c = theta;
            h.key = epoch | ((unsigned long long)(rebuilt ? 1u : 0u) << 63);
            mid[0] = h;
            st->dp_wait = 1;
            st->bk = 0;
            st->found = 0;
        }
        return;
    }
    if (nl) {
        (void)tie_by_index(ref, C, s_tied, nl, s_pos);
        __syncthreads();
        epoch++;
        if (tid < nl) b_key[s_lidx[tid]] = s_pos[tid] != NOPOS ? (epoch << PL_KSH) | s_pos[tid] : 0ull;
        __syncthreads();
    }
    dstamp(13);
    pool_finish(st, pool, b_xy, b_c, b_key, a_xy, a_c, a_key, s_ls, s_le, s_dirty, s_clash, &s_k, &s_unt, n, kmax, iter, theta,
                epoch, rebuilt, hint_below, PL_KSH, X);
    dstamp(14);
}

__global__ void __launch_bounds__(1024)
k_pool_sel(uint32_t *__restrict__ rowmax, uint32_t *__restrict__ mat, uint32_t stride, DevState *st, SlotRefH ref,
           CandArgs C, uint32_t *__restrict__ dbits, unsigned long long *__restrict__ res, uint32_t tag,
           unsigned long long *__restrict__ req, uint32_t kcap, PoolEnt *__restrict__ pool, uint32_t *__restrict__ gather,
           uint32_t hint_below, long long *__restrict__ dpkey, unsigned long long dprank, PoolEnt *__restrict__ mid) {
    __shared__ PoolLds L;
    pool_sel_body(rowmax, mat, stride, st, ref, C, dbits, res, tag, req, kcap, pool, gather, hint_below, dpkey, dprank, mid, L,
                  blockIdx.x, gridDim.x);
}

__global__ void __launch_bounds__(PL_CAP)
k_pool_sel_dp(DevState *st, const long long *__restrict__ key, uint32_t kcap, PoolEnt *__restrict__ pool,
              const PoolEnt *__restrict__ mid, uint32_t hint_below) {
    __shared__ uint32_t a_xy[PL_CAP], a_c[PL_CAP], b_xy[PL_CAP], b_c[PL_CAP];
    __shared__ unsigned long long a_key[PL_CAP], b_key[PL_CAP];
    __shared__ uint32_t s_ls[PL_CAP], s_le[PL_CAP], s_dirty[PL_CAP], s_clash[PL_CAP];
    __shared__ uint32_t s_k, s_unt;
    __shared__ PoolScratch X;
    const uint32_t tid = threadIdx.x;
    const uint32_t status = st->status;
    if (key[0] < 0 && status == 0) {
        if (tid == 0) st->status = ST_INTERNAL;
        return;
    }
    if (status || st->defer || !st->dp_wait) return;
    const PoolEnt h = mid[0];
    const uint32_t n = h.xy & 0xFFFFu, nl = h.xy >> 16, theta = h.c;
    unsigned long long epoch = h.key & 0x7FFFFFFFFFFFFFFFull;
    const bool rebuilt = (h.key >> 63) != 0;
    const uint32_t iter = st->iter, nm = st->num_merges;
    if (tid < n) {
        const PoolEnt e = mid[1 + tid];
        b_xy[tid] = e.xy;
        b_c[tid] = e.c;
        b_key[tid] = e.key;
    }
    __syncthreads();
    if (nl) {
        epoch++;
        const bool objection = key[1] < 0;
        if (tid < nl) {
            const long long p = key[2 + tid];
            b_key[mid[1 + PL_CAP + tid].xy] =
                (!objection && p != 0x7FFFFFFFFFFFFFFFll) ? (epoch << PL_KSH_DP) | (unsigned long long)p : 0ull;
        }
        __syncthreads();
    }
    pool_level_bounds(b_c, n, s_ls, s_le, X);
    pool_finish(st, pool, b_xy, b_c, b_key, a_xy, a_c, a_key, s_ls, s_le, s_dirty, s_clash, &s_k, &s_unt, n, min(kcap, nm - iter),
                iter, theta, epoch, rebuilt, hint_below, PL_KSH_DP, X);
}

}
}
```

minbpe_amd/csrc/kernels/k_step.hip:

```cpp
#include <hip/hip_runtime.h>
#include <stdint.h>

#include "../bpe_device.h"

namespace bpe {
namespace BPE_G {

constexpr uint32_t STEP_PUB_WORDS = 32;
static_assert(2 + 2 * CH_KSWEEP == STEP_PUB_WORDS, "the line holds the pairs and their counts");

union StepLds {
    PoolLds p;
    MergeLds m;
};

__device__ __forceinline__ bool step_grid_barrier(uint32_t *ctr, uint32_t target, uint32_t *s_flag) {
    __builtin_amdgcn_s_waitcnt(0);
    __syncthreads();
    if (threadIdx.x == 0) {
        __hip_atomic_fetch_add(ctr, 1u, __ATOMIC_RELAXED, __HIP_MEMORY_SCOPE_AGENT);
        uint32_t ok = 0;
        for (uint32_t spins = 0; spins < LOOKBACK_SPINS; spins++) {
            if ((int32_t)(__hip_atomic_load(ctr, __ATOMIC_RELAXED, __HIP_MEMORY_SCOPE_AGENT) - target) >= 0) {
                ok = 1;
                break;
            }
            __builtin_amdgcn_s_sleep(1);
        }
        *s_flag = ok;
    }
    __syncthreads();
    return *s_flag != 0;
}

__global__ void __launch_bounds__(LEAN_MT)
k_step(StepArgs S) {
    __shared__ StepLds U;
    __shared__ uint32_t s_b[STEP_PUB_WORDS], s_adj[CH_KMAX];
    __shared__ uint32_t s_flag;
    DevState *st = S.st;
    const uint32_t tid = threadIdx.x;
    const int swho = blockIdx.x == 0 ? 0 : (blockIdx.x == S.gm / 2 ? 1 : (blockIdx.x == gridDim.x - 1 ? 2 : -1));
    auto stamp = [&](int i) {
        if (S.stamps && tid == 0 && swho >= 0) S.stamps[(((size_t)(S.step % STEP_STAMP_RING)) * 3 + (size_t)swho) * 16 + (size_t)i] = wall_clock64();
    };
    unsigned long long *const dbg = (S.stamps && swho >= 0) ? S.stamps + (((size_t)(S.step % STEP_STAMP_RING)) * 3 + (size_t)swho) * 16 : nullptr;
    stamp(0);
    if (blockIdx.x == 0) {
        pool_sel_body(S.rowmax, S.mat, S.stride, st, S.ref, S.C, S.dbits, S.res, S.tag, S.req, S.kcap, S.pool, S.gather,
                      S.hint_below, nullptr, 0ull, S.pool + PL_CAP, U.p, 0u, 1u + S.nscan, dbg);
        __builtin_amdgcn_s_waitcnt(0);
        __syncthreads();
        stamp(1);
        if (tid < STEP_PUB_WORDS) {
            const uint32_t status = st->status, defer = st->defer;
            const uint32_t noop = (status || defer) ? 1u : 0u;
            const uint32_t K = noop ? 0u : min(st->bk, (uint32_t)CH_KSWEEP);
            uint32_t v = 0;
            if (tid == 0)
                v = K | (st->brep << 8) | ((st->sel_ran ? 1u : 0u) << 16) | (noop << 17) | ((st->pool_hint_next ? 1u : 0u) << 18) |
                    ((defer & 3u) << 19) | ((st->sel_mode & 1u) << 21);
            else if (tid == 1) v = 256u + st->iter;
            else if (tid - 2 < K) v = ((uint32_t)st->ba[tid - 2] << 16) | ((uint32_t)st->bb[tid - 2] & 0xFFFFu);
            else if (tid >= 2 + CH_KSWEEP && tid - (2 + CH_KSWEEP) < K) v = st->bcnt[tid - (2 + CH_KSWEEP)];
            s_b[tid] = v;
            granule_put(S.pub + tid, S.tag, v);
        }
        if (tid == 0) s_flag = 1;
    } else {
        if (blockIdx.x <= S.nscan)
            pool_sel_body(S.rowmax, S.mat, S.stride, st, S.ref, S.C, S.dbits, S.res, S.tag, S.req, S.kcap, S.pool, S.gather,
                          S.hint_below, nullptr, 0ull, S.pool + PL_CAP, U.p, blockIdx.x, 1u + S.nscan);
        __syncthreads();
        if (tid == 0) s_flag = 1;
        __syncthreads();
        if (tid < STEP_PUB_WORDS) {
            uint32_t v = 0;
            if (!granule_get(S.pub + tid, S.tag, v)) s_flag = 0;
            s_b[tid] = v;
        }
    }
    __syncthreads();
    if (!s_flag) {
        if (tid == 0) atomicExch(&st->status, ST_LOOKBACK);
        if (tid < STEP_PUB_WORDS) s_b[tid] = tid == 0 ? (1u << 17) : 0u;
    }
    __syncthreads();
    stamp(2);
    if (S.stamps && tid == 0 && blockIdx.x < 256)
        S.stamps[(size_t)STEP_STAMP_RING * 3 * 16 + ((size_t)(S.step % STEP_STAMP_RING) * 256 + blockIdx.x) * 2] = wall_clock64();
    const uint32_t K = s_b[0] & 0xFFu, brep = (s_b[0] >> 8) & 0xFFu, ran = (s_b[0] >> 16) & 1u, z0 = s_b[1];
    const bool sel_noop = ((s_b[0] >> 17) & 1u) != 0 || K == 0;
    if (!sel_noop && blockIdx.x < S.gm) {
        MergeLds &L = U.m;
        if (tid < CH_KMAX) {
            const uint32_t w = tid < K ? s_b[2 + tid] : 0u;
            L.s_pa[tid] = tid < K ? (w >> 16) : 0xFFFFFFFFu;
            L.s_pb[tid] = tid < K ? (w & 0xFFFFu) : 0xFFFFFFFFu;
            L.s_pb1[tid + 1] = tid < K ? (w & 0xFFFFu) : 0xFFFFFFFFu;
            if (tid == 0) L.s_pb1[0] = 0xFFFFFFFFu;
        }
        __syncthreads();
        merge_chain_body<true>(S.A, S.idx_dirty, S.use_index, L, K, z0, brep, blockIdx.x, S.gm, blockIdx.x == 0 ? nullptr : dbg);
    }
    stamp(3);
    if (S.stamps && tid == 0 && blockIdx.x < 256) {
        unsigned long long *all = S.stamps + (size_t)STEP_STAMP_RING * 3 * 16 + ((size_t)(S.step % STEP_STAMP_RING) * 256 + blockIdx.x) * 2;
        all[1] = wall_clock64();
    }
    const bool arrived = step_grid_barrier(S.bar, S.bar_target, &s_flag);
    stamp(4);
    if (!arrived && tid == 0) atomicExch(&st->status, ST_LOOKBACK);
    const uint32_t status = arrived ? ld_agent(&st->status) : (uint32_t)ST_LOOKBACK;
    const bool noop = status || ((s_b[0] >> 19) & 3u) || K == 0;
    if (!noop) {
        const uint32_t nwv4 = (((z0 + K - 1u) >> 8) + 1u) * 4u;
        const uint32_t wpw = (nwv4 + gridDim.x - 1u) / gridDim.x;
        const uint32_t tw = blockIdx.x * wpw + (uint32_t)wave_id();
        if (tid < CH_KMAX) s_adj[tid] = K == 1 ? (tid == 0 ? ld_agent(&st->adj) : 0u) : (tid < K ? ld_agent(&st->badj[tid]) : 0u);
        __syncthreads();
        if ((uint32_t)wave_id() < wpw && tw < nwv4)
            apply_chain_tokens<true>(tw * 64u + (uint32_t)lane_id(), S.mat, S.stride, S.delta, S.dl, S.rowmax, S.dbits, S.sums,
                                     nullptr, 0u, nullptr, K, z0, ran, s_b + 2, s_adj, brep);
    } else if (ran && arrived) {
        for (uint32_t i = blockIdx.x * (uint32_t)LEAN_MT + tid; i < (uint32_t)DBITS_WORDS; i += gridDim.x * (uint32_t)LEAN_MT) S.dbits[i] = 0;
    }
    stamp(5);
    if ((blockIdx.x == 0 || blockIdx.x == gridDim.x - 1) && wave_id() == 0) {
        const uint32_t lane = (uint32_t)lane_id();
        const uint32_t defer2 = (s_b[0] >> 19) & 3u, mode_used = (s_b[0] >> 21) & 1u, hint_next = (s_b[0] >> 18) & 1u;
        uint32_t v = 0;
        if (S.removed) {
#pragma unroll
            for (int i = 0; i < 4; i++) v += ld_agent(&S.removed[(lane * 4 + i) * REMOVED_STRIDE]);
        }
        static_assert(CH_RMV == 16, "lanes 4p .. 4p + 3 hold the removals of pair p");
        v += (uint32_t)__shfl_xor((int)v, 1);
        v += (uint32_t)__shfl_xor((int)v, 2);
        uint32_t rem[CH_KMAX];
#pragma unroll
        for (int p = 0; p < CH_KMAX; p++) rem[p] = (uint32_t)__shfl((int)v, 4 * p);
        if (K == 1) {
            uint32_t tot = 0;
#pragma unroll
            for (int p = 0; p < CH_KMAX; p++) tot += rem[p];
            rem[0] = tot;
        }
        if (!S.removed) {
#pragma unroll
            for (int p = 0; p < CH_KMAX; p++) rem[p] = p < CH_KSWEEP ? s_b[2 + CH_KSWEEP + p] : 0u;
        }
        const uint32_t iter = z0 - 256u;
        unsigned long long nn = st->n[S.par];
        if (!noop)
            for (uint32_t p = 0; p < K; p++) nn -= rem[p];
        if (blockIdx.x == 0) {
            if (S.removed && lane < 64) {
#pragma unroll
                for (int i = 0; i < 4; i++) S.removed[(lane * 4 + i) * REMOVED_STRIDE] = 0;
            }
            if (lane == 0) {
                if (!noop) st->iter = iter + K;
                if (status == 0) st->n[S.par ^ 1] = nn;
                st->removed = 0;
                st->pool_hint = hint_next;
                if (arrived) st->sel_ran = 0;
            }
        }
        if (blockIdx.x == gridDim.x - 1 && lane == 0) {
            if (!noop) {
                unsigned long long m = st->n[S.par];
                for (uint32_t p = 0; p < K; p++) {
                    m -= rem[p];
                    iter_rec_put(S.rec + iter + p, (int32_t)(s_b[2 + p] >> 16), (int32_t)(s_b[2 + p] & 0xFFFFu), s_b[2 + CH_KSWEEP + p], ST_OK, m);
                }
                __builtin_amdgcn_s_waitcnt(0);
                for (uint32_t p = 0; p < K; p++) iter_rec_seal(S.rec + iter + p, (unsigned long long)(iter + p) + 1);
                __builtin_amdgcn_s_waitcnt(0);
            }
            StepRec *sr = S.srec + (S.step % STEP_RING);
            step_rec_put(sr, iter, noop ? 0u : K, (status == 0 && defer2) ? (uint32_t)ST_DEFER : status, mode_used | (defer2 << 8), nn);
            __builtin_amdgcn_s_waitcnt(0);
            step_rec_seal(sr, (unsigned long long)S.step + 1);
        }
    }
    stamp(6);
    if (noop) return;
    apply_chain_commit<true>(blockIdx.x * (uint32_t)LEAN_MT + tid, gridDim.x * (uint32_t)LEAN_MT, S.nwords, S.smask, S.stage, S.hdr_cur);
    stamp(7);
}

}
}
```

Baseline: 53200 merges/s.

## Widen merge batches to 31 pairs with byte-wide pair codes

Raises the maximum number of non-conflicting merges applied per batch from 15 to 31. Pair indices widen from nibble to byte codes in the chain kernel, so the match window becomes 64-bit, and the delta replica and removal-counter layouts are resized to fit. The hash-multiplier search now builds tables in LDS across two half-waves, and the conflict checks now loop over the batch. The fused step path stays capped at 15, so only the non-fused path gets larger batches, at the cost of more registers, more LDS and wider conflict checks.

```diff
diff --git a/minbpe_amd/csrc/api/api_ctx.hip b/minbpe_amd/csrc/api/api_ctx.hip
--- a/minbpe_amd/csrc/api/api_ctx.hip
+++ b/minbpe_amd/csrc/api/api_ctx.hip
@@ -1088,6 +1088,7 @@
     const DpComm *dp = c->dp_comm;
     uint32_t kcap = (uint32_t)(dense ? CH_KDENSE : std::min(CH_KSWEEP, c->chain_kcap));
     if (dp) kcap = std::min(kcap, (uint32_t)c->dp_kcap);
+    if (fused) kcap = std::min(kcap, (uint32_t)STEP_KCAP);
     const uint32_t hint_below = (uint32_t)(c->pool_hint > 0 ? c->pool_hint : (int)kcap);
     const unsigned nscan = (unsigned)std::max(1, std::min(c->chain_scan, c->num_cus - 1));
     if (fused) {
diff --git a/minbpe_amd/csrc/bpe_device.h b/minbpe_amd/csrc/bpe_device.h
--- a/minbpe_amd/csrc/bpe_device.h
+++ b/minbpe_amd/csrc/bpe_device.h
@@ -41,7 +41,7 @@
 constexpr uint32_t TIE_WINDOW0 = 0;
 constexpr int TIE_BLOCKS = 256;
 constexpr int ROW_BLOCKS = 64;
-constexpr int DELTA_REPL = 256;
+constexpr int DELTA_REPL = 512;
 constexpr int DELTA_SKEW = 64;
 constexpr int REMOVED_STRIDE = 64;
 constexpr int LDSD_CAP = 1920;
@@ -49,17 +49,18 @@
     return (size_t)r * (4 * (size_t)stride + DELTA_SKEW);
 }
 
-constexpr int CH_KMAX = 16;
-constexpr int CH_KSWEEP = 15;
+constexpr int CH_KMAX = 32;
+constexpr int CH_KSWEEP = 31;
 constexpr int CH_RSTRIDE = 16;
 constexpr uint32_t CH_REP_COUNT = 16384;
 constexpr int CH_REP = 4;
-constexpr int CH_RMV = 16;
-constexpr int DP_KCAP_MAX = CH_KSWEEP;
+constexpr int CH_RMV = 8;
+constexpr int DP_KCAP_MAX = 15;
 constexpr int DP_KCAP_DEFAULT = 8;
 static_assert(CH_KMAX * CH_RSTRIDE <= DELTA_REPL, "a batch's delta vectors must fit the replica blocks");
 static_assert(CH_KMAX * CH_RMV <= 256, "removal counters of a batch");
-static_assert(CH_KSWEEP < 16 && CH_KSWEEP <= CH_KMAX, "pair number + 1 must fit a nibble");
+static_assert(CH_KSWEEP < 32 && CH_KSWEEP < CH_KMAX, "pair number + 1 must fit a byte, and one bit per pair a word");
+static_assert(DP_KCAP_MAX < 16 && DP_KCAP_MAX <= CH_KSWEEP, "sharded steps: the payload's tail holds 16 adj words");
 constexpr uint32_t CH_FULL = 0, CH_LIST = 1;
 constexpr int DP_KEY_WORDS = TIE_CAP + 2;
 
diff --git a/minbpe_amd/csrc/kernels/k_chain.hip b/minbpe_amd/csrc/kernels/k_chain.hip
--- a/minbpe_amd/csrc/kernels/k_chain.hip
+++ b/minbpe_amd/csrc/kernels/k_chain.hip
@@ -108,12 +108,12 @@
         auto code = [&](uint32_t w) -> uint32_t {
             const uint32_t id = w & IDMASK;
             const uint32_t e = ph[(__umul24(id, hm) >> 8) & 255u];
-            return (e >> 8) == id ? (e & 15u) : 0u;
+            return (e >> 8) == id ? (e & 255u) : 0u;
         };
 #pragma unroll
         for (int j = 0; j < MJ; j++) {
 #pragma unroll
-            for (int k = 0; k < 4; k++) ia[j] |= code(x[j][k]) << (4 * k);
+            for (int k = 0; k < 4; k++) ia[j] |= code(x[j][k]) << (8 * k);
         }
         ip = code(prev1);
     } else {
@@ -122,7 +122,7 @@
 #pragma unroll
             for (int j = 0; j < MJ; j++) {
 #pragma unroll
-                for (int k = 0; k < 4; k++) ia[j] |= ((x[j][k] & IDMASK) == a) ? (p + 1u) << (4 * k) : 0u;
+                for (int k = 0; k < 4; k++) ia[j] |= ((x[j][k] & IDMASK) == a) ? (p + 1u) << (8 * k) : 0u;
             }
             ip = ((prev1 & IDMASK) == a) ? p + 1u : ip;
         }
@@ -134,10 +134,10 @@
 #pragma unroll
         for (int k = 0; k < 4; k++) {
             const uint32_t nxt = (k < 3) ? x[j][k + 1] : nxw;
-            const uint32_t i = (ia[j] >> (4 * k)) & 15u;
+            const uint32_t i = (ia[j] >> (8 * k)) & 255u;
             const uint32_t m = (uint32_t)((nxt & NWMASK) == pb1[i]);
             rb[j] |= m << k;
-            jc[j] |= (m ? i : 0u) << (4 * k);
+            jc[j] |= (m ? i : 0u) << (8 * k);
         }
     }
     s = (uint32_t)((prev1 != INVALID_WORD) & ((first & NWMASK) == pb1[ip]));
@@ -201,7 +201,7 @@
         for (int k = 0; k < 4; k++) {
             if ((kb[j] >> k) & 1u) {
                 const uint32_t w = x[j][k];
-                const uint32_t z = z0 + ((jc[j] >> (4 * k)) & 15u) - 1u;
+                const uint32_t z = z0 + ((jc[j] >> (8 * k)) & 255u) - 1u;
                 out[o++] = ((mb[j] >> k) & 1u) ? (z | (w & (FLAG | WMASK))) : w;
             }
         }
@@ -257,11 +257,11 @@
         W[4] = x[j][3];
         W[5] = lane_next(x[j][0], dn0);
         W[6] = lane_next(x[j][1], (j < MJ - 1) ? lane_first(x[(j + 1) % MJ][1]) : tail[1]);
-        const uint32_t lo_fill = (j > 0) ? ((lane_last(jc[(j + MJ - 1) % MJ]) >> 8) & 0xFFu) : (cm2 | (cm1 << 4));
-        const uint32_t hi_fill = (j < MJ - 1) ? (lane_first(jc[(j + 1) % MJ]) & 0xFFu) : (ct0 | (ct1 << 4));
-        const uint32_t lo = (uint32_t)dpp_mov<0x138>((int)lo_fill, (int)((jc[j] >> 8) & 0xFFu));
-        const uint32_t hi = lane_next(jc[j] & 0xFFu, hi_fill);
-        const uint32_t win = lo | (jc[j] << 8) | (hi << 24);
+        const uint32_t lo_fill = (j > 0) ? (lane_last(jc[(j + MJ - 1) % MJ]) >> 16) : (cm2 | (cm1 << 8));
+        const uint32_t hi_fill = (j < MJ - 1) ? (lane_first(jc[(j + 1) % MJ]) & 0xFFFFu) : (ct0 | (ct1 << 8));
+        const uint32_t lo = (uint32_t)dpp_mov<0x138>((int)lo_fill, (int)(jc[j] >> 16));
+        const uint32_t hi = lane_next(jc[j] & 0xFFFFu, hi_fill);
+        const unsigned long long win = (unsigned long long)lo | ((unsigned long long)jc[j] << 16) | ((unsigned long long)hi << 48);
         if (mb[j] == 0) continue;
         uint32_t todo = mb[j];
 #pragma unroll
@@ -270,9 +270,9 @@
             const uint32_t k = (uint32_t)__ffs((int)todo) - 1u;
             todo &= todo - 1u;
             const int q = j * 256 + lane * 4 + (int)k;
-            const uint32_t wk = win >> (4u * k);
-            const uint32_t p = ((wk >> 8) & 15u) - 1u;
-            const int li = (int)(wk & 15u) - 1, ri = (int)((wk >> 16) & 15u) - 1;
+            const unsigned long long wk = win >> (8u * k);
+            const uint32_t p = ((uint32_t)(wk >> 16) & 255u) - 1u;
+            const int li = (int)((uint32_t)wk & 255u) - 1, ri = (int)((uint32_t)(wk >> 32) & 255u) - 1;
             const uint32_t Z = z0 + p;
             uint32_t *dl, *dr;
             if (DENSE) {
@@ -317,18 +317,26 @@
     }
 }
 
-__device__ __forceinline__ uint32_t chain_hash_find(const uint32_t *pa, uint32_t K) {
+__device__ __forceinline__ uint32_t chain_hash_find(const uint32_t *pa, uint32_t K, uint32_t *tab) {
     if (K < 5) return 0u;
-    const uint32_t m = 129u + 2u * (uint32_t)lane_id();
-    bool ok = true;
-    for (uint32_t i = 1; i < K; i++) {
-        const uint32_t hi = (__umul24(pa[i], m) >> 8) & 255u;
-        for (uint32_t j = 0; j < i; j++) ok &= hi != ((__umul24(pa[j], m) >> 8) & 255u);
-    }
-    const unsigned long long bal = __ballot(ok);
-    return bal ? 129u + 2u * (uint32_t)(__ffsll((long long)bal) - 1) : 0u;
-}
-__device__ __forceinline__ uint32_t chain_hash_build(uint32_t *s_ph, uint32_t *s_hm, const uint32_t *s_pa, uint32_t K,
+    const uint32_t lane = (uint32_t)lane_id(), half = lane >> 5, l = lane & 31u;
+    const bool in = l < K;
+    const uint32_t a = in ? pa[l] : 0u;
+    volatile uint32_t *t = tab + half * 256u;
+    for (uint32_t m = 129u; m < 256u; m += 4u) {
+        const uint32_t h = (__umul24(a, m + 2u * half) >> 8) & 255u;
+        if (in) t[h] = l;
+        __builtin_amdgcn_fence(__ATOMIC_RELEASE, "wavefront");
+        __builtin_amdgcn_wave_barrier();
+        __builtin_amdgcn_fence(__ATOMIC_ACQUIRE, "wavefront");
+        const bool clash = in && t[h] != l;
+        const unsigned long long cb = __ballot(clash);
+        if ((uint32_t)cb == 0u) return m;
+        if ((uint32_t)(cb >> 32) == 0u) return m + 2u;
+    }
+    return 0u;
+}
+__device__ __forceinline__ uint32_t chain_hash_build(uint32_t *s_ph, uint32_t *s_hm, uint32_t *s_hs, const uint32_t *s_pa, uint32_t K,
                                                      bool pre_ok = false, uint32_t pre_hm = 0) {
     if (threadIdx.x < 256) s_ph[threadIdx.x] = 0xFFFFFFFFu;
     uint32_t hm = pre_hm;
@@ -336,7 +344,7 @@
         if (threadIdx.x == 0) *s_hm = 0;
         __syncthreads();
         if (wave_id() == 0) {
-            const uint32_t f = chain_hash_find(s_pa, K);
+            const uint32_t f = chain_hash_find(s_pa, K, s_hs);
             if (lane_id() == 0) *s_hm = f;
         }
         __syncthreads();
@@ -355,6 +363,7 @@
     uint32_t s_tot[2];
     uint32_t s_pa[CH_KMAX], s_pb[CH_KMAX], s_pb1[CH_KMAX + 1];
     uint32_t s_ph[256], s_hm;
+    uint32_t s_hs[512];
 };
 template <bool THROUGH = false>
 __device__ __forceinline__ void merge_chain_body(const AbArgs &A, const uint32_t *__restrict__ idx_dirty, uint32_t use_index,
@@ -372,7 +381,7 @@
     auto &s_pa = L.s_pa;
     auto &s_pb = L.s_pb;
     auto &s_pb1 = L.s_pb1;
-    const uint32_t hm = chain_hash_build(L.s_ph, &L.s_hm, s_pa, K, pre_ok, pre_hm);
+    const uint32_t hm = chain_hash_build(L.s_ph, &L.s_hm, L.s_hs, s_pa, K, pre_ok, pre_hm);
     const uint32_t *s_ph = L.s_ph;
     const uint32_t Tl = min(A.T, have_st ? tlive_in : st->tlive);
     const uint32_t gap = have_st ? gap_in : st->gap;
@@ -446,25 +455,26 @@
         __syncthreads();
     }
 }
-enum { SW_BK = 48, SW_BZ0, SW_BREP, SW_STATUS, SW_DEFER, SW_SEL_RAN, SW_TLIVE, SW_GAP, SW_BHM, SW_BHM_KEY, SW_ADJ, SW_N };
-static_assert(SW_N <= 64, "one wave fetches the state words");
+enum { SW_BB = CH_KMAX, SW_BADJ = 2 * CH_KMAX, SW_BK = 3 * CH_KMAX, SW_BZ0, SW_BREP, SW_STATUS, SW_DEFER, SW_SEL_RAN, SW_TLIVE, SW_GAP, SW_BHM, SW_BHM_KEY, SW_ADJ, SW_N };
+constexpr int SW_WORDS = 128;
+static_assert(SW_N <= SW_WORDS, "two waves fetch the state words");
 __device__ __forceinline__ void step_words_fetch(const DevState *st, uint32_t *s_w) {
     const uint32_t i = threadIdx.x;
     if (i < (uint32_t)SW_N) {
         const uint32_t *base = reinterpret_cast<const uint32_t *>(st);
         uint32_t off;
-        if (i < 16) off = (uint32_t)offsetof(DevState, ba) / 4 + i;
-        else if (i < 32) off = (uint32_t)offsetof(DevState, bb) / 4 + (i - 16);
-        else if (i < 48) off = (uint32_t)offsetof(DevState, badj) / 4 + (i - 32);
+        if (i < (uint32_t)SW_BB) off = (uint32_t)offsetof(DevState, ba) / 4 + i;
+        else if (i < (uint32_t)SW_BADJ) off = (uint32_t)offsetof(DevState, bb) / 4 + (i - (uint32_t)SW_BB);
+        else if (i < (uint32_t)SW_BK) off = (uint32_t)offsetof(DevState, badj) / 4 + (i - (uint32_t)SW_BADJ);
         else {
-            constexpr uint32_t o[SW_N - 48] = {
+            constexpr uint32_t o[SW_N - SW_BK] = {
                 (uint32_t)offsetof(DevState, bk) / 4,      (uint32_t)offsetof(DevState, bz0) / 4,     (uint32_t)offsetof(DevState, brep) / 4,
                 (uint32_t)offsetof(DevState, status) / 4,  (uint32_t)offsetof(DevState, defer) / 4,   (uint32_t)offsetof(DevState, sel_ran) / 4,
                 (uint32_t)offsetof(DevState, tlive) / 4,   (uint32_t)offsetof(DevState, gap) / 4,     (uint32_t)offsetof(DevState, bhm) / 4,
                 (uint32_t)offsetof(DevState, bhm_key) / 4, (uint32_t)offsetof(DevState, adj) / 4};
             off = o[0];
 #pragma unroll
-            for (int k = 1; k < SW_N - 48; k++) off = (i == 48u + (uint32_t)k) ? o[k] : off;
+            for (int k = 1; k < SW_N - SW_BK; k++) off = (i == (uint32_t)SW_BK + (uint32_t)k) ? o[k] : off;
         }
         s_w[i] = base[off];
     }
@@ -473,7 +483,7 @@
 __global__ void __launch_bounds__(LEAN_MT)
 k_merge_chain(AbArgs A, const uint32_t *__restrict__ idx_dirty, uint32_t use_index, uint32_t *__restrict__ dbits) {
     __shared__ MergeLds L;
-    __shared__ uint32_t s_w[64];
+    __shared__ uint32_t s_w[SW_WORDS];
     DevState *st = A.st;
     step_words_fetch(st, s_w);
     const uint32_t ran = s_w[SW_SEL_RAN];
@@ -487,8 +497,8 @@
     const uint32_t z0 = s_w[SW_BZ0], brep = s_w[SW_BREP];
     if (threadIdx.x < CH_KMAX) {
         L.s_pa[threadIdx.x] = threadIdx.x < K ? s_w[threadIdx.x] : 0xFFFFFFFFu;
-        L.s_pb[threadIdx.x] = threadIdx.x < K ? s_w[16 + threadIdx.x] : 0xFFFFFFFFu;
-        L.s_pb1[threadIdx.x + 1] = threadIdx.x < K ? s_w[16 + threadIdx.x] : 0xFFFFFFFFu;
+        L.s_pb[threadIdx.x] = threadIdx.x < K ? s_w[SW_BB + threadIdx.x] : 0xFFFFFFFFu;
+        L.s_pb1[threadIdx.x + 1] = threadIdx.x < K ? s_w[SW_BB + threadIdx.x] : 0xFFFFFFFFu;
         if (threadIdx.x == 0) L.s_pb1[0] = 0xFFFFFFFFu;
     }
     __syncthreads();
@@ -743,22 +753,17 @@
                 v += x;
             }
         }
-        static_assert(CH_RMV == 16, "lanes 4p .. 4p + 3 hold the removals of pair p");
+        static_assert(CH_RMV == 8 && 2 * CH_KMAX == 64, "lanes 2p, 2p + 1 hold the removals of pair p");
+        const uint32_t tot = wave_sum_u32(v);
         v += (uint32_t)__shfl_xor((int)v, 1);
-        v += (uint32_t)__shfl_xor((int)v, 2);
-        uint32_t rem[CH_KMAX];
-#pragma unroll
-        for (int p = 0; p < CH_KMAX; p++) rem[p] = (uint32_t)__shfl((int)v, 4 * p);
-        if (K == 1) {
-            uint32_t tot = 0;
-#pragma unroll
-            for (int p = 0; p < CH_KMAX; p++) tot += rem[p];
-            rem[0] = tot;
-        }
-        if (!removed) {
-#pragma unroll
-            for (int p = 0; p < CH_KMAX; p++) rem[p] = st->bcnt[p];
-        }
+        __shared__ uint32_t rem[CH_KMAX];
+        if (!(threadIdx.x & 1u)) {
+            const uint32_t p = threadIdx.x >> 1;
+            rem[p] = removed ? ((K == 1 && p == 0) ? tot : v) : st->bcnt[p];
+        }
+        __builtin_amdgcn_fence(__ATOMIC_RELEASE, "wavefront");
+        __builtin_amdgcn_wave_barrier();
+        __builtin_amdgcn_fence(__ATOMIC_ACQUIRE, "wavefront");
         if (threadIdx.x == 0) {
             const unsigned long long n = st->n[par];
             unsigned long long nn = n;
@@ -819,7 +824,7 @@
               StepRec *srec, uint32_t step, uint32_t na, SlotHdr *__restrict__ hdr_cur, const StageRec *__restrict__ stage,
               uint32_t *__restrict__ removed, uint32_t *__restrict__ smask, uint32_t nwords, uint4 *__restrict__ sums,
               const uint32_t *__restrict__ folded, uint32_t fS, const uint32_t *__restrict__ ftail) {
-    __shared__ uint32_t s_w[64], s_pairs[CH_KMAX];
+    __shared__ uint32_t s_w[SW_WORDS], s_pairs[CH_KMAX];
     step_words_fetch(st, s_w);
     const uint32_t remote = (folded && ftail[16] != 0) ? 1u : 0u;
     const uint32_t status = s_w[SW_STATUS] ? s_w[SW_STATUS] : (remote ? ST_INTERNAL : 0u), defer = s_w[SW_DEFER];
@@ -827,11 +832,11 @@
     const bool noop = status || defer || K == 0;
     if (blockIdx.x < na) {
         if (noop) return;
-        if (threadIdx.x < CH_KMAX) s_pairs[threadIdx.x] = (s_w[threadIdx.x] << 16) | (s_w[16 + threadIdx.x] & 0xFFFFu);
-        if (threadIdx.x == 0 && K == 1) s_w[32] = s_w[SW_ADJ];
+        if (threadIdx.x < CH_KMAX) s_pairs[threadIdx.x] = (s_w[threadIdx.x] << 16) | (s_w[SW_BB + threadIdx.x] & 0xFFFFu);
+        if (threadIdx.x == 0 && K == 1) s_w[SW_BADJ] = s_w[SW_ADJ];
         __syncthreads();
         apply_chain_tokens<false>(blockIdx.x * 256u + threadIdx.x, mat, stride, delta, vcap, rowmax, dbits, sums, folded, fS,
-                                  ftail, K, z0, 0u, s_pairs, s_w + 32, s_w[SW_BREP]);
+                                  ftail, K, z0, 0u, s_pairs, s_w + SW_BADJ, s_w[SW_BREP]);
         return;
     }
     if (blockIdx.x == na && threadIdx.x < 64) apply_chain_records(st, par, rec, srec, step, removed, K, noop, status, defer, remote);
@@ -926,10 +931,10 @@
     const uint32_t K = bb ? min(kcap, (uint32_t)__ffsll((long long)bb) - 1u) : kcap;
     const uint32_t c = lane < K ? mat[(size_t)a * stride + b] : 0u;
     const uint32_t cmax = wave_umax_dpp(c);
-    __shared__ uint32_t s_pa[CH_KMAX];
+    __shared__ uint32_t s_pa[CH_KMAX], s_hs[512];
     if (lane < CH_KMAX) s_pa[lane] = a;
     __syncthreads();
-    const uint32_t hm = chain_hash_find(s_pa, K);
+    const uint32_t hm = chain_hash_find(s_pa, K, s_hs);
     if (lane == 0) {
         st_agent(&st->adj, 0u);
         st->count = c;
diff --git a/minbpe_amd/csrc/kernels/k_pool.hip b/minbpe_amd/csrc/kernels/k_pool.hip
--- a/minbpe_amd/csrc/kernels/k_pool.hip
+++ b/minbpe_amd/csrc/kernels/k_pool.hip
@@ -18,6 +18,7 @@
     uint32_t w[8];
     uint32_t wtot[PL_CAP / 64];
     uint32_t fv, nl, k;
+    uint32_t bad;
 };
 __device__ __forceinline__ void pool_sort(const uint32_t *ixy, const uint32_t *ic, const unsigned long long *ikey,
                                           uint32_t *oxy, uint32_t *oc, unsigned long long *okey, uint32_t n, PoolScratch &X) {
@@ -112,7 +113,10 @@
         X.rank[tid] = 0;
         X.dl[tid] = 0;
     }
-    if (tid == 0) *s_unt = 0;
+    if (tid == 0) {
+        *s_unt = 0;
+        X.bad = 0;
+    }
     __syncthreads();
     if (e < n) {
         const uint32_t lo = s_ls[e], hi = s_le[e];
@@ -139,22 +143,20 @@
         s_dirty[r] = X.dl[lo];
     }
     __syncthreads();
-    if (tid < 64) {
-        uint32_t bad = 0;
-        if (tid < nwalk) {
-            const uint32_t x = a_xy[tid] >> 16, y = a_xy[tid] & 0xFFFFu;
-            bad = (x == y) | s_dirty[tid];
-#pragma unroll
-            for (uint32_t j = 0; j < (uint32_t)CH_KSWEEP - 1u; j++) {
-                if (j < tid) {
-                    const uint32_t xj = a_xy[j] >> 16, yj = a_xy[j] & 0xFFFFu;
-                    bad |= (xj == x) | (xj == y) | (yj == x);
-                }
-            }
-        }
-        const unsigned long long bb = __ballot(bad != 0);
-        if (tid == 0) *s_k = bb ? min(nwalk, (uint32_t)__ffsll((long long)bb) - 1u) : nwalk;
-    }
+    for (uint32_t q2 = tid; q2 < 32u * nwalk; q2 += blockDim.x) {
+        const uint32_t i = q2 >> 5, j = q2 & 31u;
+        const uint32_t x = a_xy[i] >> 16, y = a_xy[i] & 0xFFFFu;
+        bool bad = false;
+        if (j == i) {
+            bad = (x == y) | (s_dirty[i] != 0);
+        } else if (j < i) {
+            const uint32_t xj = a_xy[j] >> 16, yj = a_xy[j] & 0xFFFFu;
+            bad = (xj == x) | (xj == y) | (yj == x);
+        }
+        if (bad) atomicOr(&X.bad, 1u << i);
+    }
+    __syncthreads();
+    if (tid == 0) *s_k = X.bad ? min(nwalk, (uint32_t)__ffs((int)X.bad) - 1u) : nwalk;
     __syncthreads();
     const uint32_t K = *s_k;
     if (tid == 0) {
@@ -194,7 +196,7 @@
             st->bcnt[tid] = c;
         }
         const uint32_t cmax = wave_umax_dpp(c);
-        const uint32_t hm = chain_hash_find(reinterpret_cast<const uint32_t *>(X.rank), K);
+        const uint32_t hm = chain_hash_find(reinterpret_cast<const uint32_t *>(X.rank), K, X.rank + 256);
         if (tid == 0) {
             st->brep = cmax > CH_REP_COUNT ? (uint32_t)CH_RSTRIDE : (uint32_t)CH_REP;
             st->bhm = hm;
@@ -210,9 +212,8 @@
         pool[tid - K] = e2;
         const uint32_t x = e2.xy >> 16, y = e2.xy & 0xFFFFu;
         bool touched = false;
-#pragma unroll
-        for (uint32_t p = 0; p < (uint32_t)CH_KSWEEP; p++)
-            if (p < K) touched |= ((a_xy[p] & 0xFFFFu) == x) | ((a_xy[p] >> 16) == y);
+#pragma unroll 4
+        for (uint32_t p = 0; p < K; p++) touched |= ((a_xy[p] & 0xFFFFu) == x) | ((a_xy[p] >> 16) == y);
         unt = !touched;
     }
     if (tid < PL_CAP) {
@@ -241,7 +242,7 @@
     uint32_t s_rows[PL_ROWS], s_cnt[8], s_r16[16], s_wtot[PL_CAP / 64];
     uint32_t s_fail, s_n, s_theta, s_nrows, s_nl, s_reach, s_k, s_unt, s_x;
     PoolScratch X;
-    uint32_t s_sw[64];
+    uint32_t s_sw[3 * CH_KMAX];
 };
 __device__ __forceinline__ void
 pool_sel_body(uint32_t *__restrict__ rowmax, uint32_t *__restrict__ mat, uint32_t stride, DevState *st, const SlotRefH &ref,
@@ -278,7 +279,7 @@
     uint32_t &s_fail = L.s_fail, &s_n = L.s_n, &s_theta = L.s_theta, &s_nrows = L.s_nrows, &s_nl = L.s_nl, &s_k = L.s_k, &s_reach = L.s_reach,
              &s_unt = L.s_unt, &s_x = L.s_x;
     const uint32_t tid = threadIdx.x;
-    enum { PW_STATUS = 32, PW_DEFER, PW_GAP, PW_ITER, PW_NM, PW_HINT, PW_THETA, PW_POOLN, PW_BK, PW_BZ0, PW_EPOCH_LO, PW_EPOCH_HI, PW_N };
+    enum { PW_BB = CH_KMAX, PW_STATUS = 2 * CH_KMAX, PW_DEFER, PW_GAP, PW_ITER, PW_NM, PW_HINT, PW_THETA, PW_POOLN, PW_BK, PW_BZ0, PW_EPOCH_LO, PW_EPOCH_HI, PW_N };
     PoolEnt my_ent;
     my_ent.xy = my_ent.c = 0;
     my_ent.key = 0;
@@ -286,17 +287,18 @@
     if (tid < (uint32_t)PW_N) {
         const uint32_t *base = reinterpret_cast<const uint32_t *>(st);
         uint32_t off;
-        if (tid < 16) off = (uint32_t)offsetof(DevState, ba) / 4 + tid;
-        else if (tid < 32) off = (uint32_t)offsetof(DevState, bb) / 4 + (tid - 16);
+        if (tid < (uint32_t)PW_BB) off = (uint32_t)offsetof(DevState, ba) / 4 + tid;
+        else if (tid < (uint32_t)PW_STATUS) off = (uint32_t)offsetof(DevState, bb) / 4 + (tid - (uint32_t)PW_BB);
         else {
-            constexpr uint32_t o[PW_N - 32] = {
+            static_assert(PW_N <= 3 * CH_KMAX, "s_sw");
+            constexpr uint32_t o[PW_N - PW_STATUS] = {
                 (uint32_t)offsetof(DevState, status) / 4,     (uint32_t)offsetof(DevState, defer) / 4,      (uint32_t)offsetof(DevState, gap) / 4,
                 (uint32_t)offsetof(DevState, iter) / 4,       (uint32_t)offsetof(DevState, num_merges) / 4, (uint32_t)offsetof(DevState, pool_hint) / 4,
                 (uint32_t)offsetof(DevState, pool_theta) / 4, (uint32_t)offsetof(DevState, pool_n) / 4,     (uint32_t)offsetof(DevState, bk) / 4,
                 (uint32_t)offsetof(DevState, bz0) / 4,        (uint32_t)offsetof(DevState, pool_epoch) / 4, (uint32_t)offsetof(DevState, pool_epoch) / 4 + 1};
             off = o[0];
 #pragma unroll
-            for (int k = 1; k < PW_N - 32; k++) off = (tid == 32u + (uint32_t)k) ? o[k] : off;
+            for (int k = 1; k < PW_N - PW_STATUS; k++) off = (tid == (uint32_t)PW_STATUS + (uint32_t)k) ? o[k] : off;
         }
         L.s_sw[tid] = base[off];
     }
@@ -412,7 +414,7 @@
         ekey = e.key;
         int32_t zx = -1, zy = -1;
         for (uint32_t p = 0; p < Kp; p++) {
-            if (s_sw[16 + p] == x) {
+            if (s_sw[PW_BB + p] == x) {
                 zx = (int32_t)(zp + p);
                 mxm |= 1u << p;
             }
@@ -671,16 +673,16 @@
         X.nl = 0;
     }
     __syncthreads();
-    if (tid < n) {
-        const uint32_t x = b_xy[tid] >> 16, y = b_xy[tid] & 0xFFFFu;
-#pragma unroll
-        for (uint32_t i = 0; i < (uint32_t)CH_KSWEEP; i++) {
-            if (i < nwalk) {
+    {
+        const uint32_t t = tid & (PL_CAP - 1u);
+        if (t < n) {
+            const uint32_t x = b_xy[t] >> 16, y = b_xy[t] & 0xFFFFu;
+            for (uint32_t i = tid / PL_CAP; i < nwalk; i += blockDim.x / PL_CAP) {
                 const uint32_t xi = b_xy[i] >> 16, yi = b_xy[i] & 0xFFFFu;
-                if (tid != i && tid < s_le[i] && ((xi == x) | (xi == y) | (yi == x))) s_clash[i] = 1;
-            }
-        }
-        if (tid < nwalk && x == y) s_clash[tid] = 1;
+                if (t != i && t < s_le[i] && ((xi == x) | (xi == y) | (yi == x))) s_clash[i] = 1;
+            }
+            if (tid < nwalk && x == y) s_clash[tid] = 1;
+        }
     }
     __syncthreads();
     if (tid < 64) {
diff --git a/minbpe_amd/csrc/kernels/k_step.hip b/minbpe_amd/csrc/kernels/k_step.hip
--- a/minbpe_amd/csrc/kernels/k_step.hip
+++ b/minbpe_amd/csrc/kernels/k_step.hip
@@ -7,7 +7,8 @@
 namespace BPE_G {
 
 constexpr uint32_t STEP_PUB_WORDS = 32;
-static_assert(2 + 2 * CH_KSWEEP == STEP_PUB_WORDS, "the line holds the pairs and their counts");
+constexpr int STEP_KCAP = 15;
+static_assert(2 + 2 * STEP_KCAP == STEP_PUB_WORDS && STEP_KCAP <= CH_KSWEEP, "the line holds the pairs and their counts");
 
 union StepLds {
     PoolLds p;
@@ -55,14 +56,14 @@
         if (tid < STEP_PUB_WORDS) {
             const uint32_t status = st->status, defer = st->defer;
             const uint32_t noop = (status || defer) ? 1u : 0u;
-            const uint32_t K = noop ? 0u : min(st->bk, (uint32_t)CH_KSWEEP);
+            const uint32_t K = noop ? 0u : min(st->bk, (uint32_t)STEP_KCAP);
             uint32_t v = 0;
             if (tid == 0)
                 v = K | (st->brep << 8) | ((st->sel_ran ? 1u : 0u) << 16) | (noop << 17) | ((st->pool_hint_next ? 1u : 0u) << 18) |
                     ((defer & 3u) << 19) | ((st->sel_mode & 1u) << 21);
             else if (tid == 1) v = 256u + st->iter;
             else if (tid - 2 < K) v = ((uint32_t)st->ba[tid - 2] << 16) | ((uint32_t)st->bb[tid - 2] & 0xFFFFu);
-            else if (tid >= 2 + CH_KSWEEP && tid - (2 + CH_KSWEEP) < K) v = st->bcnt[tid - (2 + CH_KSWEEP)];
+            else if (tid >= 2 + STEP_KCAP && tid - (2 + STEP_KCAP) < K) v = st->bcnt[tid - (2 + STEP_KCAP)];
             s_b[tid] = v;
             granule_put(S.pub + tid, S.tag, v);
         }
@@ -134,21 +135,16 @@
 #pragma unroll
             for (int i = 0; i < 4; i++) v += ld_agent(&S.removed[(lane * 4 + i) * REMOVED_STRIDE]);
         }
-        static_assert(CH_RMV == 16, "lanes 4p .. 4p + 3 hold the removals of pair p");
+        static_assert(CH_RMV == 8, "lanes 2p, 2p + 1 hold the removals of pair p");
+        const uint32_t tot = wave_sum_u32(v);
         v += (uint32_t)__shfl_xor((int)v, 1);
-        v += (uint32_t)__shfl_xor((int)v, 2);
-        uint32_t rem[CH_KMAX];
+        uint32_t rem[STEP_KCAP + 1];
 #pragma unroll
-        for (int p = 0; p < CH_KMAX; p++) rem[p] = (uint32_t)__shfl((int)v, 4 * p);
-        if (K == 1) {
-            uint32_t tot = 0;
-#pragma unroll
-            for (int p = 0; p < CH_KMAX; p++) tot += rem[p];
-            rem[0] = tot;
-        }
+        for (int p = 0; p < STEP_KCAP + 1; p++) rem[p] = (uint32_t)__shfl((int)v, 2 * p);
+        if (K == 1) rem[0] = tot;
         if (!S.removed) {
 #pragma unroll
-            for (int p = 0; p < CH_KMAX; p++) rem[p] = p < CH_KSWEEP ? s_b[2 + CH_KSWEEP + p] : 0u;
+            for (int p = 0; p < STEP_KCAP + 1; p++) rem[p] = p < STEP_KCAP ? s_b[2 + STEP_KCAP + p] : 0u;
         }
         const uint32_t iter = z0 - 256u;
         unsigned long long nn = st->n[S.par];
@@ -172,7 +168,7 @@
                 unsigned long long m = st->n[S.par];
                 for (uint32_t p = 0; p < K; p++) {
                     m -= rem[p];
-                    iter_rec_put(S.rec + iter + p, (int32_t)(s_b[2 + p] >> 16), (int32_t)(s_b[2 + p] & 0xFFFFu), s_b[2 + CH_KSWEEP + p], ST_OK, m);
+                    iter_rec_put(S.rec + iter + p, (int32_t)(s_b[2 + p] >> 16), (int32_t)(s_b[2 + p] & 0xFFFFu), s_b[2 + STEP_KCAP + p], ST_OK, m);
                 }
                 __builtin_amdgcn_s_waitcnt(0);
                 for (uint32_t p = 0; p < K; p++) iter_rec_seal(S.rec + iter + p, (unsigned long long)(iter + p) + 1);
```

Measured after the change: 55270 merges/s (median of 6 runs). 1.04x the previous value.
